# zengxianyu/sketchedit

Hardware: AMD Instinct MI355X
Metric: images/sec (higher is better)
Workload: dtype f32; 1 GPU; SketchEdit inference forward (netM+netG, use_cam, pool max) 256x256 batch 32 per GPU, procedural weights; global_batch=32, size=256, per_gpu_batch=32, execution=default, two streams

## Files before the change

### sketchedit_amd/_lib.py

```python
import contextlib
import ctypes
import os
import subprocess
import threading

import numpy as np

_HERE = os.path.dirname(os.path.abspath(__file__))
LIB_PATH = os.environ.get("SKETCHEDIT_HIP_LIB") or os.path.join(_HERE, "lib", "libsketchedit_hip.so")
CSRC = os.path.join(_HERE, "csrc")
SOURCES = ["se_gconv.hip", "se_rconv16.hip", "se_rconv96.hip", "se_rtile.hip", "se_rtilew.hip", "se_wino.hip", "se_wino24.hip", "se_wino48.hip", "se_wino_up.hip", "se_wino_up48.hip", "se_s2poly.hip", "se_attention.hip", "se_att_stream.hip", "se_misc.hip", "se_resize.hip",
           "se_window.hip", "se_feather.hip", "se_fill.hip", "se_select.hip", "se_lasso.hip", "se_modify.hip", "se_outline.hip", "se_move.hip", "se_blend.hip", "se_canvas.hip", "se_warp.hip", "se_filter.hip", "se_adjust.hip", "se_png.hip", "se_jpg.hip", "se_pack.hip",
           "se_plan.hip", "se_api_window.hip", "se_api_select.hip", "se_api_move.hip", "se_api_codec.hip", "se_api_debug.hip", "se_api.hip"]

SE_NET_G, SE_NET_M = 0, 1
RESAMPLE_LANCZOS, RESAMPLE_BILINEAR, RESAMPLE_BICUBIC = 1, 2, 3
FLAG_USE_CAM, FLAG_POOL_MAX, FLAG_NO_MASK_CC, FLAG_NO_MASK_COARSE, FLAG_JOINT_TRAIN_INP = 1, 2, 4, 8, 16
FLAG_LOW_LATENCY, FLAG_GRAPH, FLAG_PACKED_OUT, FLAG_BF16, FLAG_CONSERVATIVE = 32, 64, 128, 256, 512
LOW_LATENCY_MAX_PIXELS = 3 * 256 * 256
LOW_LATENCY_MAX_SINGLE_IMAGE = 512 * 512

SYMBOLS = ["se_create", "se_destroy", "se_last_error", "se_version", "se_load_weights", "se_weights_ready",
           "se_workspace_bytes", "se_netM_forward", "se_netM_forward_ex", "se_netG_forward", "se_netG_forward_taps", "se_inference", "se_inference_u8", "se_gated_conv2d",
           "se_gated_conv2d_ex", "se_attention", "se_attention_ex", "se_quantize_u8", "se_dequantize_u8", "se_inference_u8io", "se_profile_enable",
           "se_profile_report", "se_debug_set_option", "se_debug_get_option", "se_debug_reset_options", "se_debug_gconv_form",
           "se_resize_u8", "se_prepare_u8", "se_edit_u8", "se_edit_u8_workspace_bytes", "se_resample_coeffs",
           "se_window_gather_u8", "se_window_border_u8", "se_window_paste_u8", "se_edit_window_u8", "se_edit_window_u8_workspace_bytes",
           "se_window_gather_resize_u8", "se_window_paste_resize_u8", "se_edit_window_scaled_u8", "se_edit_window_scaled_u8_workspace_bytes",
           "se_window_saved_bytes", "se_window_save_u8", "se_window_swap_u8",
           "se_inference_locked", "se_inference_u8_locked", "se_window_gather_lock_u8", "se_window_paste_locked_u8",
           "se_edit_window_locked_u8", "se_edit_window_locked_u8_workspace_bytes", "se_sketch_tiles_u8",
           "se_sketch_strokes_u8",
           "se_pack_inputs", "se_column_reduce", "se_output_conv"]
PNG_SYMBOLS = ["se_png_bound", "se_png_encode_u8", "se_png_encode_u8_workspace_bytes"]
JPG_SYMBOLS = ["se_jpg_bound", "se_jpg_encode_u8", "se_jpg_encode_u8_workspace_bytes"]
JPG2_SYMBOLS = ["se_jpg2_bound", "se_jpg2_encode_u8", "se_jpg2_encode_u8_workspace_bytes", "se_jpg2_code_i16",
                "se_jpg2_code_i16_workspace_bytes"]
SE_JPG_420, SE_JPG_OPTIMIZE = 1, 2
JPG_TABLE_RECORD_BYTES = 1088
FEATHER_SYMBOLS = ["se_window_paste_feather_u8"]
FEATHER_MAX_RADIUS = 16
FILL_SYMBOLS = ["se_fill", "se_fill_window_u8", "se_fill_window_u8_workspace_bytes", "se_fill_keep_u8"]
SELECT_SYMBOLS = ["se_select_similar_u8", "se_select_flood_u8", "se_select_grow_u8"]
SELECT_MAX_GROW, SELECT_MAX_PASSES = 16, 64
LASSO_SYMBOLS = ["se_lasso_fill_u8", "se_plane_combine_u8"]
LASSO_MAX_EDGES, LASSO_MAX_EXTENT = 65536, 8192
COMBINE_ADD, COMBINE_SUBTRACT, COMBINE_INTERSECT, COMBINE_XOR, COMBINE_INVERT = range(5)
OUTLINE_SYMBOLS = ["se_outline_u8_workspace_bytes", "se_outline_u8"]
OUTLINE_TILE, OUTLINE_MAX_CAP = 64, 1 << 24
MOVE_SYMBOLS = ["se_move_drop_u8", "se_plane_shift_u8"]
MOVE_MAX_OFFSET, MOVE_MAX_RADIUS = 16384, 16
MOVE_FLIP_X, MOVE_FLIP_Y = 1, 2
BLEND_ENTRIES = ["sketchedit_move_blend_u8_workspace_bytes", "sketchedit_move_blend_u8"]
BLEND_MAX_SIDE = 2048
CANVAS_ENTRIES = ["skedit_canvas_u8"]
CANVAS_MIRROR_X, CANVAS_MIRROR_Y, CANVAS_TRANSPOSE = 1, 2, 4
CANVAS_EDGE, CANVAS_REFLECT, CANVAS_CONSTANT = 0, 1, 2
CANVAS_MAX_SIDE, CANVAS_MAX_OFFSET = 32768, 1 << 20
WARP_SYMBOLS = ["se_warp_drop_u8", "se_plane_warp_u8"]
WARP_MAX_COEF, WARP_MAX_TRANSLATION = 1 << 20, 1 << 40
FILTER_SYMBOLS = ["se_filter_blur_u8", "se_filter_mosaic_u8"]
FILTER_MAX_RADIUS, FILTER_ONE, FILTER_MAX_CELL = 32, 4096, 64
FILTER_MIN_AMOUNT, FILTER_MAX_AMOUNT, FILTER_MAX_FEATHER = -256, 1024, 16

ADJUST_SYMBOLS = ["se_adjust_u8", "se_adjust_hist_u8_workspace_bytes", "se_adjust_hist_u8", "se_adjust_lut_u8"]
ADJUST_MAX_COEF, ADJUST_MAX_OFFSET, ADJUST_ONE_AMOUNT = 32768, 1 << 20, 256
ADJUST_MAX_FEATHER, ADJUST_MAX_CLIP, ADJUST_HIST_GROUPS = 16, 200, 256
ADJUST_STRETCH, ADJUST_EQUALIZE, ADJUST_MATCH = 0, 1, 2
ADJUST_PER_CHANNEL, ADJUST_LUMA = 0, 1
MODIFY_SYMBOLS = ["se_plane_modify_u8"]
MODIFY_MAX_RADIUS = 32
MODIFY_EXPAND, MODIFY_CONTRACT, MODIFY_SMOOTH = range(3)


class SketchEditHipError(RuntimeError):
    pass


class NetGTaps(ctypes.Structure):
    _fields_ = [("pmconv6", ctypes.c_void_p), ("attn_out", ctypes.c_void_p), ("style_vec", ctypes.c_void_p)]


class Window(ctypes.Structure):
    _fields_ = [("frame_u8", ctypes.c_void_p), ("sketch_u8", ctypes.c_void_p), ("Hi", ctypes.c_int), ("Wi", ctypes.c_int),
                ("y0", ctypes.c_int), ("x0", ctypes.c_int)]


class OutputConvIO(ctypes.Structure):
    _fields_ = [(n, ctypes.c_void_p) for n in ("out", "hard", "lock", "img", "mask", "xnow", "composed", "rgb8", "m8")]


def build_library(force=False, verbose=False, extra_flags=()):
    import fcntl
    from concurrent.futures import ThreadPoolExecutor
    import glob
    hdrs = glob.glob(os.path.join(CSRC, "*.h")) + glob.glob(os.path.join(_HERE, "..", "include", "*.h"))
    hdr_t = max(os.path.getmtime(h) for h in hdrs)
    objdir = os.path.join(_HERE, "lib", "obj")
    os.makedirs(objdir, exist_ok=True)
    with open(os.path.join(_HERE, "lib", ".build.lock"), "w") as lock:
        fcntl.flock(lock, fcntl.LOCK_EX)
        jobs, objs = [], []
        for src in SOURCES:
            sp, op = os.path.join(CSRC, src), os.path.join(objdir, src.replace(".hip", ".o"))
            objs.append(op)
            cmd = ["hipcc", "--offload-arch=gfx950", "-O3", "-std=c++17", "-fPIC"] + list(extra_flags) + ["-c", sp, "-o", op]
            try:
                with open(op + ".cmd") as f:
                    same_cmd = f.read() == " ".join(cmd)
            except OSError:
                same_cmd = False
            if force or not same_cmd or not os.path.exists(op) or os.path.getmtime(op) < max(os.path.getmtime(sp), hdr_t):
                jobs.append(cmd)
        if not jobs and os.path.exists(LIB_PATH) and all(os.path.getmtime(LIB_PATH) >= os.path.getmtime(o) for o in objs):
            return LIB_PATH

        def run(cmd):
            if verbose:
                print(" ".join(cmd), flush=True)
            subprocess.check_call(cmd)
            if "-c" in cmd:
                with open(cmd[-1] + ".cmd", "w") as f:
                    f.write(" ".join(cmd))
        with ThreadPoolExecutor(max_workers=min(len(jobs), os.cpu_count() or 1) or 1) as ex:
            list(ex.map(run, jobs))
        run(["hipcc", "--offload-arch=gfx950", "-fPIC", "-shared", "-o", LIB_PATH + ".tmp"] + objs)
        os.replace(LIB_PATH + ".tmp", LIB_PATH)
    return LIB_PATH


_lib = None
_lib_lock = threading.Lock()


def load_library():
    global _lib
    with _lib_lock:
        if _lib is not None:
            return _lib
        if not os.path.exists(LIB_PATH):
            raise SketchEditHipError(
                "%s not found: build it with `python -c 'import __graft_entry__ as g; g.build()'` "
                "(there is no CPU or PyTorch fallback for this path)" % LIB_PATH)
        import torch
        lib = ctypes.CDLL(LIB_PATH)
        c_f = ctypes.c_void_p
        vp, ci, sz = ctypes.c_void_p, ctypes.c_int, ctypes.c_size_t
        lib.se_create.argtypes = [ci, ctypes.POINTER(vp)]
        lib.se_create.restype = ci
        lib.se_destroy.argtypes = [vp]
        lib.se_destroy.restype = None
        lib.se_last_error.argtypes = [vp]
        lib.se_last_error.restype = ctypes.c_char_p
        lib.se_version.argtypes = []
        lib.se_version.restype = ctypes.c_char_p
        lib.se_load_weights.argtypes = [vp, ci, ctypes.c_char_p, c_f, ctypes.POINTER(ci), ci]
        lib.se_load_weights.restype = ci
        lib.se_weights_ready.argtypes = [vp]
        lib.se_weights_ready.restype = ci
        lib.se_workspace_bytes.argtypes = [vp, ci, ci, ci]
        lib.se_workspace_bytes.restype = sz
        lib.se_netM_forward.argtypes = [vp, vp, c_f, c_f, c_f, c_f, vp, sz, ci, ci, ci]
        lib.se_netM_forward.restype = ci
        lib.se_netM_forward_ex.argtypes = [vp, vp, c_f, c_f, c_f, c_f, vp, sz, ci, ci, ci, ci]
        lib.se_netM_forward_ex.restype = ci
        lib.se_netG_forward.argtypes = [vp, vp, c_f, c_f, c_f, c_f, c_f, c_f, c_f, vp, sz, ci, ci, ci, ci]
        lib.se_netG_forward.restype = ci
        lib.se_netG_forward_taps.argtypes = [vp, vp, c_f, c_f, c_f, c_f, c_f, c_f, c_f, vp, sz, ci, ci, ci, ci, ctypes.POINTER(NetGTaps)]
        lib.se_netG_forward_taps.restype = ci
        lib.se_inference.argtypes = [vp, vp, c_f, c_f, c_f, c_f, c_f, c_f, c_f, c_f, vp, sz, ci, ci, ci, ci]
        lib.se_inference.restype = ci
        lib.se_inference_u8.argtypes = [vp, vp, c_f, c_f, vp, vp, vp, sz, ci, ci, ci, ci]
        lib.se_inference_u8.restype = ci
        lib.se_gated_conv2d.argtypes = [vp, vp, c_f, c_f, c_f, c_f] + [ci] * 10
        lib.se_gated_conv2d.restype = ci
        lib.se_gated_conv2d_ex.argtypes = [vp, vp, c_f, c_f, ci, c_f, c_f, c_f] + [ci] * 12
        lib.se_gated_conv2d_ex.restype = ci
        lib.se_attention.argtypes = [vp, vp, c_f, c_f, c_f, c_f, ci, ci, ci]
        lib.se_attention.restype = ci
        lib.se_attention_ex.argtypes = [vp, vp, c_f, c_f, c_f, c_f, ci, ci, ci, ci]
        lib.se_attention_ex.restype = ci
        lib.se_quantize_u8.argtypes = [vp, vp, c_f, c_f, vp, vp, ci, ci, ci]
        lib.se_quantize_u8.restype = ci
        lib.se_dequantize_u8.argtypes = [vp, vp, vp, vp, c_f, c_f, ci, ci, ci]
        lib.se_dequantize_u8.restype = ci
        lib.se_inference_u8io.argtypes = [vp, vp, vp, vp, vp, vp, vp, sz, ci, ci, ci, ci]
        lib.se_inference_u8io.restype = ci
        lib.se_resize_u8.argtypes = [vp, vp, vp, ci, ci, ci, ci, vp, ci, ci, ci]
        lib.se_resize_u8.restype = ci
        lib.se_prepare_u8.argtypes = [vp, vp, vp, ci, ci, vp, ci, ci, c_f, c_f, ci, ci]
        lib.se_prepare_u8.restype = ci
        lib.se_edit_u8.argtypes = [vp, vp, vp, vp, vp, vp, sz, ci, ci, ci, ci, ci, ci]
        lib.se_edit_u8.restype = ci
        lib.se_edit_u8_workspace_bytes.argtypes = [vp, ci, ci, ci]
        lib.se_edit_u8_workspace_bytes.restype = sz
        lib.se_window_gather_u8.argtypes = [vp, vp, ctypes.POINTER(Window), ci, ci, ci, c_f, c_f]
        lib.se_window_gather_u8.restype = ci
        lib.se_window_border_u8.argtypes = [vp, vp, ctypes.POINTER(Window), ci, ci, ci, vp, vp]
        lib.se_window_border_u8.restype = ci
        lib.se_window_paste_u8.argtypes = [vp, vp, ctypes.POINTER(Window), ci, ci, ci, vp, vp]
        lib.se_window_paste_u8.restype = ci
        lib.se_edit_window_u8.argtypes = [vp, vp, ctypes.POINTER(Window), ci, ci, ci, vp, vp, vp, ci, vp, sz, ci]
        lib.se_edit_window_u8.restype = ci
        lib.se_edit_window_u8_workspace_bytes.argtypes = [vp, ci, ci, ci]
        lib.se_edit_window_u8_workspace_bytes.restype = sz
        lib.se_window_gather_resize_u8.argtypes = [vp, vp, ctypes.POINTER(Window), ci, ci, ci, ci, ci, c_f, c_f]
        lib.se_window_gather_resize_u8.restype = ci
        lib.se_window_paste_resize_u8.argtypes = [vp, vp, ctypes.POINTER(Window), ci, ci, ci, ci, ci, vp, vp]
        lib.se_window_paste_resize_u8.restype = ci
        lib.se_edit_window_scaled_u8.argtypes = [vp, vp, ctypes.POINTER(Window), ci, ci, ci, ci, ci, vp, vp, vp, ci, vp, sz, ci]
        lib.se_edit_window_scaled_u8.restype = ci
        lib.se_edit_window_scaled_u8_workspace_bytes.argtypes = [vp, ci, ci, ci, ci, ci]
        lib.se_edit_window_scaled_u8_workspace_bytes.restype = sz
        lib.se_window_saved_bytes.argtypes = [ci, ci]
        lib.se_window_saved_bytes.restype = sz
        lib.se_window_save_u8.argtypes = [vp, vp, ctypes.POINTER(Window), ci, ci, ci, ctypes.POINTER(vp)]
        lib.se_window_save_u8.restype = ci
        lib.se_window_swap_u8.argtypes = [vp, vp, ctypes.POINTER(Window), ci, ci, ci, ctypes.POINTER(vp)]
        lib.se_window_swap_u8.restype = ci
        lib.se_inference_locked.argtypes = [vp, vp, c_f, c_f, vp, c_f, c_f, c_f, c_f, c_f, c_f, vp, sz, ci, ci, ci, ci]
        lib.se_inference_locked.restype = ci
        lib.se_inference_u8_locked.argtypes = [vp, vp, c_f, c_f, vp, vp, vp, vp, sz, ci, ci, ci, ci]
        lib.se_inference_u8_locked.restype = ci
        lib.se_window_gather_lock_u8.argtypes = [vp, vp, ctypes.POINTER(Window), ctypes.POINTER(vp), ci, ci, ci, ci, ci, vp]
        lib.se_window_gather_lock_u8.restype = ci
        lib.se_window_paste_locked_u8.argtypes = [vp, vp, ctypes.POINTER(Window), ctypes.POINTER(vp), ci, ci, ci, ci, ci, vp, vp]
        lib.se_window_paste_locked_u8.restype = ci
        lib.se_edit_window_locked_u8.argtypes = [vp, vp, ctypes.POINTER(Window), ctypes.POINTER(vp), ci, ci, ci, ci, ci, vp, vp, vp, ci, vp, sz, ci]
        lib.se_edit_window_locked_u8.restype = ci
        lib.se_edit_window_locked_u8_workspace_bytes.argtypes = [vp, ci, ci, ci, ci, ci]
        lib.se_edit_window_locked_u8_workspace_bytes.restype = sz
        lib.se_sketch_tiles_u8.argtypes = [vp, vp, vp, ci, ci, ci, vp]
        lib.se_sketch_tiles_u8.restype = ci
        lib.se_sketch_strokes_u8.argtypes = [vp, vp, vp, ci, ci, ci, vp, ci, vp, vp]
        lib.se_sketch_strokes_u8.restype = ci
        lib.se_pack_inputs.argtypes = [vp, vp, ci, c_f, c_f, c_f, c_f, c_f, vp, vp, ci, ci, ci, ci, ci]
        lib.se_pack_inputs.restype = ci
        lib.se_column_reduce.argtypes = [vp, vp, c_f, c_f, vp, ci, ci, ci, ci, ci, ci]
        lib.se_column_reduce.restype = ci
        lib.se_output_conv.argtypes = [vp, vp, c_f, c_f, c_f, ci, ci, ci, ci, ci, ctypes.POINTER(OutputConvIO), ci, ci, ci]
        lib.se_output_conv.restype = ci
        lib.se_png_bound.argtypes = [ci, ci]
        lib.se_png_bound.restype = sz
        lib.se_png_encode_u8.argtypes = [vp, vp, ctypes.POINTER(Window), ci, ci, ci, vp, sz, vp, vp, sz]
        lib.se_png_encode_u8.restype = ci
        lib.se_png_encode_u8_workspace_bytes.argtypes = [vp, ci, ci, ci]
        lib.se_png_encode_u8_workspace_bytes.restype = sz
        lib.se_jpg_bound.argtypes = [ci, ci]
        lib.se_jpg_bound.restype = sz
        lib.se_jpg_encode_u8.argtypes = [vp, vp, ctypes.POINTER(Window), ci, ci, ci, ci, vp, sz, vp, vp, sz]
        lib.se_jpg_encode_u8.restype = ci
        lib.se_jpg_encode_u8_workspace_bytes.argtypes = [vp, ci, ci, ci]
        lib.se_jpg_encode_u8_workspace_bytes.restype = sz
        lib.se_jpg2_bound.argtypes = [ci, ci, ci]
        lib.se_jpg2_bound.restype = sz
        lib.se_jpg2_encode_u8.argtypes = [vp, vp, ctypes.POINTER(Window), ci, ci, ci, ci, ci, vp, sz, vp, vp, vp, sz]
        lib.se_jpg2_encode_u8.restype = ci
        lib.se_jpg2_encode_u8_workspace_bytes.argtypes = [vp, ci, ci, ci, ci]
        lib.se_jpg2_encode_u8_workspace_bytes.restype = sz
        lib.se_jpg2_code_i16.argtypes = [vp, vp, vp, ci, ci, ci, ci, vp, sz, vp, vp, vp, sz]
        lib.se_jpg2_code_i16.restype = ci
        lib.se_jpg2_code_i16_workspace_bytes.argtypes = [vp, ci, ci, ci, ci]
        lib.se_jpg2_code_i16_workspace_bytes.restype = sz
        lib.se_window_paste_feather_u8.argtypes = [vp, vp, ctypes.POINTER(Window), ctypes.POINTER(vp), ci, ci, ci, ci, vp, vp]
        lib.se_window_paste_feather_u8.restype = ci
        lib.se_fill.argtypes = [vp, vp, c_f, c_f, vp, vp, c_f, c_f, c_f, c_f, vp, sz, ci, ci, ci, ci]
        lib.se_fill.restype = ci
        lib.se_fill_window_u8.argtypes = [vp, vp, ctypes.POINTER(Window), ctypes.POINTER(vp), ctypes.POINTER(vp), ci, ci, ci, ci, ci, vp, vp, vp, sz, ci]
        lib.se_fill_window_u8.restype = ci
        lib.se_fill_window_u8_workspace_bytes.argtypes = [vp, ci, ci, ci, ci, ci]
        lib.se_fill_window_u8_workspace_bytes.restype = sz
        lib.se_fill_keep_u8.argtypes = [vp, vp, ctypes.POINTER(Window), ctypes.POINTER(vp), ctypes.POINTER(vp), ctypes.POINTER(vp), ci, ci, ci]
        lib.se_fill_keep_u8.restype = ci
        lib.se_select_similar_u8.argtypes = [vp, vp, vp, ci, ci, ci, ci, ci, ci, vp]
        lib.se_select_similar_u8.restype = ci
        lib.se_select_flood_u8.argtypes = [vp, vp, vp, ci, ci, ci, vp]
        lib.se_select_flood_u8.restype = ci
        lib.se_select_grow_u8.argtypes = [vp, vp, vp, ci, ci, ci, vp]
        lib.se_select_grow_u8.restype = ci
        lib.se_lasso_fill_u8.argtypes = [vp, vp, vp, ci, ci, ci, vp]
        lib.se_lasso_fill_u8.restype = ci
        lib.se_plane_combine_u8.argtypes = [vp, vp, vp, vp, ci, ci, ci, vp]
        lib.se_plane_combine_u8.restype = ci
        lib.se_plane_modify_u8.argtypes = [vp, vp, vp, ci, ci, ci, ci, vp]
        lib.se_plane_modify_u8.restype = ci
        lib.se_move_drop_u8.argtypes =[vp, vp, vp, ci, ci, vp, ci, ci, ci, ci, vp, vp] + [ci] * 8
        lib.se_move_drop_u8.restype = ci
        lib.sketchedit_move_blend_u8_workspace_bytes.argtypes = [ci, ci]
        lib.sketchedit_move_blend_u8_workspace_bytes.restype = sz
        lib.sketchedit_move_blend_u8.argtypes = [vp, vp, vp, ci, ci, vp, ci, ci, ci, ci, vp, vp] + [ci] * 7 + [vp, sz]
        lib.sketchedit_move_blend_u8.restype = ci
        lib.skedit_canvas_u8.argtypes = [vp, vp, vp, ci, ci, ci, vp, ci, ci, ci, ci, ci, ci, ctypes.c_uint]
        lib.skedit_canvas_u8.restype = ci
        lib.se_plane_shift_u8.argtypes = [vp, vp, vp, ci, ci] + [ci] * 7 + [vp]
        lib.se_plane_shift_u8.restype = ci
        lib.se_warp_drop_u8.argtypes = [vp, vp, vp, ci, ci, vp, ci, ci, ci, ci, vp, vp] + [ci] * 8 + [vp]
        lib.se_warp_drop_u8.restype = ci
        lib.se_plane_warp_u8.argtypes = [vp, vp, vp, ci, ci] + [ci] * 4 + [vp, vp]
        lib.se_plane_warp_u8.restype = ci
        lib.se_filter_blur_u8.argtypes = [vp, vp, vp, ci, ci, vp, ci, ci, ci, ci, vp, vp] + [ci] * 4 + [vp, ci, ci, ci]
        lib.se_filter_blur_u8.restype = ci
        lib.se_filter_mosaic_u8.argtypes = [vp, vp, vp, ci, ci, vp, ci, ci, ci, ci, vp, vp] + [ci] * 7
        lib.se_filter_mosaic_u8.restype = ci
        lib.se_adjust_u8.argtypes = [vp, vp, vp, ci, ci, vp, ci, ci, ci, ci, vp, vp] + [ci] * 4 + [vp, vp, ci, ci]
        lib.se_adjust_u8.restype = ci
        lib.se_adjust_hist_u8_workspace_bytes.argtypes = [ci, ci]
        lib.se_adjust_hist_u8_workspace_bytes.restype = sz
        lib.se_adjust_hist_u8.argtypes = [vp, vp, vp, ci, ci, vp] + [ci] * 4 + [vp, vp, sz]
        lib.se_adjust_hist_u8.restype = ci
        lib.se_adjust_lut_u8.argtypes = [vp, vp, vp, vp, ci, ci, ci, vp]
        lib.se_adjust_lut_u8.restype = ci
        lib.se_outline_u8_workspace_bytes.argtypes = [vp, ci, ci]
        lib.se_outline_u8_workspace_bytes.restype = sz
        lib.se_outline_u8.argtypes = [vp, vp, vp, ci, ci, vp, ci, vp, vp, sz]
        lib.se_outline_u8.restype = ci
        lib.se_resample_coeffs.argtypes = [ci, ci, ci, vp, vp, sz]
        lib.se_resample_coeffs.restype = ci
        lib.se_profile_enable.argtypes = [vp, ci]
        lib.se_profile_enable.restype = ci
        lib.se_profile_report.argtypes = [vp, ctypes.c_char_p, sz]
        lib.se_profile_report.restype = ci
        lib.se_debug_set_option.argtypes = [ctypes.c_char_p, ci]
        lib.se_debug_set_option.restype = ci
        lib.se_debug_get_option.argtypes = [ctypes.c_char_p, ctypes.POINTER(ci)]
        lib.se_debug_get_option.restype = ci
        lib.se_debug_reset_options.argtypes = []
        lib.se_debug_reset_options.restype = None
        _lib = lib
        return lib


_shared = {}
_shared_lock = threading.Lock()


def shared_engine(device=0):
    with _shared_lock:
        if device not in _shared:
            _shared[device] = Engine(device)
        return _shared[device]


def set_option(name, value):
    if load_library().se_debug_set_option(name.encode(), int(value)):
        raise SketchEditHipError("unknown developer switch %r" % name)


def get_option(name):
    v = ctypes.c_int(0)
    if load_library().se_debug_get_option(name.encode(), ctypes.byref(v)):
        raise SketchEditHipError("unknown developer switch %r" % name)
    return v.value


def reset_options():
    load_library().se_debug_reset_options()


def gconv_form(cin, cout, H, W, k=3, stride=1, rate=1, act="elu", upsample=False, cin1=0, x1_is_vector=False, B=1,
               low_latency=False, bf16=False, conservative=False, net=SE_NET_G):
    flags = (FLAG_LOW_LATENCY if low_latency else 0) | (FLAG_BF16 if bf16 else 0) | (FLAG_CONSERVATIVE if conservative else 0)
    buf = ctypes.create_string_buffer(64)
    fn = load_library().se_debug_gconv_form
    fn.argtypes, fn.restype = [ctypes.c_int] * 14 + [ctypes.c_char_p, ctypes.c_size_t], ctypes.c_int
    if fn(cin, cin1, int(bool(x1_is_vector)), cout, k, stride, rate, {"elu": 0, "relu": 1, None: 2}[act],
          int(bool(upsample)), B, H, W, flags, net, buf, len(buf)):
        raise SketchEditHipError("gconv_form: not a layer gated_conv2d takes")
    return buf.value.decode().split(",")


def s2poly_tables():
    return np.array([[get_option("SE_S2POLY_TABLE:%d,%d" % (q, j)) for j in range(7)] for q in range(5)], np.int32)


def s2poly_probe_layer(cout):
    p = lambda n: (((7919 * n) % 2053 - 1026) / 1024.0).astype(np.float32)
    return p(np.arange(cout * 48 * 9, dtype=np.int64)).reshape(cout, 48, 3, 3), p(10007 + np.arange(cout, dtype=np.int64))


def s2poly_probe_pack(cout):
    fn = load_library().se_debug_get_option
    n = (cout // 96) * 38 * 96 * 32
    out = np.zeros(n + cout, np.int32)
    v = ctypes.c_int(0)
    for i in range(n + cout):
        if fn(("SE_S2POLY_PACK:%d,%d" % (cout, i)).encode(), ctypes.byref(v)):
            raise SketchEditHipError("SE_S2POLY_PACK: cout must be 96 or 192")
        out[i] = v.value
    f = out.view(np.float32)
    return f[:n].reshape(cout // 96, 38, 96, 32).copy(), f[n:].copy()


def pair_rule(B, H, W, low_latency=False):
    v = ctypes.c_int(-1)
    name = "SE_PAIR_RULE:%d,%d,%d,%d" % (B, H, W, FLAG_LOW_LATENCY if low_latency else 0)
    if load_library().se_debug_get_option(name.encode(), ctypes.byref(v)):
        raise SketchEditHipError("pair_rule: bad shape B=%d H=%d W=%d" % (B, H, W))
    return bool(v.value)


def flags_from_opt(opt):
    f = 0
    if getattr(opt, "use_cam", False):
        f |= FLAG_USE_CAM
    pool = getattr(opt, "pool_type", "avg")
    if pool == "max":
        f |= FLAG_POOL_MAX
    elif pool != "avg":
        raise NotImplementedError(pool)
    if getattr(opt, "no_mask_cc", False):
        f |= FLAG_NO_MASK_CC
    if getattr(opt, "no_mask_coarse", False):
        f |= FLAG_NO_MASK_COARSE
    if getattr(opt, "joint_train_inp", False):
        f |= FLAG_JOINT_TRAIN_INP
    return f


def _ptr(t):
    return None if t is None else ctypes.c_void_p(t.data_ptr())


def _check_dev(*ts):
    import torch
    for t in ts:
        if t is None:
            continue
        if not (isinstance(t, torch.Tensor) and t.is_cuda and t.dtype == torch.float32 and t.is_contiguous()):
            raise SketchEditHipError("expected contiguous float32 CUDA(HIP) tensors")


def upload_u8(a, device):
    import warnings
    import torch
    if isinstance(a, np.ndarray):
        with warnings.catch_warnings():
            warnings.simplefilter("ignore", UserWarning)
            a = torch.from_numpy(np.ascontiguousarray(a))
    return a.to(device, non_blocking=True).contiguous()


def _check_dev_u8(*ts):
    import torch
    for t in ts:
        if not (isinstance(t, torch.Tensor) and t.is_cuda and t.dtype == torch.uint8 and t.is_contiguous()):
            raise SketchEditHipError("expected contiguous uint8 CUDA(HIP) tensors")


class Engine:

    def __init__(self, device=0):
        import torch
        if not torch.cuda.is_available():
            raise SketchEditHipError("no HIP device visible: the sketchedit_amd forward only runs on an MI355X")
        self.lib = load_library()
        self.device = int(device)
        h = ctypes.c_void_p()
        if self.lib.se_create(self.device, ctypes.byref(h)) != 0:
            raise SketchEditHipError("se_create: " + self.lib.se_last_error(None).decode())
        self.h = h
        self._ws = None
        self._ws_lock = threading.Lock()
        self._ws_stream = None
        self._graph_stream = None
        self.precision = "f32"
        self.conservative = False
        self._static = {}
        self._graph_lock = threading.Lock()

    def close(self):
        if getattr(self, "h", None):
            self.lib.se_destroy(self.h)
            self.h = None

    def __del__(self):
        try:
            self.close()
        except Exception:
            pass

    def _err(self, what):
        raise SketchEditHipError("%s: %s" % (what, self.lib.se_last_error(self.h).decode()))

    def load_state_dict(self, net, state_dict):
        net_id = SE_NET_G if net == "G" else SE_NET_M
        for k, v in state_dict.items():
            a = v.detach().cpu().numpy() if hasattr(v, "detach") else np.asarray(v)
            a = np.ascontiguousarray(a, dtype=np.float32)
            shape = (ctypes.c_int * a.ndim)(*a.shape)
            if self.lib.se_load_weights(self.h, net_id, k.encode(), a.ctypes.data_as(ctypes.c_void_p), shape, a.ndim):
                self._err("se_load_weights(%s)" % k)

    def weights_ready(self):
        return bool(self.lib.se_weights_ready(self.h))

    def workspace(self, B, H, W):
        need = self.lib.se_workspace_bytes(self.h, B, H, W)
        if need == 0:
            self._err("se_workspace_bytes")
        return self._workspace_bytes(need)

    def _workspace_bytes(self, need):
        import torch
        with self._ws_lock:
            cur = torch.cuda.current_stream(self.device)
            if self._ws is None or self._ws.numel() < need:
                if self._ws is not None:
                    self._ws.record_stream(self._ws_stream)
                self._ws = torch.empty(need, dtype=torch.uint8, device="cuda:%d" % self.device)
                with self._graph_lock:
                    self._static.clear()
            elif self._ws_stream is not None and self._ws_stream != cur:
                cur.wait_stream(self._ws_stream)
            self._ws_stream = cur
            return self._ws

    def _stream(self):
        import torch
        return ctypes.c_void_p(torch.cuda.current_stream(self.device).cuda_stream)

    def netM(self, image, sketch, want_image=True):
        import torch
        _check_dev(image, sketch)
        B, _, H, W = image.shape
        ws = self.workspace(B, H, W)
        mask = torch.empty((B, 1, H, W), dtype=torch.float32, device=image.device)
        mim = torch.empty((B, 3, H, W), dtype=torch.float32, device=image.device) if want_image else None
        if self.lib.se_netM_forward_ex(self.h, self._stream(), _ptr(image), _ptr(sketch), _ptr(mask), _ptr(mim),
                                       _ptr(ws), ws.numel(), B, H, W,
                                       (FLAG_BF16 if self.precision == "bf16" else 0) | (FLAG_CONSERVATIVE if self.conservative else 0)):
            self._err("se_netM_forward_ex")
        return mask, mim

    def netG(self, x, x2, mask, mask2, guide, flags):
        import torch
        _check_dev(x, x2, mask, mask2, guide)
        B, _, H, W = x.shape
        ws = self.workspace(B, H, W)
        coarse = torch.empty((B, 3, H, W), dtype=torch.float32, device=x.device)
        fine = torch.empty_like(coarse)
        flags = (flags & 31) | (FLAG_BF16 if self.precision == "bf16" else 0)
        if self.lib.se_netG_forward(self.h, self._stream(), _ptr(x), _ptr(x2), _ptr(mask), _ptr(mask2), _ptr(guide),
                                    _ptr(coarse), _ptr(fine), _ptr(ws), ws.numel(), B, H, W, flags):
            self._err("se_netG_forward")
        return coarse, fine

    def netG_taps(self, x, x2, mask, mask2, guide, flags):
        import torch
        _check_dev(x, x2, mask, mask2, guide)
        B, _, H, W = x.shape
        ws = self.workspace(B, H, W)
        mk = lambda *shape: torch.empty(shape, dtype=torch.float32, device=x.device)
        r = dict(coarse=mk(B, 3, H, W), fine=mk(B, 3, H, W), pmconv6=mk(B, 96, H // 4, W // 4), style_vec=mk(B, 96))
        if flags & FLAG_USE_CAM:
            r["attn_out"] = mk(B, 96, H // 4, W // 4)
        taps = NetGTaps(r["pmconv6"].data_ptr(), r["attn_out"].data_ptr() if "attn_out" in r else None, r["style_vec"].data_ptr())
        flags = (flags & 31) | (FLAG_BF16 if self.precision == "bf16" else 0)
        if self.lib.se_netG_forward_taps(self.h, self._stream(), _ptr(x), _ptr(x2), _ptr(mask), _ptr(mask2), _ptr(guide),
                                         _ptr(r["coarse"]), _ptr(r["fine"]), _ptr(ws), ws.numel(), B, H, W, flags, ctypes.byref(taps)):
            self._err("se_netG_forward_taps")
        return r

    def set_conservative(self, on=True):
        self.conservative = bool(on)

    def set_precision(self, precision):
        if precision not in ("f32", "bf16"):
            raise ValueError(precision)
        self.precision = precision

    @staticmethod
    def is_low_latency(B, H, W, low_latency=None):
        if low_latency is not None:
            return bool(low_latency)
        return B * H * W <= LOW_LATENCY_MAX_PIXELS or (B == 1 and H * W <= LOW_LATENCY_MAX_SINGLE_IMAGE)

    def exec_flags(self, B, H, W, low_latency=None, graph=False):
        return (FLAG_LOW_LATENCY if self.is_low_latency(B, H, W, low_latency) else 0) | (FLAG_GRAPH if graph else 0) | \
            (FLAG_BF16 if self.precision == "bf16" else 0) | (FLAG_CONSERVATIVE if self.conservative else 0)

    def inference(self, image, sketch, flags, visualize=False, out=None, low_latency=None, graph=False, lock=None):
        import torch
        _check_dev(image, sketch)
        if lock is not None:
            self._check_lock(lock, image)
            graph = False
        if graph and out is not None:
            raise SketchEditHipError("graph=True replays into buffers the Engine keeps per shape: `out=` cannot be honoured "
                                     "(copy from the returned tensors, or call without graph=True)")
        B, _, H, W = image.shape
        ws = self.workspace(B, H, W)
        dev = image.device
        flags = (flags & 31) | self.exec_flags(B, H, W, low_latency, graph)

        def new_outputs(have=None):
            mk = lambda c: torch.empty((B, c, H, W), dtype=torch.float32, device=dev)
            o = dict(composed=have["composed"], mask=have["mask"]) if have else dict(composed=mk(3), mask=mk(1))
            if visualize:
                o.update(hard=mk(1), maskim=mk(3), coarse=mk(3), fine=mk(3))
            return o

        if graph:
            with self._graph_lock:
                return self._inference_graph(image, sketch, flags, visualize, ws, B, H, W, new_outputs)
        r = new_outputs(out)
        self._call_inference(image, sketch, r, ws, B, H, W, flags, self._stream(), lock)
        return r

    @staticmethod
    def _check_lock(lock, image):
        _check_dev_u8(lock)
        B, _, H, W = image.shape
        if tuple(lock.shape) != (B, H, W):
            raise SketchEditHipError("lock: expected a (B,H,W) uint8 plane of the images' size")

    def _call_inference(self, image, sketch, r, ws, B, H, W, flags, stream, lock=None):
        if lock is not None:
            if self.lib.se_inference_locked(self.h, stream, _ptr(image), _ptr(sketch), _ptr(lock), _ptr(r["composed"]),
                                            _ptr(r["mask"]), _ptr(r.get("hard")), _ptr(r.get("maskim")), _ptr(r.get("coarse")),
                                            _ptr(r.get("fine")), _ptr(ws), ws.numel(), B, H, W, flags):
                self._err("se_inference_locked")
            return
        if self.lib.se_inference(self.h, stream, _ptr(image), _ptr(sketch), _ptr(r["composed"]), _ptr(r["mask"]),
                                 _ptr(r.get("hard")), _ptr(r.get("maskim")), _ptr(r.get("coarse")), _ptr(r.get("fine")),
                                 _ptr(ws), ws.numel(), B, H, W, flags):
            self._err("se_inference")

    def _inference_graph(self, image, sketch, flags, visualize, ws, B, H, W, new_outputs):
        import torch
        key = (B, H, W, bool(visualize))
        st = self._static.get(key)
        if st is None:
            st = self._static[key] = {"image": torch.empty_like(image), "sketch": torch.empty_like(sketch),
                                      "outs": new_outputs()}
        st["image"].copy_(image)
        st["sketch"].copy_(sketch)
        image, sketch = st["image"], st["sketch"]
        r = dict(st["outs"])
        cur = torch.cuda.current_stream(self.device)
        if self._graph_stream is None:
            self._graph_stream = torch.cuda.Stream(device=self.device)
        gs = self._graph_stream
        gs.wait_stream(cur)
        self._call_inference(image, sketch, r, ws, B, H, W, flags, ctypes.c_void_p(gs.cuda_stream))
        cur.wait_stream(gs)
        return r

    def inference_u8(self, image, sketch, flags, low_latency=None, lock=None):
        import torch
        _check_dev(image, sketch)
        if lock is not None:
            self._check_lock(lock, image)
        B, _, H, W = image.shape
        ws = self.workspace(B, H, W)
        rgb = torch.empty((B, H, W, 3), dtype=torch.uint8, device=image.device)
        m8 = torch.empty((B, H, W), dtype=torch.uint8, device=image.device)
        flags = (flags & 31) | self.exec_flags(B, H, W, low_latency, False)
        if lock is not None:
            if self.lib.se_inference_u8_locked(self.h, self._stream(), _ptr(image), _ptr(sketch), _ptr(lock), _ptr(rgb), _ptr(m8),
                                               _ptr(ws), ws.numel(), B, H, W, flags):
                self._err("se_inference_u8_locked")
        elif self.lib.se_inference_u8(self.h, self._stream(), _ptr(image), _ptr(sketch), _ptr(rgb), _ptr(m8), _ptr(ws),
                                      ws.numel(), B, H, W, flags):
            self._err("se_inference_u8")
        return rgb, m8

    def dequantize_u8(self, image_u8, sketch_u8):
        import torch
        _check_dev_u8(image_u8, sketch_u8)
        B, H, W, _ = image_u8.shape
        image = torch.empty((B, 3, H, W), dtype=torch.float32, device=image_u8.device)
        sketch = torch.empty((B, 1, H, W), dtype=torch.float32, device=image_u8.device)
        if self.lib.se_dequantize_u8(self.h, self._stream(), _ptr(image_u8), _ptr(sketch_u8), _ptr(image), _ptr(sketch), B, H, W):
            self._err("se_dequantize_u8")
        return image, sketch

    def inference_u8io(self, image_u8, sketch_u8, flags, low_latency=None, out=None):
        import torch
        _check_dev_u8(image_u8, sketch_u8)
        B, H, W, _ = image_u8.shape
        assert tuple(sketch_u8.shape) == (B, H, W)
        ws = self.workspace(B, H, W)
        rgb, m8 = out if out is not None else (torch.empty((B, H, W, 3), dtype=torch.uint8, device=image_u8.device),
                                               torch.empty((B, H, W), dtype=torch.uint8, device=image_u8.device))
        flags = (flags & 31) | self.exec_flags(B, H, W, low_latency, False)
        if self.lib.se_inference_u8io(self.h, self._stream(), _ptr(image_u8), _ptr(sketch_u8), _ptr(rgb), _ptr(m8), _ptr(ws),
                                      ws.numel(), B, H, W, flags):
            self._err("se_inference_u8io")
        return rgb, m8

    def resize_u8(self, x, size, filter=RESAMPLE_BICUBIC, out=None):
        import torch
        _check_dev_u8(x)
        flat = x.dim() == 3
        B, Hin, Win = x.shape[:3]
# ... 845 lines not shown
```

### sketchedit_amd/csrc/se_api_debug.hip

```cpp
#include "se_host.h"
#include "se_s2poly.h"

using namespace se;

extern "C" {

int se_profile_enable(se_ctx* c, int on) {
  if (!c) return 1;
  std::lock_guard<std::mutex> lk(c->mu);
  HIPCHK(c, hipSetDevice(c->device));
  c->prof.recs.clear();
  c->prof.used = 0;
  if (on && c->prof.pool.empty()) {
    c->prof.pool.resize(2 * 1024);
    for (auto& e : c->prof.pool) HIPCHK(c, hipEventCreate(&e));
  }
  c->prof.on = on != 0;
  return 0;
}

int se_profile_report(se_ctx* c, char* buf, size_t cap) {
  if (!c || !buf || cap < 64) return 1;
  std::lock_guard<std::mutex> lk(c->mu);
  HIPCHK(c, hipSetDevice(c->device));
  HIPCHK(c, hipDeviceSynchronize());
  double ms[PL_COUNT] = {0}, fl[PL_COUNT] = {0}, by[PL_COUNT] = {0}, ex[PL_COUNT] = {0}, bl[PL_COUNT] = {0};
  long n[PL_COUNT] = {0};
  for (auto& r : c->prof.recs) {
    float t = 0.f;
    if (hipEventElapsedTime(&t, r.a, r.b) == hipSuccess) { ms[r.label] += t; fl[r.label] += r.flops; ex[r.label] += r.exec_flops; by[r.label] += r.bytes; bl[r.label] += (double)r.blocks; n[r.label]++; }
  }
  std::string s = "{\"kernels\": [";
  bool first = true;
  for (int l = 0; l < PL_COUNT; ++l) {
    if (!n[l]) continue;
    char t[384];
    snprintf(t, sizeof t, "%s{\"kernel\": \"%s\", \"launches\": %ld, \"total_ms\": %.6f, \"flops\": %.6e, \"flops_executed\": %.6e, \"bytes\": %.6e, \"workgroups\": %.1f}",
             first ? "" : ", ", prof_label_name(l), n[l], ms[l], fl[l], ex[l], by[l], bl[l] / (double)n[l]);
    s += t;
    first = false;
  }
  s += "], \"layers\": [";
  std::vector<std::string> keys;
  std::map<std::string, std::pair<double, double>> agg;
  std::map<std::string, double> aggx;
  std::map<std::string, long> cnt;
  for (auto& r : c->prof.recs) {
    if (!r.name) continue;
    float t = 0.f;
    if (hipEventElapsedTime(&t, r.a, r.b) != hipSuccess) continue;
    std::string k = std::string(prof_label_name(r.label)) + ":" + r.name;
    if (!cnt.count(k)) keys.push_back(k);
    agg[k].first += t; agg[k].second += r.flops; aggx[k] += r.exec_flops; cnt[k]++;
  }
  first = true;
  for (auto& k : keys) {
    char t[384];
    snprintf(t, sizeof t, "%s{\"layer\": \"%s\", \"launches\": %ld, \"total_ms\": %.6f, \"flops\": %.6e, \"flops_executed\": %.6e}",
             first ? "" : ", ", k.c_str(), cnt[k], agg[k].first, agg[k].second, aggx[k]);
    s += t;
    first = false;
  }
  s += "], \"launches\": [";
  first = true;
  for (auto& r : c->prof.recs) {
    char t[256];
    snprintf(t, sizeof t, "%s{\"form\": \"%s\", \"kernel\": \"%s\", \"layer\": \"%s\", \"workgroups\": %ld}", first ? "" : ", ",
             r.form ? r.form : "?", prof_label_name(r.label), r.name ? r.name : "", r.blocks);
    s += t;
    first = false;
  }
  s += "]}";
  if (s.size() + 1 > cap) return fail(c, "profile buffer too small");
  memcpy(buf, s.c_str(), s.size() + 1);
  return 0;
}

int se_debug_set_option(const char* name, int value) { return opt_set(name, value); }
int se_debug_get_option(const char* name, int* value) {
  static const char q[] = "SE_PAIR_RULE:";
  if (name && value && !strncmp(name, q, sizeof q - 1)) {
    int B = 0, H = 0, W = 0, flags = 0, end = 0;
    if (sscanf(name + sizeof q - 1, "%d,%d,%d,%d%n", &B, &H, &W, &flags, &end) != 4 || name[sizeof q - 1 + end] || B < 1 || H < 1 || W < 1) return 1;
    *value = pair_rule(B, H, W, flags) ? 1 : 0;
    return 0;
  }
  static const char qt[] = "SE_S2POLY_TABLE:", qp[] = "SE_S2POLY_PACK:";
  if (name && value && !strncmp(name, qt, sizeof qt - 1)) {
    int q = -1, j = -1, end = 0;
    if (sscanf(name + sizeof qt - 1, "%d,%d%n", &q, &j, &end) != 2 || name[sizeof qt - 1 + end] || q < 0 || q > 4 || j < 0 || j > 6) return 1;
    *value = j == 0 ? s2poly_src_a(q) : j == 1 ? s2poly_src_b(q) : j < 5 ? s2poly_wcoef(q, j - 2) : s2poly_fold(q, j - 5);
    return 0;
  }
  if (name && value && !strncmp(name, qp, sizeof qp - 1)) {
    int cout = 0, end = 0;
    long long i = -1;
    if (sscanf(name + sizeof qp - 1, "%d,%lld%n", &cout, &i, &end) != 2 || name[sizeof qp - 1 + end] || (cout != 96 && cout != 192) || i < 0) return 1;
    static std::mutex mu;
    static std::vector<float> kept[2];
    std::lock_guard<std::mutex> lk(mu);
    std::vector<float>& all = kept[cout == 192];
    if (all.empty()) {
      auto probe = [](long long n) { return (float)((7919 * n) % 2053 - 1026) / 1024.f; };
      std::vector<float> w((size_t)cout * 48 * 9), b(cout), bias;
      for (size_t n = 0; n < w.size(); ++n) w[n] = probe((long long)n);
      for (int n = 0; n < cout; ++n) b[n] = probe(10007 + n);
      if (!s2poly_pack_host(w.data(), b.data(), cout, all, bias)) return 1;
      all.insert(all.end(), bias.begin(), bias.end());
    }
    if ((size_t)i >= all.size()) return 1;
    memcpy(value, &all[(size_t)i], sizeof(int));
    return 0;
  }
  return opt_get(name, value);
}
void se_debug_reset_options(void) { opt_reset(); }

int se_debug_gconv_form(int cin, int cin1, int src1_is_vector, int cout, int k, int stride, int rate, int act, int upsample,
                        int B, int H, int W, int exec_flags, int net_id, char* out, size_t cap) {
  if (!out || cin <= 0 || cin1 < 0 || cout <= 0 || k <= 0 || stride <= 0 || rate <= 0 || B <= 0 || H <= 0 || W <= 0) return 1;
  const bool bf = (exec_flags & SE_FLAG_BF16) != 0;
  const int gran = bf ? 8 : 4;
  if (cin1 && ((cin % gran) || (cin1 % gran))) return 1;
  const LayerDef d = {"test", cin + cin1, cout, k, stride, rate, act, upsample};
  const bool raw = small_layer(d);
  if (raw && (k != 3 || cin != 12 || cin1 || (cout != 1 && cout != 3) || stride != 1 || rate != 1 || upsample)) return 1;
  if (!raw && (cout % 8)) return 1;
  const LayerFacts f = layer_facts(d, cin + cin1);
  if (!raw && f.cfg < 0) return 1;
  const int Cp = (cin + gran - 1) & ~(gran - 1);
  if (!raw && Cp + cin1 != f.CG[bf] * gran) return 1;
  const bool vec = cin1 && src1_is_vector;
  const ConvCall q = {d, f, B, H, W, Cp, cin1, cin1 ? (vec ? SRC2_VECTOR : SRC2_TENSOR) : SRC2_NONE, bf,
                      (exec_flags & SE_FLAG_LOW_LATENCY) != 0, (exec_flags & SE_FLAG_CONSERVATIVE) != 0, net_id, vec};
  const Choice ch = choose_form(q);
  const char* name = form_name(ch, q);
  if (!name) return 1;
  const std::string s = std::string(ch.fold ? "vecbias," : "") + name;
  if (s.size() + 1 > cap) return 1;
  memcpy(out, s.c_str(), s.size() + 1);
  return 0;
}

int se_gated_conv2d_ex(se_ctx* c, void* stream, const float* x, const float* x1, int x1_is_vector, const float* w_host,
                       const float* b_host, float* y, int B, int Cin, int Cin1, int H, int W, int Cout, int k, int stride,
                       int rate, int act, int upsample, int exec_flags) {
  if (!c || !x || !w_host || !b_host || !y) return 1;
  std::lock_guard<std::mutex> lk(c->mu);
  HIPCHK(c, hipSetDevice(c->device));
  begin_call(c, stream, exec_flags & (SE_FLAG_LOW_LATENCY | SE_FLAG_BF16));
  const bool bf = c->bf16;
  if (!x1) Cin1 = 0;
  if (x1 && ((Cin % 4) || (Cin1 % 4))) return fail(c, "two-source conv: channel counts must be multiples of 4");
  if (bf && x1 && ((Cin % 8) || (Cin1 % 8))) return fail(c, "two-source bf16 conv: channel counts must be multiples of 8");
  const int CinT = Cin + Cin1;
  Layer L;
  L.def = LayerDef{"test", CinT, Cout, k, stride, rate, act, upsample};
  const bool raw = small_layer(L.def);
  if (raw && (k != 3 || CinT != 12 || x1 || (Cout != 1 && Cout != 3) || stride != 1 || rate != 1 || upsample))
    return fail(c, "raw conv: only 3x3 12->{1,3}");
  if (!raw && (Cout % 8)) return fail(c, "gated conv needs Cout %% 8 == 0");
  L.w.assign(w_host, w_host + (size_t)Cout * CinT * k * k);
  L.b.assign(b_host, b_host + Cout);
  std::vector<int> chans(CinT);
  std::iota(chans.begin(), chans.end(), 0);
  if (pack_layer_images(L, chans, c->err)) return 1;
  const int Cp = bf ? (Cin + 7) & ~7 : (Cin + 3) & ~3;
  DevBuf xin, x1in, yout, vb_test;
  struct Drain {
    se_ctx* c;
    ~Drain() {
      (void)hipStreamSynchronize(c->st);
      c->vbias_ws = nullptr; c->vec32 = nullptr;
    }
  } drain{c};
  HIPCHK(c, xin.alloc((size_t)B * H * W * Cp * 4));
  if (poison(c, xin, (size_t)B * H * W * Cp * 4, c->st)) return 1;
  int rc = (bf ? launch_nchw_to_nhwc16 : launch_nchw_to_nhwc)(x, xin, B, Cin, Cp, H, W, c->st) != hipSuccess;
  if (!rc && x1) {
    const size_t n1 = x1_is_vector ? (size_t)B * Cin1 : (size_t)B * H * W * Cin1;
    HIPCHK(c, x1in.alloc(n1 * 4));
    if (poison(c, x1in, n1 * 4, c->st)) return 1;
    if (x1_is_vector && !bf) rc = hipMemcpyAsync(x1in, x1, n1 * 4, hipMemcpyDeviceToDevice, c->st) != hipSuccess;
    else if (x1_is_vector) rc = launch_nchw_to_nhwc16(x1, x1in, B, Cin1, Cin1, 1, 1, c->st) != hipSuccess;
    else rc = (bf ? launch_nchw_to_nhwc16 : launch_nchw_to_nhwc)(x1, x1in, B, Cin1, Cin1, H, W, c->st) != hipSuccess;
  }
  if (!rc && raw) {
    SmallConvParams sp;
    memset(&sp, 0, sizeof sp);
    sp.x = xin; sp.w = L.direct[bf]; sp.b = L.d_b; sp.B = B; sp.H = H; sp.W = W; sp.cout = Cout; sp.mode = 4;
    sp.bf16 = bf ? 1 : 0;
    sp.out_nchw = y;
    rc = launch_small_conv(sp, c->st) != hipSuccess;
  } else if (!rc) {
    const ConvShape sh = conv_shape(L.def, H, W);
    const int Gs = bf ? (Cout / 2 + 7) & ~7 : Cout / 2;
    HIPCHK(c, yout.alloc((size_t)B * sh.Ho * sh.Wo * Gs * 4));
    if (poison(c, yout, (size_t)B * sh.Ho * sh.Wo * Gs * 4, c->st)) return 1;
    if (x1in && x1_is_vector) {
      HIPCHK(c, vb_test.alloc((size_t)B * 9 * 192 * 4));
      if (poison(c, vb_test, (size_t)B * 9 * 192 * 4, c->st)) return 1;
      c->vbias_ws = vb_test;
      c->vec32 = bf ? x1 : nullptr;
    }
    rc = run_gconv(c, L, xin, Cp, x1in, Cin1, x1_is_vector, yout, B, H, W);
    if (!rc) rc = (bf ? launch_nhwc16_to_nchw : launch_nhwc_to_nchw)(yout, y, B, Cout / 2, Gs, sh.Ho, sh.Wo, c->st) != hipSuccess;
  }
  return rc;
}

int se_gated_conv2d(se_ctx* c, void* stream, const float* x, const float* w_host, const float* b_host, float* y, int B,
                    int Cin, int H, int W, int Cout, int k, int stride, int rate, int act, int upsample) {
  return se_gated_conv2d_ex(c, stream, x, nullptr, 0, w_host, b_host, y, B, Cin, 0, H, W, Cout, k, stride, rate, act,
                            upsample, 0);
}

int se_attention_ex(se_ctx* c, void* stream, const float* x, const float* mask_full, float* out, float* similar_out, int B,
                    int h, int w, int exec_flags) {
  if (!c || !x || !mask_full || !out) return 1;
  std::lock_guard<std::mutex> lk(c->mu);
  if (h < 4 || w < 4 || (h % 2) || (w % 2)) return fail(c, "attention: h, w must be even and >= 4");
  HIPCHK(c, hipSetDevice(c->device));
  begin_call(c, stream, exec_flags & SE_FLAG_BF16);
  const bool bf = c->bf16;
  const int R = (h / 2) * (w / 2), Rp = att_row_stride(R, true) + 64;
  const bool streaming = att_streaming(h, w, bf, similar_out != nullptr);
  const int L = ((h - 4) / 2 + 1) * ((w - 4) / 2 + 1);
  if (streaming && similar_out)
    return fail(c, "attention: similar_out (the %d x %d score matrix) is not available on a %dx%d feature map: "
                   "it runs in the streaming form, which never forms it", L, L, h, w);
  const size_t rr = streaming ? 0 : 2 * (size_t)B * R * Rp;
  const size_t bytes = ((size_t)B * h * w * 96 * 3 + rr + (size_t)B * Rp * (7 + 4 * 96) + 64 * 96 * B + 2 * (size_t)B * R + 9 * (size_t)(w / 2 + 72) + (size_t)B * (768 + (h / 2) * 384)) * 4 + (1 << 16);
  char* ws = nullptr;
  HIPCHK(c, hipMalloc(&ws, bytes));
  if (poison(c, ws, bytes, c->st)) { (void)hipStreamSynchronize(c->st); (void)hipFree(ws); return 1; }
  c->arena.reset(ws, bytes, false);
  c->arena2.reset(nullptr, 0, false);
  Plan P(c, c->G, B);
  Act xin = P.alloc(h, w, 96), o = P.alloc(h, w, 96);
  int rc = P.rc;
  if (!rc) rc = (bf ? launch_nchw_to_nhwc16 : launch_nchw_to_nhwc)(x, xin.p, B, 96, 96, h, w, c->st) != hipSuccess;
  if (!rc) rc = run_attention(c, P, xin, mask_full, o, similar_out);
  if (!rc) rc = (bf ? launch_nhwc16_to_nchw : launch_nhwc_to_nchw)(o.p, out, B, 96, 96, h, w, c->st) != hipSuccess;
  (void)hipStreamSynchronize(c->st);
  (void)hipFree(ws);
  return rc;
}

int se_attention(se_ctx* c, void* stream, const float* x, const float* mask_full, float* out, float* similar_out, int B,
                 int h, int w) {
  return se_attention_ex(c, stream, x, mask_full, out, similar_out, B, h, w, 0);
}

int se_pack_inputs(se_ctx* c, void* stream, int net_id, const float* x, const float* x2, const float* mask, const float* mask2,
                   const float* guide, void* packed_out, void* style_out, int B, int H, int W, int flags, int exec_flags) {
  if (!c) return 1;
  std::lock_guard<std::mutex> lk(c->mu);
  if (B < 1 || H < 1 || W < 1) return fail(c, "pack: bad shape B=%d H=%d W=%d", B, H, W);
  if (net_id != SE_NET_M && net_id != SE_NET_G) return fail(c, "pack: net_id must be SE_NET_G or SE_NET_M");
  if (!x || !guide || !packed_out || (net_id == SE_NET_G && (!x2 || !mask || !mask2 || !style_out))) return fail(c, "null pointer argument");
  HIPCHK(c, hipSetDevice(c->device));
  begin_call(c, stream, exec_flags & SE_FLAG_BF16);
  if (net_id == SE_NET_M) {
    HIPCHK(c, (c->bf16 ? launch_pack_m16 : launch_pack_m)(x, guide, (float*)packed_out, B, H, W, c->st));
  } else {
    HIPCHK(c, (c->bf16 ? launch_pack_g16 : launch_pack_g)(x, x2, mask, mask2, guide, (float*)packed_out, (float*)style_out, B, H, W,
                                                          (flags & SE_FLAG_NO_MASK_CC) ? 1 : 0,
                                                          (flags & SE_FLAG_JOINT_TRAIN_INP) ? 1 : 0, c->st));
  }
  return 0;
}

int se_column_reduce(se_ctx* c, void* stream, const float* x, float* out, unsigned short* out_bf16, int B, int C, int H, int W,
                     int op, int exec_flags) {
  if (!c) return 1;
  std::lock_guard<std::mutex> lk(c->mu);
  if (!x || !out) return fail(c, "null pointer argument");
  if (B < 1 || C < 1 || H < 1 || W < 1) return fail(c, "column reduce: bad shape B=%d C=%d H=%d W=%d", B, C, H, W);
  if (op < 0 || op > 2) return fail(c, "column reduce: op must be 0 (max), 1 (mean) or 2 (rsqrt of the sum of squares)");
  const bool bf = (exec_flags & SE_FLAG_BF16) != 0;
  if (C > 256 || C % (bf ? 8 : 4))
    return fail(c, "column reduce: C = %d must be a multiple of %d and at most 256", C, bf ? 8 : 4);
  if ((double)B * H * W * C * (bf ? 2 : 4) >= 2147483648.0) return fail(c, "column reduce: B H W C beyond the 32-bit byte range");
  HIPCHK(c, hipSetDevice(c->device));
  begin_call(c, stream, exec_flags & SE_FLAG_BF16);
  DevBuf xin, part;
  struct Drain {
    se_ctx* c;
    ~Drain() { (void)hipStreamSynchronize(c->st); }
  } drain{c};
  const size_t xbytes = (size_t)B * H * W * C * (bf ? 2 : 4), pbytes = (size_t)B * COLREDUCE_SPLITS * C * 4;
  HIPCHK(c, xin.alloc(xbytes));
  HIPCHK(c, part.alloc(pbytes));
  if (poison(c, xin, xbytes, c->st) || poison(c, part, pbytes, c->st)) return 1;
  HIPCHK(c, (bf ? launch_nchw_to_nhwc16 : launch_nchw_to_nhwc)(x, xin, B, C, C, H, W, c->st));
  HIPCHK(c, launch_colreduce(xin, part, out, B, H * W, C, op, c->st, bf ? 1 : 0, (float*)out_bf16));
  return 0;
}

int se_output_conv(se_ctx* c, void* stream, const float* x, const float* w_host, const float* b_host, int B, int H, int W, int cout,
                   int mode, const se_output_conv_io* io, int no_mask_coarse, int packed, int exec_flags) {
  if (!c) return 1;
  std::lock_guard<std::mutex> lk(c->mu);
  if (!x || !w_host || !b_host || !io) return fail(c, "null pointer argument");
  if (B < 1 || H < 1 || W < 1) return fail(c, "output conv: bad shape B=%d H=%d W=%d", B, H, W);
  if (mode < 0 || mode > 3) return fail(c, "output conv: mode must be 0..3");
  if (cout != (mode == 0 ? 1 : 3)) return fail(c, "output conv: mode %d has %d output channels", mode, mode == 0 ? 1 : 3);
  if (mode == 0 && !io->out) return fail(c, "output conv: mode 0 writes `out`");
  if (mode == 2 && (!io->img || !io->mask || !io->xnow)) return fail(c, "output conv: mode 2 needs img, mask and xnow");
  if (mode == 3 && (io->composed || io->rgb8 || io->m8) && (!io->img || !io->mask))
    return fail(c, "output conv: the composite of mode 3 needs img and mask");
  HIPCHK(c, hipSetDevice(c->device));
  begin_call(c, stream, exec_flags & SE_FLAG_BF16);
  const bool bf = c->bf16;
  Layer L;
  L.def = LayerDef{"test", 12, cout, 3, 1, 1, ACT_NONE, 0};
  L.w.assign(w_host, w_host + (size_t)cout * 12 * 9);
  L.b.assign(b_host, b_host + cout);
  std::vector<int> chans(12);
  std::iota(chans.begin(), chans.end(), 0);
  if (pack_layer_images(L, chans, c->err)) return 1;
  DevBuf xin;
  struct Drain {
    se_ctx* c;
    ~Drain() { (void)hipStreamSynchronize(c->st); }
  } drain{c};
  const int Cp = bf ? 16 : 12;
  const size_t xbytes = (size_t)B * H * W * Cp * (bf ? 2 : 4);
  HIPCHK(c, xin.alloc(xbytes));
  if (poison(c, xin, xbytes, c->st)) return 1;
  HIPCHK(c, (bf ? launch_nchw_to_nhwc16 : launch_nchw_to_nhwc)(x, xin, B, 12, Cp, H, W, c->st));
  SmallConvParams sp;
  memset(&sp, 0, sizeof sp);
  sp.x = xin; sp.w = L.direct[bf]; sp.b = L.d_b; sp.B = B; sp.H = H; sp.W = W; sp.cout = cout;
  sp.bf16 = bf ? 1 : 0;
  sp.mode = mode; sp.out_nchw = io->out; sp.hard = io->hard; sp.img = io->img; sp.mask = io->mask; sp.xnow = (float*)io->xnow;
  sp.composed = io->composed; sp.no_mask_coarse = no_mask_coarse ? 1 : 0;
  if (mode == 3) { sp.rgb8 = io->rgb8; sp.m8 = io->m8; }
  if (mode == 0) sp.lock = io->lock;
  if (packed) {
    const long packed_bs = 4l * H * W;
    if (mode == 0) sp.out_bs = packed_bs;
    if (mode == 3) { sp.mask_bs = packed_bs; sp.comp_bs = packed_bs; }
  }
  HIPCHK(c, launch_small_conv(sp, c->st));
  return 0;
}

}
```

### sketchedit_amd/csrc/se_dispatch.h

```cpp
#pragma once
#include "se_kernels.h"

namespace se {

enum { ACT_ELU = 0, ACT_RELU = 1, ACT_NONE = 2 };

struct LayerDef {
  const char* name;
  int cin, cout, k, stride, rate, act, up;
};

inline bool small_layer(const LayerDef& d) { return d.act == ACT_NONE || d.cout == 3; }

struct ConvShape { int Ho, Wo, pad; };
inline ConvShape conv_shape(const LayerDef& d, int Hin, int Win) {
  const int pad = d.rate * (d.k - 1) / 2;
  if (d.up) return {2 * Hin, 2 * Win, pad};
  const int span = d.rate * (d.k - 1) + 1;
  return {(Hin + 2 * pad - span) / d.stride + 1, (Win + 2 * pad - span) / d.stride + 1, pad};
}

inline int choose_cfg(int G) {
  if (G <= 16) return GC_N24;
  if (G <= 24) return GC_N48;
  if (G <= 48) return GC_N96;
  if (G <= 96) return GC_N192;
  return -1;
}

inline bool rconv96_eligible(const LayerDef& d) {
  if (d.cout != 96 || d.rate != 1 || d.k != 3 || d.act == ACT_NONE) return false;
  if (d.stride == 2) return !d.up && d.cin == 24;
  if (d.stride != 1) return false;
  return d.up ? d.cin == 96 : (d.cin == 48 || d.cin == 24);
}

struct LayerFacts {
  bool small;
  int cfg, NP, G, T;
  int nch[2], CG[2];
  int dense, nchd;
  bool u, ub, u1, wv, wv16, u24, ub24, u24b, wx, wx2, wd, wdw, w16d, w16s, w96;
  bool s2p;
};

inline LayerFacts layer_facts(const LayerDef& d, int nchans) {
  LayerFacts f = {};
  f.cfg = -1;
  f.small = small_layer(d);
  if (f.small) return f;
  f.G = d.cout / 2;
  if (choose_cfg(f.G) < 0 || (f.G % 4)) return f;
  f.cfg = choose_cfg(f.G);
  f.NP = gconv_np(f.cfg);
  const int KW = d.up ? 2 : d.k;
  f.T = KW * KW;
  for (int bf = 0; bf < 2; ++bf) {
    const int per = bf ? 8 : 4, Cp = (nchans + per - 1) / per * per;
    f.CG[bf] = Cp / per;
    f.nch[bf] = (f.T * Cp + 8 * per - 1) / (8 * per);
  }
  const bool first = d.k == 5 && d.stride == 1 && d.rate == 1 && d.cout == 48;
  f.w16d = first && nchans >= 3 && nchans <= 4;
  f.wd = f.wdw = first && nchans >= 3 && nchans <= 5;
  f.dense = f.wd ? nchans : 0;
  f.nchd = (25 * f.dense + 31) / 32;
  f.w16s = d.k == 3 && d.stride == 1 && !d.up && (d.cin == 96 || d.cin == 192) && d.cout == 192;
  f.w96 = rconv96_eligible(d);
  f.s2p = d.k == 3 && d.stride == 2 && d.rate == 1 && !d.up && nchans == 48 && d.cin == 48 && (d.cout == 96 || d.cout == 192);
  if (d.k != 3 || d.stride != 1 || (nchans + 3) / 4 * 4 != d.cin) return f;
  if (d.up) {
    f.u = f.ub = (d.cin == 96 && d.cout == 96) || (d.cin == 48 && d.cout == 48);
  } else if ((d.cin == 96 || d.cin == 192) && d.cout == 192) {
    f.u = f.u24 = f.ub24 = true;
    f.u1 = f.wv = f.wv16 = f.u24b = d.cin == 192;
  } else if (d.cin == 48 && d.cout == 192) {
    f.u24 = f.ub24 = true;
  } else if (d.cin == 24 && d.cout == 24 && d.rate == 1) {
    f.wx = f.wx2 = true;
  } else if ((d.cin == 48 || d.cin == 24) && d.cout == 96) {
    f.u = f.ub = true;
  }
  return f;
}

enum { SRC2_NONE = 0, SRC2_TENSOR = 1, SRC2_VECTOR = 2 };
struct ConvCall {
  LayerDef def; LayerFacts facts;
  int B, Hin, Win, C0, C1;
  int src2;
  bool bf16, low_latency, conservative;
  int net;
  bool fold_scratch;
};

enum Form {
  F_SMALL_CONV, F_WINO, F_WINO24, F_WINO24_C48, F_WINO48, F_WINO48_C24, F_WINOUP, F_WINOUP48, F_RTILEW, F_RTILEW2,
  F_RTILE_DENSE5, F_RTILE_DENSE5W, F_RTILE_D4, F_RTILE, F_RCONV16, F_RCONV16_DUAL, F_RCONV96, F_S2POLY48, F_GATHER
};
struct Choice {
  Form form;
  bool fold;
  bool wino_range;
};

inline bool magic_cg_ok(int CG, int nch) {
  const int m = (65536 + CG - 1) / CG;
  for (int gi = 0; gi < nch * 8 + 8; ++gi)
    if (((gi * m) >> 16) != gi / CG) return false;
  return true;
}
inline bool magic_kw_ok(int KW, int T) {
  const int m = 256 / KW + 1;
  for (int t = 0; t <= T + 8; ++t)
    if (((t * m) >> 8) != t / KW) return false;
  return true;
}

inline Form choose_rtile(const ConvCall& q) {
  const LayerDef& d = q.def;
  const LayerFacts& f = q.facts;
  const bool bf = q.bf16;
  const int Hin = q.Hin, Win = q.Win, C0 = q.C0;
  const long long B = q.B;
  if (!opt(OPT_RTILE) || q.src2 || d.stride != 1 || d.rate != 1 || (f.cfg != GC_N48 && f.cfg != GC_N24)) return F_GATHER;
  const int TR = rtile_rows(bf);
  const long tiles = (long)((Hin + TR - 1) / TR) * ((Win + 15) / 16) * (d.up ? 4 : 1);
  if (q.low_latency && tiles < opt(OPT_RTILE_LL_MIN)) return F_GATHER;
  const int es = bf ? 2 : 4, gran = bf ? 8 : 4;
  if (C0 != f.CG[bf] * gran) return F_GATHER;
  const int wx_mode = opt(OPT_RTILE_WX);
  if (wx_mode != 0 && !bf && f.wx && d.k == 3 && !d.up && C0 == 24 && d.cin == 24 && d.cout == 24 && (Win % 2) == 0 &&
      B * Hin * Win * 96 < (1ll << 31))
    return wx_mode != 1 && f.wx2 && (Hin % 2) == 0 ? F_RTILEW2 : F_RTILEW;
  if (opt(OPT_RTILE_DENSE) != 0 && !bf && f.wd && f.dense && d.k == 5 && !d.up && f.cfg == GC_N48 && (long long)Hin * Win * C0 * 4 < (1ll << 31))
    return opt(OPT_RTILE_D5W) != 0 && f.wdw && (Win % 2) == 0 ? F_RTILE_DENSE5W : F_RTILE_DENSE5;
  if (opt(OPT_RTILE_DENSE) != 0 && bf && f.w16d && d.k == 5 && !d.up && f.cfg == GC_N48 && C0 == 8 && B * Hin * Win * 16 < (1ll << 31))
    return F_RTILE_D4;
  const int KW = d.up ? 2 : d.k;
  const int raw_bytes = ((TR + KW - 1) * (16 + KW - 1) * C0 * es + 1023) & ~1023;
  if (raw_bytes + f.nch[bf] * f.NP * 128 > 80 * 1024) return F_GATHER;
  if (B * Hin * Win * C0 * es >= (1ll << 31)) return F_GATHER;
  if (!magic_cg_ok(f.CG[bf], f.nch[bf]) || !magic_kw_ok(KW, f.T)) return F_GATHER;
  return F_RTILE;
}

inline bool rconv16_dual_ok(const LayerFacts& f, const LayerDef& d, int Hin, int Win) {
  if (opt(OPT_RCONV16_DUAL) == 0) return false;
  return f.w16s && (d.rate % 2) == 0 && Win / d.rate == 8 && Hin / d.rate <= 8 && Hin / d.rate >= 4;
}

inline Choice choose_form(const ConvCall& q) {
  const LayerDef& d = q.def;
  const LayerFacts& f = q.facts;
  const int Hin = q.Hin, Win = q.Win, C0 = q.C0, C1 = q.C1;
  const long long B = q.B;
  const bool two = q.src2 != SRC2_NONE, vec = q.src2 == SRC2_VECTOR, ll = q.low_latency;
  const ConvShape sh = conv_shape(d, Hin, Win);
  Choice ch = {F_GATHER, false, false};
  auto is = [&](Form form) { ch.form = form; return ch; };
  if (f.small) return is(F_SMALL_CONV);
  if (q.bf16) {
    const bool use_rconv = opt(OPT_RCONV16) != 0 && !ll && d.k == 3 && d.stride == 1 && !d.up && d.cout == 192 && C0 == 96 && f.w16s &&
                           B * Hin * Win * 192 < (1ll << 31);
    if (opt(OPT_VECBIAS) != 0 && use_rconv && vec && q.fold_scratch && f.wv16 && d.rate == 1 && d.cin == 192 && C1 == 96 && Hin >= 12 && Win >= 12) {
      ch.fold = true;
      return is(F_RCONV16);
    }
    if (use_rconv && d.cin == 96 && !two && (Hin % d.rate) == 0 && (Win % d.rate) == 0 && f.nch[1] == 14) {
      if (Hin / d.rate >= 12 && Win / d.rate >= 12) return is(F_RCONV16);
      if (rconv16_dual_ok(f, d, Hin, Win)) return is(F_RCONV16_DUAL);
    }
    if (opt(OPT_RCONV96) != 0 && !ll && f.w96 && !two && C0 == d.cin && Hin >= 12 && Win >= 12 &&
        B * sh.Ho * sh.Wo * 96 < (1ll << 31) && B * Hin * Win * C0 * 2 < (1ll << 31))
      return is(F_RCONV96);
    return is(choose_rtile(q));
  }
  auto grid_ok = [&](long wgs, int min_wg) { return !ll || (min_wg > 0 && wgs >= min_wg); };
  const int min192 = opt(OPT_LL_WINO_MIN_WG), min48 = opt(OPT_LL_WINO48_MIN_WG);
  const int f43_mode = opt(OPT_WINOGRAD_F43);
  const bool use_wino = opt(OPT_WINOGRAD) != 0;
  const bool even2 = (Hin % (2 * d.rate)) == 0 && (Win % (2 * d.rate)) == 0;
  const long wg64 = ((long)(Hin / 2) * (Win / 2) + 63) / 64;
  const bool fits96 = B * Hin * Win * 384 < (1ll << 31), fits48 = B * Hin * Win * 192 < (1ll << 31);
  const bool wino_src_ok = (!two && C0 == 96 && d.cin == 96) || (two && C0 == 96 && C1 == 96 && d.cin == 192);
  if (use_wino && !d.up && f.u && wino_src_ok && !fits96) ch.wino_range = true;
  if (use_wino && !d.up && f.u && wino_src_ok && fits96 && even2 && grid_ok(wg64, min192)) {
    ch.fold = opt(OPT_VECBIAS) != 0 && vec && d.rate == 1 && f.u1 && f.wv && q.fold_scratch && Hin >= 2 && Win >= 2;
    const bool s1 = two && !ch.fold;
    const bool f43_net_ok = q.net == 0 || (f43_mode == 1 && !q.conservative);
    const bool f43 = (f43_mode == 1 || f43_mode == 2) && f43_net_ok && (s1 ? (!vec && f.u24b) : f.u24) && f.ub24 && (Win % (4 * d.rate)) == 0;
    return is(f43 ? F_WINO24 : F_WINO);
  }
  if (use_wino && f43_mode != 0 && !d.up && !two && C0 == 48 && d.cin == 48 && d.cout == 192 && d.stride == 1 && f.u24 && f.ub24 && fits96 &&
      (Hin % (2 * d.rate)) == 0 && (Win % (4 * d.rate)) == 0 && grid_ok(((long)(Hin / 2) * (Win / 4) + 31) / 32, min192))
    return is(F_WINO24_C48);
  if (use_wino && opt(OPT_WINOGRAD48) != 0 && !d.up && f.u && f.ub && !two && fits48 && even2 && grid_ok(wg64, min48)) {
    if (C0 == 48 && d.cin == 48) return is(F_WINO48);
    if (C0 == 24 && d.cin == 24 && d.cout == 96 && d.stride == 1) return is(F_WINO48_C24);
  }
  if (use_wino && opt(OPT_WINOGRAD_UP) != 0 && d.up && f.u && f.ub && !two && (Hin % 2) == 0 && (Win % 2) == 0 && grid_ok(4 * wg64, min48)) {
    if (C0 == 96 && d.cin == 96 && fits96) return is(F_WINOUP);
    if (opt(OPT_WINOGRAD_UP48) != 0 && C0 == 48 && d.cin == 48 && d.cout == 48 && fits48 && B * sh.Ho * sh.Wo * 96 < (1ll << 31)) return is(F_WINOUP48);
  }
  const int s2_mode = opt(OPT_S2_POLY);
  if ((s2_mode == 1 || (s2_mode == 2 && q.net == 0)) && !ll && f.s2p && !two && d.k == 3 && d.stride == 2 && d.rate == 1 && !d.up && C0 == 48 &&
      d.cin == 48 && (d.cout == 96 || d.cout == 192) && (Hin % 4) == 0 && (Win % 4) == 0 && fits48)
    return is(F_S2POLY48);
  return is(choose_rtile(q));
}

inline const char* gconv_form_name(int cfg, bool small_grid, bool up2, bool two_src, bool bf16) {
#define SE_GF(n) n, n "_bf16", n "_2src", n "_2src_bf16", n "_up2", n "_up2_bf16", n "_up2_2src", n "_up2_2src_bf16"
#define SE_GS(n) { SE_GF(n), SE_GF(n "_small") }
  static const char* const names[4][16] = {SE_GS("gconv_n192"), SE_GS("gconv_n96"), SE_GS("gconv_n48"), SE_GS("gconv_n24")};
#undef SE_GS
#undef SE_GF
  if (cfg < 0 || cfg > 3) return nullptr;
  return names[cfg][(small_grid ? 8 : 0) | (up2 ? 4 : 0) | (two_src ? 2 : 0) | (bf16 ? 1 : 0)];
}

inline const char* form_name(const Choice& ch, const ConvCall& q) {
  const LayerDef& d = q.def;
  const bool two = q.src2 != SRC2_NONE && !ch.fold;
  switch (ch.form) {
    case F_SMALL_CONV: return "small_conv";
    case F_WINO: return two ? "wino_2src" : "wino";
    case F_WINO24: return two ? "wino24_2src" : "wino24";
    case F_WINO24_C48: return "wino24_c48";
    case F_WINO48: return "wino48";
    case F_WINO48_C24: return "wino48_c24";
    case F_WINOUP: return "winoup";
    case F_WINOUP48: return "winoup48";
    case F_RTILEW: return "rtilew";
    case F_RTILEW2: return "rtilew2";
    case F_RTILE_DENSE5: return "rtile_dense5";
    case F_RTILE_DENSE5W: return "rtile_dense5w";
    case F_RTILE_D4: return "rtile_bf16_d4";
    case F_RTILE: return q.bf16 ? (d.up ? "rtile_bf16_up2" : "rtile_bf16") : (d.up ? "rtile_up2" : "rtile");
    case F_RCONV16: return "rconv16";
    case F_RCONV16_DUAL: return "rconv16_dual";
    case F_S2POLY48: return "s2poly48";
    case F_RCONV96: return d.up ? "rconv96_up" : d.stride == 2 ? "rconv96_s2" : q.C0 == 24 ? "rconv96_c24" : "rconv96";
    case F_GATHER: return gconv_form_name(q.facts.cfg, q.low_latency, d.up != 0, q.C0 / (q.bf16 ? 8 : 4) != q.facts.CG[q.bf16], q.bf16);
  }
  return nullptr;
}

}
```

### sketchedit_amd/csrc/se_kernels.h

```cpp
#pragma once
#include <hip/hip_runtime.h>
#include <stddef.h>
#include <stdint.h>

#include <vector>

struct se_window;

namespace se {

enum ProfLabel { PL_GCONV_N192 = 0, PL_GCONV_N96, PL_GCONV_N48, PL_GCONV_N24, PL_WINO_N192, PL_WINO_N96, PL_WINO_UP96, PL_SMALL_CONV, PL_PACK, PL_COLREDUCE,
                 PL_ATT_PREP, PL_ATT_SCORE, PL_ATT_SOFTMAX, PL_ATT_BOXSUM, PL_ATT_PV, PL_LAYOUT,
                 PL_ATT_STREAM_STATS, PL_ATT_STREAM_OUT, PL_RESIZE_H, PL_RESIZE_V, PL_WINDOW_GATHER, PL_WINDOW_BORDER, PL_WINDOW_PASTE,
                 PL_WINDOW_RESAMPLE_H, PL_WINDOW_PASTE_V, PL_WINDOW_SAVE, PL_WINDOW_SWAP, PL_WINDOW_LOCK_GATHER, PL_WINDOW_PASTE_LOCKED,
                 PL_WINDOW_PASTE_V_LOCKED, PL_SKETCH_TILES, PL_SKETCH_STROKES, PL_PNG_ROWS, PL_PNG_STRIPES,
                 PL_PNG_FINISH, PL_JPG_BLOCKS, PL_JPG_ROWS, PL_JPG_FINISH, PL_JPG2_BLOCKS, PL_JPG2_HIST, PL_JPG2_TABLES,
                 PL_WINDOW_PASTE_FEATHER, PL_FILL_MASKS, PL_FILL_KEEP, PL_BLEND_INIT, PL_BLEND_PULL, PL_BLEND_RELAX, PL_BLEND_APPLY, PL_CANVAS_MAP, PL_CANVAS_TURN,
                 PL_SELECT_SIMILAR, PL_SELECT_FLOOD, PL_SELECT_GROW, PL_MODIFY_DISC, PL_MODIFY_VOTE,
                 PL_LASSO_FILL, PL_PLANE_COMBINE, PL_ADJUST, PL_HIST_TILES, PL_HIST_SUM, PL_ADJUST_LUT, PL_OUTLINE_COUNT, PL_OUTLINE_SCAN, PL_OUTLINE_EMIT, PL_FILTER_BLUR, PL_FILTER_MOSAIC, PL_MOVE_DROP,
                 PL_PLANE_SHIFT, PL_WARP_DROP, PL_PLANE_WARP, PL_COUNT };
const char* prof_label_name(int l);
struct Profiler {
  struct Rec { int label; const char* name; const char* form; double flops; double exec_flops; double bytes; long blocks; hipEvent_t a, b; };
  std::vector<Rec> recs;
  std::vector<hipEvent_t> pool;
  size_t used = 0;
  bool on = false;
};
void set_profiler(Profiler* p);
void set_launch_cost(double flops, double bytes, const char* name = nullptr, double exec_flops = -1.0);
void set_launch_grid(long blocks);
hipError_t ensure_max_lds(const void* func, int bytes);

#define SE_OPTIONS(X)                                                                                         \
  X(XCD_REMAP, 1)                                                             \
  X(RTILE, 1)                                              \
  X(RTILE_LL_MIN, 256)         \
  X(RTILE_WX, 2)          \
  X(RTILE_DENSE, 1)                                          \
  X(RTILE_D5W, 1)                                        \
  X(TEST_OFFSET_LIMIT, 0)  \
  X(TEST_POISON, 0)       \
  X(RCONV16, 1) X(RCONV16_DUAL, 1) X(RCONV96, 1) X(VECBIAS, 1)                                                  \
  X(WINOGRAD, 1) X(WINOGRAD48, 1) X(WINOGRAD_UP, 1) X(WINOGRAD_UP48, 1)                                         \
  X(WINOGRAD_F43, 1)      \
  X(S2_POLY, 1)           \
  X(GCONV_FAST, 1) X(FORK_DEFAULT, 1) X(LL_WINO_MIN_WG, 64) X(LL_WINO48_MIN_WG, 128)                            \
  X(ATT_FUSED, -1) X(ATT_FUSED_BF16, -1) X(ATT_PTILDE_LDS, 1) X(ATT_STATS_LDS, 1) X(ATT_E16, 1) X(ATT_SYM, 1)   \
  X(ATT_STREAM, 0)        \
  X(PAIR_MIN_PIXELS, 1 << 21)
enum Opt {
#define X(name, dflt) OPT_##name,
  SE_OPTIONS(X)
#undef X
  OPT_COUNT
};
int opt(int o);
int opt_set(const char* name, int value);
int opt_get(const char* name, int* value);
void opt_reset();
long long opt_epoch();

struct GConvParams {
  const float* src0;
  const float* src1;
  const float* wpk;
  const float* bias;
  float* dst;
  const float* zeros;
  int B, Hin, Win, Ho, Wo;
  int C0, C1;
  int C0g, CG;
  int T, KW;
  int magicCG, magicKW;
  int magicKH;
  unsigned rep;
  unsigned div_hw_m, div_w_m;
  int div_hw_l, div_w_l;
  int stride, dil, pad;
  int ushift;
  int up2;
  int OH, OW;
  int Hlim, Wlim;
  int src1_vec;
  int nch;
  int G;
  int act;
  int total_pix;
  int xcd;
  int np_full;
  int nf_full;
  int bf16;
  int small_grid;
};

static inline void udiv_magic_host(unsigned d, unsigned* m, int* l) {
  int ll = 0;
  while ((1ull << ll) < d) ++ll;
  *l = ll;
  *m = (unsigned)(((1ull << 32) * ((1ull << ll) - d)) / d + 1);
}

enum GConvCfg { GC_N192 = 0, GC_N96 = 1, GC_N48 = 2, GC_N24 = 3 };
static inline int gconv_np(int cfg) { return cfg == GC_N192 ? 192 : cfg == GC_N96 ? 96 : cfg == GC_N48 ? 48 : 32; }
static inline bool gconv_mixed(int cfg) { return cfg >= GC_N48; }

hipError_t launch_gconv(int cfg, const GConvParams& p, hipStream_t st);

struct WinoParams {
  const float* src;
  const float* src1;
  int src1_vec;
  const float* upk;
  const float* bias;
  float* dst;
  int B, h, w, d;
  int th, tw;
  int total_tiles;
  int act;
  int xcd;
  unsigned div_tpi_m, div_tw_m, div_d_m;
  int div_tpi_l, div_tw_l, div_d_l;
  const float* vbias;
};
hipError_t launch_wino(const WinoParams& p, hipStream_t st);
hipError_t launch_vecbias(const float* wv, const float* vec, float* T, int B, int C1, hipStream_t st, int round_vec = 0);
hipError_t launch_wino24(const WinoParams& p, hipStream_t st);
hipError_t launch_wino24_c48(const WinoParams& p, hipStream_t st);
hipError_t launch_wino48(const WinoParams& p, hipStream_t st);
hipError_t launch_wino48_c24(const WinoParams& p, hipStream_t st);
hipError_t launch_winoup(const WinoParams& p, hipStream_t st);
hipError_t launch_winoup48(const WinoParams& p, hipStream_t st);
hipError_t launch_s2poly48(const WinoParams& p, int halves, hipStream_t st);

struct RConvParams {
  const void* src;
  const void* wpk;
  const float* bias;
  void* dst;
  int B, h, w, d;
  int hs, ws;
  int ty, tx;
  int act;
  int xcd;
  const float* vbias;
  int dual;
};
hipError_t launch_rconv16(const RConvParams& p, hipStream_t st);

struct RConv96Params {
  const void* src;
  const void* wpk;
  const float* bias;
  void* dst;
  int B, h, w;
  int CG;
  int ty, tx;
  int stride, oh, ow;
  int up2;
  int act;
  int xcd;
};
hipError_t launch_rconv96(const RConv96Params& p, hipStream_t st);

struct RTileParams {
  const float* src;
  const float* wpk;
  const float* bias;
  float* dst;
  int B, Hin, Win;
  int C;
  int CG;
  int T, KW;
  int magicCG, magicKW;
  int pad;
  int up2, OH, OW;
  int G;
  int nch, NP;
  int RH, RW;
  int raw_bytes;
  unsigned div_cg_m, div_rw_m;
  int div_cg_l, div_rw_l;
  int ty, tx;
  int act, bf16, xcd;
  int dense;
};
hipError_t launch_rtile(const RTileParams& p, hipStream_t st);
hipError_t launch_rtilew(const RTileParams& p, hipStream_t st);
hipError_t launch_rtilew2(const RTileParams& p, hipStream_t st);
int rtile_rows(bool bf16);

struct SmallConvParams {
  const float* x;
  const float* w;
  const float* b;
  int B, H, W, cout;
  int mode;
  float* out_nchw;
  float* hard;
  const float* img;
  const float* mask;
  float* xnow;
  float* composed;
  int no_mask_coarse;
  long out_bs;
  long mask_bs;
  long comp_bs;
  int bf16;
  unsigned char* rgb8;
  unsigned char* m8;
  const unsigned char* lock;
};
hipError_t launch_small_conv(const SmallConvParams& p, hipStream_t st);

hipError_t launch_pack_m(const float* image, const float* sketch, float* dst4, int B, int H, int W, hipStream_t st);
hipError_t launch_pack_g(const float* x, const float* x2, const float* mask, const float* mask2, const float* guide,
                         float* coarse8, float* style8, int B, int H, int W, int no_mask_cc, int joint,
                         hipStream_t st);
hipError_t launch_nchw_to_nhwc(const float* src, float* dst, int B, int C, int Cpad, int H, int W, hipStream_t st);
hipError_t launch_dequantize_u8(const unsigned char* rgb, const unsigned char* sk8, const float* lut, float* image, float* sketch,
                                int B, int H, int W, hipStream_t st);
hipError_t launch_nhwc_to_nchw(const float* src, float* dst, int B, int C, int Cstride, int H, int W, hipStream_t st);
hipError_t launch_quantize_u8(const float* composed, const float* mask, unsigned char* rgb, unsigned char* m8, int B, int H,
                              int W, hipStream_t st);
hipError_t launch_colreduce(const float* x, float* partial, float* out, int B, int HW, int C, int op, hipStream_t st,
                            int x_bf16 = 0, float* out_bf16 = nullptr);
hipError_t launch_pack_m16(const float* image, const float* sketch, float* dst8, int B, int H, int W, hipStream_t st);
hipError_t launch_pack_g16(const float* x, const float* x2, const float* mask, const float* mask2, const float* guide,
                           float* coarse8, float* style8, int B, int H, int W, int no_mask_cc, int joint, hipStream_t st);
hipError_t launch_nchw_to_nhwc16(const float* src, float* dst, int B, int C, int Cpad, int H, int W, hipStream_t st);
hipError_t launch_nhwc16_to_nchw(const float* src, float* dst, int B, int C, int Cstride, int H, int W, hipStream_t st);
static const int COLREDUCE_SPLITS = 128;

struct AttParams {
  const float* x;
  const float* rn;
  float* xn;
  const float* hard;
  float* valid;
  float* S;
  float* out;
  int B, h, w, hs, ws, L, Lp;
  float scale;
  float th;
  int hc, wc, R, Rp;
  float* xT;
  float* E;
  float* P;
  float* Pt;
  float* stats;
  float* kmul;
  float* kadd;
  int guard;
  float* validR;
  float* similar;
  int bf16;
  int e16;
  float* emean;
  float* epart;
  float* ea;
  float* eb;
  float* ea4;
  float* kadd2;
  int sym;
  int symT;
};
hipError_t launch_attention(const AttParams& p, hipStream_t st);
hipError_t launch_att2_prep(const AttParams& p, hipStream_t st);
hipError_t launch_attention_stream(const AttParams& p, hipStream_t st);
int att_stream_xt_tail();

int resample_ksize(int in, int out, int filter);
int resample_coeffs(int in, int out, int filter, int* bounds, int* kk);
enum { RESIZE_OUT_U8 = 0, RESIZE_OUT_IMAGE_F32 = 1, RESIZE_OUT_SKETCH_F32 = 2, RESIZE_OUT_LOCK_U8 = 3 };
struct ResizeOut {
  int mode;
  unsigned char* u8;
  float* f32;
  const float* lut;
  int H, W;
};
hipError_t launch_resample_h(const unsigned char* in, const int* d_bounds, const int* d_kk, const int* h_bounds, int ksize,
                             int B, int Hrows, int Win, int Wout, int C, const ResizeOut& o, hipStream_t st);
hipError_t launch_resample_v(const unsigned char* in, const int* d_bounds, const int* d_kk, int ksize, int B, int Hin, int Hout,
                             int W, int C, const ResizeOut& o, hipStream_t st);
hipError_t launch_window_resample_h(const se_window* d_wins, const int* d_bounds, const int* d_kk, const int* h_bounds, int ksize,
                                    int B, int hs, int ws, int Wout, int C, const ResizeOut& o, hipStream_t st);
hipError_t launch_window_paste_v(const se_window* d_wins, const unsigned char* rgb, const unsigned char* m8, const int* d_bounds,
                                 const int* d_kk, int ksize, int B, int Hin, int hs, int P, int ws, hipStream_t st, bool locked = false);
hipError_t launch_window_lock_resample_h(const se_window* d_wins, const int* d_bounds, const int* d_kk, const int* h_bounds, int ksize,
                                         int B, int hs, int ws, int Wout, const ResizeOut& o, hipStream_t st);
constexpr int RESAMPLE_MAX_KSIZE = 8191;

hipError_t launch_window_gather(const se_window* d_wins, const float* lut, float* image, float* sketch, int B, int H, int W,
                                hipStream_t st);
hipError_t launch_window_border(const se_window* d_wins, const unsigned char* m8, int* hits, int B, int H, int W, int hs, int ws,
                                hipStream_t st);
hipError_t launch_window_paste(const se_window* d_wins, const unsigned char* rgb, const unsigned char* m8, int B, int H, int W,
                               hipStream_t st, bool locked = false);
hipError_t launch_window_paste_feather(const se_window* d_wins, const unsigned char* rgb, const unsigned char* m8, int B, int hs, int ws,
                                       int radius, hipStream_t st);
hipError_t launch_window_lock_gather(const se_window* d_wins, unsigned char* out, int B, int H, int W, hipStream_t st);
hipError_t launch_window_journal(const se_window* d_wins, int B, int hs, int ws, bool swap, hipStream_t st);
hipError_t launch_sketch_tiles(const unsigned char* plane, int Hi, int Wi, int tile, int* tiles_out, hipStream_t st);
hipError_t launch_sketch_strokes(const se_window* d_wins, int B, int hs, int ws, const int* segs, long nseg_sum, unsigned char* sketch_out,
                                 hipStream_t st);
hipError_t launch_fill_masks(const unsigned char* fill, const unsigned char* lock, float* hole, float* hard, float* zero, int B, int H,
                             int W, hipStream_t st);
hipError_t launch_fill_keep(const se_window* d_wins, int B, int hs, int ws, hipStream_t st);
hipError_t launch_select_similar(const unsigned char* frame, int Hi, int Wi, int seed_y, int seed_x, int tolerance, int contiguous,
                                 unsigned char* state, hipStream_t st);
hipError_t launch_select_flood(unsigned char* state, int Hi, int Wi, unsigned* changed, hipStream_t st);
hipError_t launch_select_grow(const unsigned char* state, int Hi, int Wi, int grow, unsigned char* out, hipStream_t st);
hipError_t launch_plane_modify(const unsigned char* plane, int Hi, int Wi, int op, int radius, unsigned char* out, hipStream_t st);
hipError_t launch_lasso_fill(const int* edges, int N, int Hi, int Wi, unsigned char* plane_out, hipStream_t st);
hipError_t launch_plane_combine(const unsigned char* a, const unsigned char* b, int Hi, int Wi, int op, unsigned char* out, hipStream_t st);
hipError_t launch_outline_count(const unsigned char* plane, int Hi, int Wi, int* cnt, hipStream_t st);
hipError_t launch_outline_scan(int* cnt, int Hi, int Wi, int cap, int* info_out, hipStream_t st);
hipError_t launch_outline_emit(const unsigned char* plane, int Hi, int Wi, const int* offs, int* edges_out, int cap, hipStream_t st);
hipError_t launch_move_drop(unsigned char* frame, int Hi, int Wi, const unsigned char* lift, int ly0, int lx0, int lw, int lpitch,
                            const unsigned char* sel, const unsigned char* lock, int by0, int bx0, int by1, int bx1, int dy, int dx, int flip,
                            int radius, hipStream_t st);
hipError_t launch_plane_shift(const unsigned char* sel, int Hi, int Wi, int by0, int bx0, int by1, int bx1, int dy, int dx, int flip,
                              unsigned char* out, hipStream_t st);
size_t blend_workspace_bytes(int eh, int ew);
hipError_t launch_move_blend(unsigned char* frame, int Hi, int Wi, const unsigned char* lift, int ly0, int lx0, int lh, int lw, int lpitch,
                             const unsigned char* sel, const unsigned char* lock, int by0, int bx0, int by1, int bx1, int dy, int dx, int flip,
                             void* ws, hipStream_t st);
hipError_t launch_canvas(const unsigned char* in, int Hi, int Wi, int C, unsigned char* out, int Hn, int Wn, int oy, int ox, int orient,
                         int pad, unsigned rgb, hipStream_t st);
hipError_t launch_filter_blur(unsigned char* frame, int Hi, int Wi, const unsigned char* lift, int ly0, int lx0, int lw, int lpitch,
                              const unsigned char* sel, const unsigned char* lock, int by0, int bx0, int by1, int bx1, const int* taps,
                              int radius, int amount, int feather, hipStream_t st);
hipError_t launch_filter_mosaic(unsigned char* frame, int Hi, int Wi, const unsigned char* lift, int ly0, int lx0, int lw, int lpitch,
                                const unsigned char* sel, const unsigned char* lock, int by0, int bx0, int by1, int bx1, int cell, int amount,
                                int feather, hipStream_t st);
int adjust_hist_groups(int bh, int bw);
hipError_t launch_adjust(unsigned char* frame, int Hi, int Wi, const unsigned char* lift, int ly0, int lx0, int lw, int lpitch,
                         const unsigned char* sel, const unsigned char* lock, int by0, int bx0, int by1, int bx1, const unsigned char* lut,
                         const int* matrix, int amount, int feather, hipStream_t st);
hipError_t launch_hist_tiles(const unsigned char* frame, int Wi, const unsigned char* sel, int by0, int bx0, int by1, int bx1, unsigned* slabs,
                             hipStream_t st);
hipError_t launch_hist_sum(const unsigned* slabs, int groups, unsigned* hist, hipStream_t st);
hipError_t launch_adjust_lut(const unsigned* hist_src, const unsigned* hist_ref, int mode, int which, int clip, unsigned char* lut, hipStream_t st);
hipError_t launch_warp_drop(unsigned char* frame, int Hi, int Wi, const unsigned char* lift, int ly0, int lx0, int lw, int lpitch,
                            const unsigned char* sel, const unsigned char* lock, int by0, int bx0, int by1, int bx1, int ry0, int rx0,
                            int rh, int rw, const long long* m, hipStream_t st);
hipError_t launch_plane_warp(const unsigned char* sel, int Hi, int Wi, int by0, int bx0, int by1, int bx1, const long long* m,
                             unsigned char* out, hipStream_t st);
int png_stripes(int hs);
size_t png_stripe_bound(size_t n);
size_t png_slot_bytes(int ws);
hipError_t launch_png_rows(const se_window* d_wins, int B, int hs, int ws, unsigned char* ftype, hipStream_t st);
hipError_t launch_png_stripes(const se_window* d_wins, int B, int hs, int ws, const unsigned char* ftype, unsigned* sizes, unsigned* parts,
                              unsigned char* slots, hipStream_t st);
hipError_t launch_png_finish(int B, int hs, int ws, const unsigned* sizes, const unsigned* parts, const unsigned char* slots, unsigned char* out,
                             size_t cap, unsigned long long* sizes_out, hipStream_t st);
int jpg_rows(int hs, int flags);
int jpg_row_blocks(int ws, int flags);
size_t jpg_row_bound(int nblk, int flags);
size_t jpg_slot_bytes(int nblk, int flags);
hipError_t launch_jpg_blocks(const se_window* d_wins, int B, int hs, int ws, int quality, short* coef, hipStream_t st);
hipError_t launch_jpg2_blocks420(const se_window* d_wins, int B, int hs, int ws, int quality, short* coef, hipStream_t st);
hipError_t launch_jpg2_hist(int B, int R, int nblk, int flags, const short* coef, unsigned* hist, hipStream_t st);
hipError_t launch_jpg2_tables(int B, int R, const unsigned* hist, unsigned* codes, unsigned char* tables_out, hipStream_t st);
hipError_t launch_jpg_rows(int B, int R, int nblk, int flags, const short* coef, const unsigned* codes, unsigned* sizes,
                           unsigned char* slots, hipStream_t st);
hipError_t launch_jpg_finish(int B, int R, int nblk, size_t slot_bytes, const unsigned* sizes, const unsigned char* slots,
                             unsigned char* out, size_t cap, unsigned long long* sizes_out, hipStream_t st);

}
```

### sketchedit_amd/csrc/se_pack.h

```cpp
#pragma once
#include <hip/hip_runtime.h>

#include "se_dispatch.h"

#include <cstddef>
#include <string>
#include <vector>

namespace se {

class DevBuf {
 public:
  DevBuf() = default;
  DevBuf(const DevBuf&) = delete;
  DevBuf& operator=(const DevBuf&) = delete;
  DevBuf(DevBuf&& o) noexcept : p_(o.p_) { o.p_ = nullptr; }
  DevBuf& operator=(DevBuf&& o) noexcept {
    if (this != &o) { reset(); p_ = o.p_; o.p_ = nullptr; }
    return *this;
  }
  ~DevBuf() { reset(); }
  hipError_t alloc(size_t bytes) { reset(); return hipMalloc(&p_, bytes); }
  void reset() {
    if (p_) (void)hipFree(p_);
    p_ = nullptr;
  }
  operator float*() const { return p_; }

 private:
  float* p_ = nullptr;
};

struct Layer {
  LayerDef def;
  std::vector<float> w, b;
  bool have_w = false, have_b = false, packed = false;
  LayerFacts facts = {};
  DevBuf direct[2];
  DevBuf d_b;
  DevBuf d_u;
  DevBuf d_ub;
  DevBuf d_w16d;
  DevBuf d_w16s;
  DevBuf d_w96;
  DevBuf d_u1;
  DevBuf d_wv;
  DevBuf d_wv16;
  DevBuf d_u24;
  DevBuf d_ub24;
  DevBuf d_u24b;
  DevBuf d_wx;
  DevBuf d_wx2;
  DevBuf d_wd;
  DevBuf d_wdw;
  DevBuf d_s2p;
  DevBuf d_s2pb;
};

int pack_layer_images(Layer& L, const std::vector<int>& chans, std::string& err);

}
```

### sketchedit_amd/csrc/se_pack.hip

```cpp
#include "se_pack.h"
#include "se_kernels.h"
#include "se_s2poly.h"

#include <cstring>

namespace se {
namespace {

template <class V>
int upload(DevBuf& dst, const std::vector<V>& host, std::string& err) {
  const size_t bytes = host.size() * sizeof(V);
  hipError_t e = dst.alloc(bytes);
  if (e == hipSuccess) e = hipMemcpy(dst, host.data(), bytes, hipMemcpyHostToDevice);
  if (e == hipSuccess) return 0;
  err = std::string("weight image upload failed: ") + hipGetErrorString(e);
  return 1;
}

unsigned short bf16_bits(float f) {
  unsigned u;
  memcpy(&u, &f, 4);
  if ((u & 0x7fffffffu) > 0x7f800000u) return (unsigned short)((u >> 16) | 0x40);
  u += 0x7fffu + ((u >> 16) & 1u);
  return (unsigned short)(u >> 16);
}
float bf16_round(float f) {
  const unsigned u = (unsigned)bf16_bits(f) << 16;
  float r;
  memcpy(&r, &u, 4);
  return r;
}

int mixed_row_channel(int n, int G) {
  const int f = n / 16 * 8 + n % 8;
  if (f >= G) return -1;
  return n % 16 < 8 ? f : G + f;
}

int out_channel_of_row(int cfg, int n, int G) {
  if (gconv_mixed(cfg)) return mixed_row_channel(n, G);
  const int NF = gconv_np(cfg) / 32;
  const int nt = n / 16, r = n % 16;
  if (nt < NF) { int f = nt * 16 + r; return f < G ? f : -1; }
  int g = (nt - NF) * 16 + r;
  return g < G ? G + g : -1;
}

std::vector<float> mixed_bias(const Layer& L, int NP) {
  std::vector<float> bias(NP);
  for (int n = 0; n < NP; ++n) bias[n] = L.b[mixed_row_channel(n, NP / 2)];
  return bias;
}

int swz(int n, int s, int e, int per = 4) { return (s ^ ((n >> 1) & 7)) * per + e; }

float subpixel_tap(const float* g, int py, int px, int a, int b) {
  float v = 0.f;
  for (int ky = a == 0 ? 0 : 1 + py; ky <= (a == 0 ? py : 2); ++ky)
    for (int kx = b == 0 ? 0 : 1 + px; kx <= (b == 0 ? px : 2); ++kx) v += g[ky * 3 + kx];
  return v;
}

void wino_f23(const float* g, int stride, float u[4]) {
  static const float Gm[4][3] = {{1.f, 0.f, 0.f}, {.5f, .5f, .5f}, {.5f, -.5f, .5f}, {0.f, 0.f, 1.f}};
  for (int nu = 0; nu < 4; ++nu) u[nu] = Gm[nu][0] * g[0] + Gm[nu][1] * g[stride] + Gm[nu][2] * g[2 * stride];
}
void wino_f22(const float* g, float U[4][4]) {
  float t[3][4];
  for (int kx = 0; kx < 3; ++kx) wino_f23(g + kx, 3, t[kx]);
  for (int xi = 0; xi < 4; ++xi) {
    const float r[3] = {t[0][xi], t[1][xi], t[2][xi]};
    wino_f23(r, 1, U[xi]);
  }
}
void winoup_class(const float* w9, int py, int px, float U[3][3]) {
  static const float Gm[3][2] = {{1.f, 0.f}, {1.f, 1.f}, {0.f, 1.f}};
  float g[2][2];
  for (int a = 0; a < 2; ++a)
    for (int b = 0; b < 2; ++b) g[a][b] = subpixel_tap(w9, py, px, a, b);
  for (int xi = 0; xi < 3; ++xi)
    for (int nu = 0; nu < 3; ++nu) {
      float u = 0.f;
      for (int a = 0; a < 2; ++a)
        for (int b = 0; b < 2; ++b) u += Gm[xi][a] * Gm[nu][b] * g[a][b];
      U[xi][nu] = u;
    }
}

template <class E> E to_elem(float v);
template <> float to_elem<float>(float v) { return v; }
template <> unsigned short to_elem<unsigned short>(float v) { return bf16_bits(v); }

template <class E>
int pack_direct(Layer& L, const std::vector<int>& cin_map, std::string& err) {
  constexpr int KC = 128 / sizeof(E), PER = 16 / sizeof(E), BF = sizeof(E) == 2;
  const LayerDef& d = L.def;
  const LayerFacts& f = L.facts;
  if (f.cfg < 0) {
    err = std::string("layer ") + d.name + ": unsupported gated width " + std::to_string(f.G);
    return 1;
  }
  const int cfg = f.cfg, G = f.G, NP = f.NP, nch = f.nch[BF];
  const int Cp = (int)cin_map.size();
  const bool up2 = d.up != 0;
  const int KW = up2 ? 2 : d.k, K = f.T * Cp, ncls = up2 ? 4 : 1;
  std::vector<E> img((size_t)ncls * nch * NP * KC, E(0));
  for (int cls = 0; cls < ncls; ++cls)
    for (int n = 0; n < NP; ++n) {
      const int oc = out_channel_of_row(cfg, n, G);
      if (oc < 0) continue;
      for (int kf = 0; kf < K; ++kf) {
        const int tap = kf / Cp, ic = cin_map[kf % Cp];
        if (ic < 0) continue;
        const int ty = tap / KW, tx = tap % KW, kin = kf % KC;
        const float* g = &L.w[((size_t)oc * d.cin + ic) * d.k * d.k];
        const float v = up2 ? subpixel_tap(g, cls >> 1, cls & 1, ty, tx) : g[ty * d.k + tx];
        img[(((size_t)cls * nch + kf / KC) * NP + n) * KC + swz(n, kin / PER, kin % PER, PER)] = to_elem<E>(v);
      }
    }
  return upload(L.direct[BF], img, err);
}

int pack_wino(Layer& L, std::string& err);
int pack_wino24(Layer& L, std::string& err);
int pack_rtilew(Layer& L, std::string& err);
int pack_wino48(Layer& L, std::string& err);
int pack_wino48_c24(Layer& L, std::string& err);
int pack_winoup(Layer& L, std::string& err);
int pack_winoup48(Layer& L, std::string& err);

int pack_layer(Layer& L, const std::vector<int>& cin_map, std::string& err) {
  const LayerDef& d = L.def;
  const LayerFacts& f = L.facts;
  if (pack_direct<float>(L, cin_map, err)) return 1;
  std::vector<float> bias(f.NP, 0.f);
  for (int n = 0; n < f.NP; ++n) {
    const int oc = out_channel_of_row(f.cfg, n, f.G);
    if (oc >= 0) bias[n] = L.b[oc];
  }
  if (upload(L.d_b, bias, err)) return 1;
  L.packed = true;
  if (f.u && d.up) return d.cin == 96 ? pack_winoup(L, err) : pack_winoup48(L, err);
  if (f.u && f.u24) return pack_wino(L, err);
  if (f.u24) return pack_wino24(L, err);
  if (f.wx) return pack_rtilew(L, err);
  if (f.u) return d.cin == 48 ? pack_wino48(L, err) : pack_wino48_c24(L, err);
  return 0;
}

int dense_kin(int j) {
  const int step = j / 4;
  return (step / 4) * 16 + (j % 4) * 4 + step % 4;
}

int pack_layer_dense(Layer& L, const std::vector<int>& cin_map, std::string& err) {
  const LayerDef& d = L.def;
  const int Cd = L.facts.dense;
  const int G = d.cout / 2, NP = 48, T = d.k * d.k, K = T * Cd, nch = L.facts.nchd;
  std::vector<float> img((size_t)nch * NP * 32, 0.f);
  for (int n = 0; n < NP; ++n) {
    const int oc = out_channel_of_row(GC_N48, n, G);
    if (oc < 0) continue;
    for (int kf = 0; kf < K; ++kf) {
      const int tap = kf / Cd, ic = cin_map[kf % Cd], ty = tap / d.k, tx = tap % d.k;
      const int kin = dense_kin(kf % 32);
      img[((size_t)(kf / 32) * NP + n) * 32 + swz(n, kin / 4, kin % 4)] = L.w[(((size_t)oc * d.cin + ic) * d.k + ty) * d.k + tx];
    }
  }
  if (upload(L.d_wd, img, err)) return 1;
  static const double Gx[6][5] = {{1. / 4, 0., 0., 0., 0.}, {-1. / 6, -1. / 6, -1. / 6, -1. / 6, -1. / 6}, {-1. / 6, 1. / 6, -1. / 6, 1. / 6, -1. / 6},
                                  {1. / 24, 1. / 12, 1. / 6, 1. / 3, 2. / 3}, {1. / 24, -1. / 12, 1. / 6, -1. / 3, 2. / 3}, {0., 0., 0., 0., 1.}};
  std::vector<float> imw((size_t)6 * NP * 32, 0.f);
  for (int n = 0; n < NP; ++n) {
    const int oc = out_channel_of_row(GC_N48, n, G);
    if (oc < 0) continue;
    for (int j = 0; j < 5 * Cd; ++j) {
      const int ky = j / Cd, ic = cin_map[j % Cd];
      const float* g = &L.w[(((size_t)oc * d.cin + ic) * 5 + ky) * 5];
      const int kin = dense_kin(j);
      for (int nu = 0; nu < 6; ++nu) {
        double u = 0.;
        for (int kx = 0; kx < 5; ++kx) u += Gx[nu][kx] * (double)g[kx];
        imw[((size_t)nu * NP + n) * 32 + swz(n, kin / 4, kin % 4)] = (float)u;
      }
    }
  }
  return upload(L.d_wdw, imw, err);
}

int pack_layer16_d4(Layer& L, const std::vector<int>& cin4, std::string& err) {
  const LayerDef& d = L.def;
  const int G = d.cout / 2, NP = 48, nch = 2;
  std::vector<unsigned short> img((size_t)nch * NP * 64, 0);
  for (int n = 0; n < NP; ++n) {
    const int oc = out_channel_of_row(GC_N48, n, G);
    if (oc < 0) continue;
    for (int ky = 0; ky < 5; ++ky)
      for (int kx = 0; kx < 5; ++kx)
        for (int cc = 0; cc < 4; ++cc) {
          const int ic = cin4[cc];
          if (ic < 0) continue;
          const int gi = 3 * ky + kx / 2, e = 4 * (kx & 1) + cc;
          img[((size_t)(gi / 8) * NP + n) * 64 + swz(n, gi % 8, e, 8)] = bf16_bits(L.w[(((size_t)oc * d.cin + ic) * 5 + ky) * 5 + kx]);
        }
  }
  return upload(L.d_w16d, img, err);
}

int pack_rconv16(Layer& L, std::string& err) {
  const LayerDef& d = L.def;
  static const int F[4] = {0, 2, 3, 1};
  std::vector<unsigned short> img((size_t)27 * 192 * 32, 0);
  for (int n = 0; n < 192; ++n) {
    const int oc = out_channel_of_row(GC_N192, n, 96);
    const int rt = n / 16, r = n % 16;
    for (int s = 0; s < 27; ++s) {
      const int tap = s / 3, kk = s % 3, ty = tap / 3, tx = tap % 3;
      for (int e = 0; e < 32; ++e) {
        const int ic = kk * 32 + e, g = e / 8;
        const float v = L.w[(((size_t)oc * d.cin + ic) * 3 + ty) * 3 + tx];
        img[((size_t)s * 12 + rt) * 512 + r * 32 + ((g ^ F[r >> 2]) * 8) + (e % 8)] = bf16_bits(v);
      }
    }
  }
  return upload(L.d_w16s, img, err);
}

int pack_rconv96(Layer& L, std::string& err) {
  const LayerDef& d = L.def;
  static const int F[4] = {0, 2, 3, 1};
  const bool up2 = d.up != 0;
  const int KW = up2 ? 2 : 3, T = KW * KW, CG = d.cin / 8, NG = T * CG, nstep = (NG + 3) / 4, ncls = up2 ? 4 : 1;
  std::vector<unsigned short> img((size_t)ncls * nstep * 96 * 32, 0);
  for (int cls = 0; cls < ncls; ++cls)
    for (int n = 0; n < 96; ++n) {
      const int oc = out_channel_of_row(GC_N96, n, 48);
      const int rt = n / 16, r = n % 16;
      for (int gi = 0; gi < NG; ++gi) {
        const int tap = gi / CG, cg = gi % CG, ty = tap / KW, tx = tap % KW, s_ = gi / 4, g = gi % 4;
        for (int e = 0; e < 8; ++e) {
          const float* w9 = &L.w[((size_t)oc * d.cin + cg * 8 + e) * 9];
          const float v = up2 ? subpixel_tap(w9, cls >> 1, cls & 1, ty, tx) : w9[ty * 3 + tx];
          img[(((size_t)cls * nstep + s_) * 6 + rt) * 512 + r * 32 + ((g ^ F[r >> 2]) * 8) + e] = bf16_bits(v);
        }
      }
    }
  return upload(L.d_w96, img, err);
}

int pack_wino(Layer& L, std::string& err) {
  const LayerDef& d = L.def;
  const int NP = 192, nch = d.cin / 32;
  std::vector<float> img((size_t)16 * nch * NP * 32, 0.f);
  for (int n = 0; n < NP; ++n) {
    const int oc = out_channel_of_row(GC_N192, n, 96);
    for (int ic = 0; ic < d.cin; ++ic) {
      float U[4][4];
      wino_f22(&L.w[((size_t)oc * d.cin + ic) * 9], U);
      for (int pos = 0; pos < 16; ++pos)
        img[(((size_t)pos * nch + ic / 32) * NP + n) * 32 + swz(n, ic % 32 / 4, ic % 4)] = U[pos >> 2][pos & 3];
    }
  }
  if (upload(L.d_u, img, err)) return 1;
  if (L.facts.u1) {
    std::vector<float> img1((size_t)16 * 3 * NP * 32), wv((size_t)9 * 96 * NP);
    for (int pos = 0; pos < 16; ++pos)
      memcpy(&img1[(size_t)pos * 3 * NP * 32], &img[(size_t)pos * nch * NP * 32], (size_t)3 * NP * 32 * 4);
    for (int n = 0; n < NP; ++n) {
      const int oc = out_channel_of_row(GC_N192, n, 96);
      for (int t = 0; t < 9; ++t)
        for (int ch = 0; ch < 96; ++ch) wv[((size_t)t * 96 + ch) * NP + n] = L.w[((size_t)oc * d.cin + 96 + ch) * 9 + t];
    }
    if (upload(L.d_u1, img1, err) || upload(L.d_wv, wv, err)) return 1;
    for (auto& v : wv) v = bf16_round(v);
    if (upload(L.d_wv16, wv, err)) return 1;
  }
  return pack_wino24(L, err);
}

int pack_rtilew(Layer& L, std::string& err) {
  const LayerDef& d = L.def;
  const int G = d.cout / 2;
  std::vector<float> img((size_t)4 * 3 * 24 * 32, 0.f), img2((size_t)16 * 24 * 32, 0.f);
  for (int prow = 0; prow < 24; ++prow) {
    const int oc = prow < 8 ? prow : prow < 16 ? G + (prow - 8) : prow < 20 ? 8 + (prow - 16) : G + 8 + (prow - 20);
    for (int ic = 0; ic < 24; ++ic) {
      const float* g = &L.w[((size_t)oc * d.cin + ic) * 9];
      for (int ky = 0; ky < 3; ++ky) {
        float u[4];
        wino_f23(g + 3 * ky, 1, u);
        const int k = ky * 24 + ic;
        for (int nu = 0; nu < 4; ++nu) img[(((size_t)nu * 3 + k / 32) * 24 + prow) * 32 + swz(prow, k % 32 / 4, k % 4)] = u[nu];
      }
      float U[4][4];
      wino_f22(g, U);
      const int s_ = ic < 16 ? ic / 4 : 4 + (ic - 16) / 2, e = ic < 16 ? ic % 4 : (ic - 16) % 2 + 2 * (((ic - 16) / 2) & 1);
      for (int pos = 0; pos < 16; ++pos) img2[((size_t)pos * 24 + prow) * 32 + swz(prow, s_, e)] = U[pos >> 2][pos & 3];
    }
  }
  if (upload(L.d_wx, img, err)) return 1;
  return upload(L.d_wx2, img2, err);
}

int pack_wino24(Layer& L, std::string& err) {
  const LayerDef& d = L.def;
  static const double Gy[4][3] = {{1., 0., 0.}, {.5, .5, .5}, {.5, -.5, .5}, {0., 0., 1.}};
  static const double Gx[6][3] = {{1. / 4, 0., 0.}, {-1. / 6, -1. / 6, -1. / 6}, {-1. / 6, 1. / 6, -1. / 6},
                                  {1. / 24, 1. / 12, 1. / 6}, {1. / 24, -1. / 12, 1. / 6}, {0., 0., 1.}};
  static const int NU[2][3] = {{0, 1, 2}, {5, 3, 4}};
  const int NP = 192;
  const int nchk_first = d.cin == 48 ? 2 : 3, nchk_last = L.facts.u24b ? 6 : nchk_first;
  for (int nchk = nchk_first; nchk <= nchk_last; nchk += 3) {
    std::vector<float> img((size_t)24 * nchk * NP * 32, 0.f);
    for (int n = 0; n < NP; ++n) {
      const int oc = mixed_row_channel(n, 96);
      for (int ic = 0; ic < nchk * 32 && ic < d.cin; ++ic) {
        const float* g = &L.w[((size_t)oc * d.cin + ic) * 9];
        double tt[4][3];
        for (int i = 0; i < 4; ++i)
          for (int kx = 0; kx < 3; ++kx) tt[i][kx] = Gy[i][0] * g[kx] + Gy[i][1] * g[3 + kx] + Gy[i][2] * g[6 + kx];
        for (int xi = 0; xi < 4; ++xi)
          for (int h = 0; h < 2; ++h)
            for (int j = 0; j < 3; ++j) {
              const int nu = NU[h][j];
              const double u = tt[xi][0] * Gx[nu][0] + tt[xi][1] * Gx[nu][1] + tt[xi][2] * Gx[nu][2];
              const int it = ((xi * 2 + h) * nchk + ic / 32) * 3 + j;
              img[((size_t)it * NP + n) * 32 + swz(n, ic % 32 / 4, ic % 4)] = (float)u;
            }
      }
    }
    if (upload(nchk <= 3 ? L.d_u24 : L.d_u24b, img, err)) return 1;
    if (nchk <= 3 && upload(L.d_ub24, mixed_bias(L, NP), err)) return 1;
  }
  return 0;
}

int pack_wino48(Layer& L, std::string& err) {
  const LayerDef& d = L.def;
  const int NP = 96;
  std::vector<float> img((size_t)24 * NP * 32, 0.f);
  for (int n = 0; n < NP; ++n) {
    const int oc = mixed_row_channel(n, 48);
    for (int ic = 0; ic < 48; ++ic) {
      float U[4][4];
      wino_f22(&L.w[((size_t)oc * d.cin + ic) * 9], U);
      for (int pos = 0; pos < 16; ++pos) {
        const int pp = pos >> 1, u6 = (pos & 1) * 3 + ic / 16;
        const int it = pp * 3 + u6 / 2, kin = (u6 % 2) * 16 + ic % 16;
        img[((size_t)it * NP + n) * 32 + swz(n, kin / 4, kin % 4)] = U[pos >> 2][pos & 3];
      }
    }
  }
  if (upload(L.d_u, img, err)) return 1;
  return upload(L.d_ub, mixed_bias(L, NP), err);
}

int pack_wino48_c24(Layer& L, std::string& err) {
  const LayerDef& d = L.def;
  const int NP = 96;
  std::vector<float> img((size_t)16 * NP * 32, 0.f);
  for (int n = 0; n < NP; ++n) {
    const int oc = mixed_row_channel(n, 48);
    for (int ic = 0; ic < 24; ++ic) {
      float U[4][4];
      wino_f22(&L.w[((size_t)oc * d.cin + ic) * 9], U);
      const int s_ = ic < 16 ? ic / 4 : 4 + (ic - 16) / 2, e = ic < 16 ? ic % 4 : (ic - 16) % 2;
      for (int pos = 0; pos < 16; ++pos) img[((size_t)pos * NP + n) * 32 + swz(n, s_, e)] = U[pos >> 2][pos & 3];
    }
  }
  if (upload(L.d_u, img, err)) return 1;
  return upload(L.d_ub, mixed_bias(L, NP), err);
}

int pack_winoup(Layer& L, std::string& err) {
  const LayerDef& d = L.def;
  const int NP = 96;
  std::vector<float> img((size_t)4 * 27 * NP * 32, 0.f);
  for (int cls = 0; cls < 4; ++cls)
    for (int n = 0; n < NP; ++n) {
      const int oc = mixed_row_channel(n, 48);
      for (int ic = 0; ic < 96; ++ic) {
        float U[3][3];
        winoup_class(&L.w[((size_t)oc * d.cin + ic) * 9], cls >> 1, cls & 1, U);
        for (int xi = 0; xi < 3; ++xi)
          for (int nu = 0; nu < 3; ++nu) {
            const int it = (xi * 3 + nu) * 3 + ic / 32, kin = ic % 32;
            img[(((size_t)cls * 27 + it) * NP + n) * 32 + swz(n, kin / 4, kin % 4)] = U[xi][nu];
          }
      }
    }
  if (upload(L.d_u, img, err)) return 1;
  return upload(L.d_ub, mixed_bias(L, NP), err);
}

int pack_winoup48(Layer& L, std::string& err) {
  const LayerDef& d = L.def;
  const int NP = 48, NIT = 14;
  std::vector<float> img((size_t)4 * NIT * NP * 32, 0.f);
  for (int cls = 0; cls < 4; ++cls)
    for (int n = 0; n < NP; ++n) {
      const int oc = mixed_row_channel(n, 24);
      for (int ic = 0; ic < 48; ++ic) {
        float U[3][3];
        winoup_class(&L.w[((size_t)oc * d.cin + ic) * 9], cls >> 1, cls & 1, U);
        for (int pos = 0; pos < 9; ++pos) {
          const int pp = pos >> 1, u6 = (pos & 1) * 3 + ic / 16;
          const int it = pp * 3 + u6 / 2, kin = (u6 % 2) * 16 + ic % 16;
          img[(((size_t)cls * NIT + it) * NP + n) * 32 + swz(n, kin / 4, kin % 4)] = U[pos / 3][pos % 3];
        }
      }
    }
  if (upload(L.d_u, img, err)) return 1;
  return upload(L.d_ub, mixed_bias(L, NP), err);
}

int pack_s2poly48(Layer& L, std::string& err) {
  const LayerDef& d = L.def;
  std::vector<float> img, bias;
  if (d.cin != 48 || (int)L.w.size() != d.cout * 48 * 9 || !s2poly_pack_host(L.w.data(), L.b.data(), d.cout, img, bias)) {
    err = std::string("layer ") + d.name + ": no polyphase image for this shape";
    return 1;
  }
  if (upload(L.d_s2p, img, err)) return 1;
  return upload(L.d_s2pb, bias, err);
}

int pack_small(Layer& L, std::string& err) {
  const LayerDef& d = L.def;
  std::vector<float> img((size_t)d.cout * 9 * 12);
  for (int oc = 0; oc < d.cout; ++oc)
    for (int t = 0; t < 9; ++t)
      for (int ic = 0; ic < 12; ++ic) img[((size_t)oc * 9 + t) * 12 + ic] = L.w[(((size_t)oc * 12 + ic) * 3 + t / 3) * 3 + t % 3];
  if (upload(L.direct[0], img, err) || upload(L.d_b, L.b, err)) return 1;
  for (auto& v : img) v = bf16_round(v);
  if (upload(L.direct[1], img, err)) return 1;
  L.packed = true;
  return 0;
}

int pack_gated(Layer& L, const std::vector<int>& chans, std::string& err) {
  const LayerFacts& f = L.facts;
  const int nc = (int)chans.size();
  auto padded = [&](int per) {
    std::vector<int> m(chans);
    m.resize((nc + per - 1) / per * per, -1);
    return m;
  };
  if (pack_direct<unsigned short>(L, padded(8), err)) return 1;
  if (f.w16d && pack_layer16_d4(L, padded(4), err)) return 1;
  if (f.w16s && pack_rconv16(L, err)) return 1;
  if (f.w96 && pack_rconv96(L, err)) return 1;
  if (f.wd && pack_layer_dense(L, chans, err)) return 1;
  if (f.s2p) {
    for (int i = 0; i < nc; ++i)
      if (chans[i] != i) { err = std::string("layer ") + L.def.name + ": the polyphase image needs its input channels in checkpoint order"; return 1; }
    if (pack_s2poly48(L, err)) return 1;
  }
  return pack_layer(L, padded(4), err);
}

}

int pack_layer_images(Layer& L, const std::vector<int>& chans, std::string& err) {
  const LayerFacts f = L.facts = layer_facts(L.def, (int)chans.size());
  if (f.small ? pack_small(L, err) : pack_gated(L, chans, err)) return 1;
  const struct { const char* name; const float* img; bool fact; } have[] = {
      {"u", L.d_u, f.u}, {"ub", L.d_ub, f.ub}, {"u1", L.d_u1, f.u1}, {"wv", L.d_wv, f.wv}, {"wv16", L.d_wv16, f.wv16},
      {"u24", L.d_u24, f.u24}, {"ub24", L.d_ub24, f.ub24}, {"u24b", L.d_u24b, f.u24b}, {"wx", L.d_wx, f.wx}, {"wx2", L.d_wx2, f.wx2},
      {"wd", L.d_wd, f.wd}, {"wdw", L.d_wdw, f.wdw}, {"w16d", L.d_w16d, f.w16d}, {"w16s", L.d_w16s, f.w16s}, {"w96", L.d_w96, f.w96},
      {"s2p", L.d_s2p, f.s2p}, {"s2pb", L.d_s2pb, f.s2p}};
  for (const auto& h : have)
    if ((h.img != nullptr) != h.fact) {
      err = std::string("layer ") + L.def.name + ": weight image " + h.name + (h.fact ? " is missing" : " was built against the layer's facts");
      return 1;
    }
  return 0;
}

}
```

### sketchedit_amd/csrc/se_plan.hip

```cpp
#include "se_host.h"

#include <numeric>

using namespace se;

namespace {

#define ENC(p)                                                                                    \
  {p "2_downsample", 24, 96, 3, 2, 1, ACT_ELU, 0}, {p "3", 48, 96, 3, 1, 1, ACT_ELU, 0},          \
      {p "4_downsample", 48, 192, 3, 2, 1, ACT_ELU, 0}, {p "5", 96, 192, 3, 1, 1, ACT_ELU, 0},    \
      {p "6", 96, 192, 3, 1, 1, ACT_ELU, 0}, {p "7_atrous", 96, 192, 3, 1, 2, ACT_ELU, 0},        \
      {p "8_atrous", 96, 192, 3, 1, 4, ACT_ELU, 0}, {p "9_atrous", 96, 192, 3, 1, 8, ACT_ELU, 0}, \
      {p "10_atrous", 96, 192, 3, 1, 16, ACT_ELU, 0}
#define DEC(p, c11in, c17out)                                                                        \
  {p "11", c11in, 192, 3, 1, 1, ACT_ELU, 0}, {p "12", 96, 192, 3, 1, 1, ACT_ELU, 0},                 \
      {p "13_upsample_conv", 96, 96, 3, 1, 1, ACT_ELU, 1}, {p "14", 48, 96, 3, 1, 1, ACT_ELU, 0},    \
      {p "15_upsample_conv", 48, 48, 3, 1, 1, ACT_ELU, 1}, {p "16", 24, 24, 3, 1, 1, ACT_ELU, 0},    \
      {p "17", 12, c17out, 3, 1, 1, ACT_NONE, 0}

}

namespace se {

const LayerDef G_LAYERS[] = {
    {"conv1", 5, 48, 5, 1, 1, ACT_ELU, 0}, ENC("conv"), DEC("conv", 192, 3),
    {"wconv1", 5, 48, 5, 1, 1, ACT_ELU, 0}, ENC("wconv"),
    {"xconv1", 3, 48, 5, 1, 1, ACT_ELU, 0},
    {"xconv2_downsample", 24, 48, 3, 2, 1, ACT_ELU, 0}, {"xconv3", 24, 96, 3, 1, 1, ACT_ELU, 0},
    {"xconv4_downsample", 48, 96, 3, 2, 1, ACT_ELU, 0}, {"xconv5", 48, 192, 3, 1, 1, ACT_ELU, 0},
    {"xconv6", 96, 192, 3, 1, 1, ACT_ELU, 0}, {"xconv7_atrous", 96, 192, 3, 1, 2, ACT_ELU, 0},
    {"xconv8_atrous", 96, 192, 3, 1, 4, ACT_ELU, 0}, {"xconv9_atrous", 96, 192, 3, 1, 8, ACT_ELU, 0},
    {"xconv10_atrous", 96, 192, 3, 1, 16, ACT_ELU, 0},
    {"pmconv1", 3, 48, 5, 1, 1, ACT_ELU, 0},
    {"pmconv2_downsample", 24, 48, 3, 2, 1, ACT_ELU, 0}, {"pmconv3", 24, 96, 3, 1, 1, ACT_ELU, 0},
    {"pmconv4_downsample", 48, 192, 3, 2, 1, ACT_ELU, 0}, {"pmconv5", 96, 192, 3, 1, 1, ACT_ELU, 0},
    {"pmconv6", 96, 192, 3, 1, 1, ACT_RELU, 0}, {"pmconv9", 96, 192, 3, 1, 1, ACT_ELU, 0},
    {"pmconv10", 96, 192, 3, 1, 1, ACT_ELU, 0},
    DEC("allconv", 192, 3),
};
const LayerDef M_LAYERS[] = {
    {"conv1", 4, 48, 5, 1, 1, ACT_ELU, 0}, ENC("conv"), DEC("conv", 96, 3), DEC("conv_mask_", 96, 1),
};
const int NG = sizeof(G_LAYERS) / sizeof(LayerDef), NM = sizeof(M_LAYERS) / sizeof(LayerDef);

}

namespace {

struct ConvLaunch {
  se_ctx* c;
  const Layer& L; const LayerDef& d; const LayerFacts& f;
  const float* src0; int C0; const float* src1; int C1, src1_vec; float* dst;
  int B, Hin, Win, Ho, Wo, pad;
  bool bf;
  double alg(int taps) const { return 2.0 * (double)B * Ho * Wo * d.cout * d.cin * taps; }

  WinoParams wino_params(const float* upk, const float* bias, int dil, int tcols) const {
    WinoParams wp;
    memset(&wp, 0, sizeof wp);
    wp.src = src0; wp.upk = upk; wp.bias = bias; wp.dst = dst;
    wp.B = B; wp.h = Hin; wp.w = Win; wp.d = dil; wp.th = Hin / 2; wp.tw = Win / tcols;
    wp.total_tiles = B * wp.th * wp.tw; wp.act = d.act;
    wp.xcd = xcd_remap_enabled();
    udiv_magic_host((unsigned)(wp.th * wp.tw), &wp.div_tpi_m, &wp.div_tpi_l);
    udiv_magic_host((unsigned)wp.tw, &wp.div_tw_m, &wp.div_tw_l);
    udiv_magic_host((unsigned)wp.d, &wp.div_d_m, &wp.div_d_l);
    return wp;
  }
  int launch_form_wino(const Choice& ch) const {
    const double alg3x3 = alg(9);
    if (ch.form == F_WINO24_C48) {
      const WinoParams wp = wino_params(L.d_u24, L.d_ub24, d.rate, 4);
      set_launch_cost(alg3x3, 4.0 * ((double)B * Hin * Win * 48 + (double)B * Hin * Win * 96), d.name, alg3x3 * 24.0 / 72.0);
      HIPCHK(c, launch_wino24_c48(wp, c->st));
      return 0;
    }
    const bool folded = ch.fold, f43 = ch.form == F_WINO24;
    if (folded) HIPCHK(c, launch_vecbias(L.d_wv, src1, c->vbias_ws, B, 96, c->st));
    const float* s1 = folded ? nullptr : src1;
    WinoParams wp = f43 ? wino_params(s1 ? L.d_u24b : L.d_u24, L.d_ub24, d.rate, 4) : wino_params(folded ? L.d_u1 : L.d_u, L.d_b, d.rate, 2);
    wp.src1 = s1; wp.src1_vec = folded ? 0 : src1_vec; wp.vbias = folded ? c->vbias_ws : nullptr;
    if ((double)B * Hin * Win * 384.0 >= 2147483648.0) return fail(c, "layer %s: tensor exceeds 2^31 bytes", d.name);
    set_launch_cost(alg3x3, 4.0 * 2.0 * (double)B * Hin * Win * 96, d.name,
                    f43 ? alg3x3 * 24.0 / 72.0 * (folded ? 0.5 : 1.0) : alg3x3 * 16.0 / 36.0 * (folded ? 0.5 : 1.0));
    HIPCHK(c, f43 ? launch_wino24(wp, c->st) : launch_wino(wp, c->st));
    return 0;
  }
  int launch_form_wino48(const Choice& ch) const {
    const WinoParams wp = wino_params(L.d_u, L.d_ub, d.rate, 2);
    const bool c24 = ch.form == F_WINO48_C24;
    set_launch_cost(alg(9), c24 ? 4.0 * ((double)B * Hin * Win * 24 + (double)B * Hin * Win * 48) : 4.0 * 2.0 * (double)B * Hin * Win * 48, d.name,
                    alg(9) * 16.0 / 36.0);
    HIPCHK(c, c24 ? launch_wino48_c24(wp, c->st) : launch_wino48(wp, c->st));
    return 0;
  }
  int launch_form_s2poly(const Choice&) const {
    const int halves = d.cout / 96;
    WinoParams wp = wino_params(L.d_s2p, L.d_s2pb, 1, 2);
    wp.th = Hin / 4; wp.tw = Win / 4; wp.total_tiles = B * wp.th * wp.tw;
    udiv_magic_host((unsigned)(wp.th * wp.tw), &wp.div_tpi_m, &wp.div_tpi_l);
    udiv_magic_host((unsigned)wp.tw, &wp.div_tw_m, &wp.div_tw_l);
    set_launch_cost(alg(9), 4.0 * ((double)halves * B * Hin * Win * 48 + (double)B * Ho * Wo * (d.cout / 2)), d.name, alg(9) * 25.0 / 36.0);
    HIPCHK(c, launch_s2poly48(wp, halves, c->st));
    return 0;
  }
  int launch_form_winoup(const Choice& ch) const {
    const WinoParams wp = wino_params(L.d_u, L.d_ub, 1, 2);
    if (ch.form == F_WINOUP) {
      set_launch_cost(alg(9), 4.0 * ((double)B * Hin * Win * 96 + (double)B * Ho * Wo * 48), d.name, alg(9) * 9.0 / 36.0);
      HIPCHK(c, launch_winoup(wp, c->st));
      return 0;
    }
    set_launch_cost(alg(9), 4.0 * ((double)B * Hin * Win * 48 + (double)B * Ho * Wo * 24), d.name, alg(9) * 9.0 / 36.0 * 28.0 / 27.0);
    HIPCHK(c, launch_winoup48(wp, c->st));
    return 0;
  }

  RTileParams rtile_params(const float* wpk, int trows) const {
    RTileParams p;
    memset(&p, 0, sizeof p);
    p.src = src0; p.wpk = wpk; p.bias = L.d_b; p.dst = dst;
    p.B = B; p.Hin = Hin; p.Win = Win; p.C = C0; p.OH = Ho; p.OW = Wo;
    p.G = bf ? (f.G + 7) & ~7 : f.G; p.NP = f.NP;
    p.ty = (Hin + trows - 1) / trows; p.tx = (Win + 15) / 16;
    p.act = d.act; p.bf16 = bf ? 1 : 0; p.xcd = xcd_remap_enabled();
    return p;
  }
  int launch_form_rtilew(const Choice& ch) const {
    const bool two_d = ch.form == F_RTILEW2;
    RTileParams p = rtile_params(two_d ? L.d_wx2 : L.d_wx, 16);
    udiv_magic_host((unsigned)(p.ty * p.tx), &p.div_cg_m, &p.div_cg_l);
    udiv_magic_host((unsigned)p.tx, &p.div_rw_m, &p.div_rw_l);
    set_launch_cost(alg(9), 4.0 * ((double)B * Hin * Win * d.cin + (double)B * Ho * Wo * (d.cout / 2)), d.name,
                    (double)B * p.ty * p.tx * 8.0 * (two_d ? 96.0 : 160.0) * 2048.0);
    HIPCHK(c, two_d ? launch_rtilew2(p, c->st) : launch_rtilew(p, c->st));
    return 0;
  }
  int launch_form_rtile_dense5(const Choice& ch) const {
    const bool along_x = ch.form == F_RTILE_DENSE5W;
    const long long per_img = (long long)Hin * Win * C0 * 4;
    const long long lim = addr_limit();
    const int bmax = (int)std::max<long long>(1, (lim - 1) / per_img);
    for (int b0 = 0; b0 < B; b0 += bmax) {
      const int nb = std::min(bmax, B - b0);
      RTileParams p = rtile_params(along_x ? L.d_wdw : L.d_wd, 8);
      p.src = src0 + (size_t)b0 * Hin * Win * C0; p.dst = dst + (size_t)b0 * Ho * Wo * f.G; p.B = nb;
      p.dense = along_x ? f.dense + 100 : f.dense; p.nch = f.nchd;
      const double algn = 2.0 * (double)nb * Ho * Wo * d.cout * d.cin * 25;
      set_launch_cost(algn, 4.0 * ((double)nb * Hin * Win * d.cin + (double)nb * Ho * Wo * (d.cout / 2)), d.name,
                      along_x ? (double)nb * p.ty * p.tx * 4.0 * (6.0 * ((5 * f.dense + 3) / 4) * 3.0) * 2048.0
                              : 2.0 * (double)nb * Hin * Win * 48.0 * (4.0 * ((25 * f.dense + 3) / 4)));
      HIPCHK(c, launch_rtile(p, c->st));
    }
    return 0;
  }
  int launch_form_rtile(const Choice& ch) const {
    const int es = bf ? 2 : 4, TR = rtile_rows(bf);
    RTileParams p = rtile_params(ch.form == F_RTILE_D4 ? L.d_w16d : L.direct[bf], TR);
    p.pad = pad;
    if (ch.form == F_RTILE_D4) {
      p.CG = 1; p.T = 25; p.KW = 5; p.nch = 2; p.dense = 204;
      p.RH = 32 + 4; p.RW = 21;
      p.raw_bytes = (p.RH * p.RW * 8 + 1023) & ~1023;
      udiv_magic_host(1u, &p.div_cg_m, &p.div_cg_l);
      set_launch_cost(alg(25), 2.0 * ((double)B * Hin * Win * d.cin + (double)B * Ho * Wo * (d.cout / 2)), d.name, 2.0 * (double)B * Hin * Win * 48.0 * 128.0);
    } else {
      const int KW = d.up ? 2 : d.k, CG = f.CG[bf], nch = f.nch[bf];
      p.CG = CG; p.T = f.T; p.KW = KW; p.nch = nch; p.up2 = d.up ? 1 : 0;
      p.RH = TR + KW - 1; p.RW = 16 + KW - 1;
      p.raw_bytes = (p.RH * p.RW * C0 * es + 1023) & ~1023;
      p.magicCG = (65536 + CG - 1) / CG; p.magicKW = 256 / KW + 1;
      udiv_magic_host((unsigned)(C0 * es / 16), &p.div_cg_m, &p.div_cg_l);
      set_launch_cost(alg(d.k * d.k), (double)es * ((double)B * Hin * Win * d.cin + (double)B * Ho * Wo * (d.cout / 2)), d.name,
                      2.0 * (double)B * Hin * Win * (d.up ? 4.0 : 1.0) * f.NP * (nch * (bf ? 64.0 : 32.0)));
    }
    udiv_magic_host((unsigned)p.RW, &p.div_rw_m, &p.div_rw_l);
    HIPCHK(c, launch_rtile(p, c->st));
    return 0;
  }

  int launch_form_rconv16(const Choice& ch) const {
    if (ch.fold) HIPCHK(c, launch_vecbias(L.d_wv16, c->vec32, c->vbias_ws, B, 96, c->st, 1));
    RConvParams rp;
    memset(&rp, 0, sizeof rp);
    rp.dual = ch.form == F_RCONV16_DUAL;
    rp.src = src0; rp.wpk = L.d_w16s; rp.bias = L.d_b; rp.dst = dst; rp.vbias = ch.fold ? c->vbias_ws : nullptr;
    rp.B = B; rp.h = Hin; rp.w = Win; rp.d = d.rate; rp.hs = Hin / d.rate; rp.ws = Win / d.rate;
    rp.ty = (rp.hs + 7) / 8; rp.tx = (rp.ws + 15) / 16;
    rp.act = d.act; rp.xcd = xcd_remap_enabled();
    set_launch_cost(alg(9), 2.0 * 2.0 * (double)B * Hin * Win * 96, d.name, 2.0 * (double)B * Hin * Win * 192.0 * 864.0);
    HIPCHK(c, launch_rconv16(rp, c->st));
    return 0;
  }
  int launch_form_rconv96(const Choice&) const {
    RConv96Params rp;
    memset(&rp, 0, sizeof rp);
    rp.src = src0; rp.wpk = L.d_w96; rp.bias = L.d_b; rp.dst = dst;
    rp.B = B; rp.h = Hin; rp.w = Win; rp.CG = C0 / 8;
    rp.stride = d.stride; rp.oh = Ho; rp.ow = Wo;
    rp.ty = ((d.stride == 2 ? Ho : Hin) + 15) / 16; rp.tx = ((d.stride == 2 ? Wo : Win) + 15) / 16;
    rp.up2 = d.up ? 1 : 0; rp.act = d.act; rp.xcd = xcd_remap_enabled();
    const int T = d.up ? 4 : 9, nstep = (T * rp.CG + 3) / 4;
    set_launch_cost(alg(9), 2.0 * ((double)B * Hin * Win * d.cin + (double)B * Ho * Wo * 48), d.name,
                    2.0 * (double)B * (d.stride == 2 ? (double)Ho * Wo : (double)Hin * Win) * (d.up ? 4.0 : 1.0) * 96.0 * (nstep * 32.0));
    HIPCHK(c, launch_rconv96(rp, c->st));
    return 0;
  }

  int launch_form_gather(const Choice&) const {
    const int es = bf ? 2 : 4, gran = bf ? 8 : 4, CG = f.CG[bf], nch = f.nch[bf], KW = d.up ? 2 : d.k;
    GConvParams p;
    memset(&p, 0, sizeof p);
    p.bf16 = bf ? 1 : 0;
    p.src0 = src0; p.src1 = src1 ? src1 : src0; p.wpk = L.direct[bf]; p.bias = L.d_b; p.dst = dst; p.zeros = c->zeros;
    p.B = B; p.Hin = Hin; p.Win = Win; p.Ho = d.up ? Hin : Ho; p.Wo = d.up ? Win : Wo;
    p.up2 = d.up ? 1 : 0; p.OH = Ho; p.OW = Wo;
    p.C0 = C0; p.C1 = C1 ? C1 : C0; p.C0g = C0 / gran; p.CG = CG;
    p.T = f.T; p.KW = KW; p.stride = d.stride; p.dil = d.rate; p.pad = pad;
    p.magicCG = (65536 + CG - 1) / CG; p.magicKW = 256 / KW + 1; p.magicKH = f.T / KW;
    if (!magic_cg_ok(CG, nch)) return fail(c, "layer %s: magic division check failed", d.name);
    if (!magic_kw_ok(KW, f.T)) return fail(c, "layer %s: magic tap division check failed", d.name);
    const int Gs = bf ? (f.G + 7) & ~7 : f.G;
    if ((double)B * Hin * Win * (C0 > C1 ? C0 : C1) * es >= 2147483648.0 || (double)B * Ho * Wo * Gs * es >= 2147483648.0)
      return fail(c, "layer %s: a tensor of this launch exceeds 2^31 bytes (32-bit byte offsets) -- split the batch", d.name);
    for (int j = 0; j < p.magicKH; ++j) p.rep |= 1u << (j * KW);
    udiv_magic_host((unsigned)(p.Ho * p.Wo), &p.div_hw_m, &p.div_hw_l);
    udiv_magic_host((unsigned)p.Wo, &p.div_w_m, &p.div_w_l);
    p.Hlim = Hin; p.Wlim = Win;
    p.src1_vec = src1_vec; p.nch = nch; p.G = Gs; p.act = d.act; p.total_pix = B * p.Ho * p.Wo;
    p.xcd = xcd_remap_enabled();
    p.np_full = f.NP; p.nf_full = f.NP / 32; p.small_grid = c->low_latency ? 1 : 0;
    set_launch_cost(alg(d.k * d.k), (double)es * ((double)B * Hin * Win * d.cin + (double)B * Ho * Wo * (d.cout / 2)), d.name,
                    2.0 * (double)B * p.Ho * p.Wo * (d.up ? 4.0 : 1.0) * f.NP * (nch * (bf ? 64.0 : 32.0)));
    HIPCHK(c, launch_gconv(f.cfg, p, c->st));
    return 0;
  }
};

}

namespace se {

int run_gconv(se_ctx* c, const Layer& L, const float* src0, int C0, const float* src1, int C1, int src1_vec, float* dst,
              int B, int Hin, int Win) {
  const LayerDef& d = L.def;
  const LayerFacts& f = L.facts;
  const ConvShape sh = conv_shape(d, Hin, Win);
  const bool bf = c->bf16;
  if (!L.packed) return fail(c, "layer %s: weights not loaded", d.name);
  if (bf && !L.direct[1]) return fail(c, "layer %s: no bf16 weight image", d.name);
  if (bf && (C0 + C1) != f.CG[1] * 8) return fail(c, "layer %s: bf16 source channels %d+%d != packed %d", d.name, C0, C1, f.CG[1] * 8);
  if (!bf && (C0 + C1) != f.CG[0] * 4) return fail(c, "layer %s: source channels %d+%d != packed %d", d.name, C0, C1, f.CG[0] * 4);
  const ConvCall q = {d, f, B, Hin, Win, C0, C1, src1 ? (src1_vec ? SRC2_VECTOR : SRC2_TENSOR) : SRC2_NONE, bf, c->low_latency,
                      c->conservative, c->cur_net, c->vbias_ws && (!bf || c->vec32)};
  const Choice ch = choose_form(q);
  static bool said = false;
  if (ch.wino_range && !said) {
    said = true;
    fprintf(stderr, "sketchedit_hip: layer %s: %d x %dx%d x 96 floats exceed the Winograd kernel's 32-bit byte offsets; "
                    "using the direct kernel (about 2x slower) -- split the batch\n", d.name, B, Hin, Win);
  }
  const ConvLaunch a = {c, L, d, f, src0, C0, src1, C1, src1_vec, dst, B, Hin, Win, sh.Ho, sh.Wo, sh.pad, bf};
  switch (ch.form) {
    case F_WINO: case F_WINO24: case F_WINO24_C48: return a.launch_form_wino(ch);
    case F_WINO48: case F_WINO48_C24: return a.launch_form_wino48(ch);
    case F_WINOUP: case F_WINOUP48: return a.launch_form_winoup(ch);
    case F_RTILEW: case F_RTILEW2: return a.launch_form_rtilew(ch);
    case F_RTILE_DENSE5: case F_RTILE_DENSE5W: return a.launch_form_rtile_dense5(ch);
    case F_RTILE: case F_RTILE_D4: return a.launch_form_rtile(ch);
    case F_RCONV16: case F_RCONV16_DUAL: return a.launch_form_rconv16(ch);
    case F_RCONV96: return a.launch_form_rconv96(ch);
    case F_S2POLY48: return a.launch_form_s2poly(ch);
    case F_GATHER: return a.launch_form_gather(ch);
    case F_SMALL_CONV: break;
  }
  return fail(c, "layer %s: not a gated conv", d.name);
}

}

namespace {

Act encoder(Plan& P, const std::string& p, Act& in, Act* keep9, Layer* first = nullptr) {
  Act x = first ? P.conv_layer(*first, in) : P.conv((p + "1").c_str(), in);
  x = P.conv((p + "2_downsample").c_str(), x);
  x = P.conv((p + "3").c_str(), x);
  x = P.conv((p + "4_downsample").c_str(), x);
  x = P.conv((p + "5").c_str(), x);
  x = P.conv((p + "6").c_str(), x);
  x = P.conv((p + "7_atrous").c_str(), x);
  x = P.conv((p + "8_atrous").c_str(), x);
  Act x9 = P.conv((p + "9_atrous").c_str(), x);
  Act x10 = P.conv((p + "10_atrous").c_str(), x9, keep9 == nullptr);
  if (keep9) *keep9 = x9;
  return x10;
}

Act decoder(Plan& P, const std::string& p, Act& in, const float* src1 = nullptr, int C1 = 0, int vec = 0) {
  Act x = P.conv((p + "11").c_str(), in, true, src1, C1, vec);
  x = P.conv((p + "12").c_str(), x);
  x = P.conv((p + "13_upsample_conv").c_str(), x);
  x = P.conv((p + "14").c_str(), x);
  x = P.conv((p + "15_upsample_conv").c_str(), x);
  x = P.conv((p + "16").c_str(), x);
  return x;
}

int small(Plan& P, const char* name, Act& in, int mode, float* out_nchw, float* hard, const float* img,
          const float* mask, float* xnow, float* composed, int no_mask_coarse, long packed_bs = 0,
          const unsigned char* lock = nullptr) {
  if (P.rc) return P.rc;
  se_ctx* c = P.c;
  if (!c->dry) {
    Layer& L = P.net.at(name);
    if (!L.packed) return P.rc = fail(c, "layer %s: weights not loaded", name);
    SmallConvParams sp;
    memset(&sp, 0, sizeof sp);
    sp.x = in.p; sp.w = L.direct[c->bf16]; sp.b = L.d_b; sp.B = P.B; sp.H = in.H; sp.W = in.W; sp.cout = L.def.cout;
    sp.bf16 = c->bf16 ? 1 : 0;
    sp.mode = mode; sp.out_nchw = out_nchw; sp.hard = hard; sp.img = img; sp.mask = mask; sp.xnow = xnow;
    sp.composed = composed; sp.no_mask_coarse = no_mask_coarse;
    if (mode == 3) { sp.rgb8 = c->rgb8; sp.m8 = c->m8; }
    if (mode == 0) sp.lock = lock;
    if (packed_bs) {
      if (mode == 0) sp.out_bs = packed_bs;
      if (mode == 3) { sp.mask_bs = packed_bs; sp.comp_bs = packed_bs; }
    }
    set_launch_cost(2.0 * (double)P.B * in.H * in.W * L.def.cout * 108.0,
                    4.0 * (double)P.B * in.H * in.W * (12 + L.def.cout), L.def.name);
    hipError_t e = launch_small_conv(sp, c->st);
    if (e != hipSuccess) return P.rc = fail(c, "small conv %s: %s", name, hipGetErrorString(e));
  }
  P.free(in);
  return 0;
}

}

namespace se {

int plan_netM(se_ctx* c, const float* image, const float* sketch, float* mask_out, float* hard_out, float* maskim_out,
              int B, int H, int W, long packed_bs, const unsigned char* lock) {
  Plan P(c, c->M, B);
  c->cur_net = SE_NET_M;
  Act in = P.alloc(H, W, 4);
  if (P.rc) return P.rc;
  if (!c->dry) HIPCHK(c, c->bf16 ? launch_pack_m16(image, sketch, in.p, B, H, W, c->st) : launch_pack_m(image, sketch, in.p, B, H, W, c->st));
  Act x9;
  const bool want_img = maskim_out != nullptr;
  Act x10 = encoder(P, "conv", in, want_img ? &x9 : nullptr);
  if (want_img) {
    Act d = decoder(P, "conv", x9);
    small(P, "conv17", d, 1, maskim_out, nullptr, nullptr, nullptr, nullptr, nullptr, 0);
  }
  Act d = decoder(P, "conv_mask_", x10);
  small(P, "conv_mask_17", d, 0, mask_out, hard_out, nullptr, nullptr, nullptr, nullptr, 0, packed_bs, lock);
  return P.rc;
}

int plan_netG(se_ctx* c, const float* x, const float* x2, const float* mask, const float* mask2, const float* guide,
              float* coarse_out, float* fine_out, const float* soft_mask, float* composed_out, int B, int H, int W,
              int flags, long packed_bs) {
  Plan P(c, c->G, B);
  c->cur_net = SE_NET_G;
  const int joint = (flags & SE_FLAG_JOINT_TRAIN_INP) ? 1 : 0;
  Act cin = P.alloc(H, W, 8);
  P.ar = P.forked() ? &c->arena2 : P.home();
  Act sin = P.alloc(H, W, joint ? 4 : 8);
  P.ar = P.home();
  if (P.rc) return P.rc;
  if (!c->dry)
    HIPCHK(c, (c->bf16 ? launch_pack_g16 : launch_pack_g)(x, x2, mask, mask2, guide, cin.p, sin.p, B, H, W,
                                                          (flags & SE_FLAG_NO_MASK_CC) ? 1 : 0, joint, c->st));
  if (P.side_begin()) return 1;
  Act xs = encoder(P, "wconv", sin, nullptr, joint ? &c->wconv1_j4 : nullptr);
  Act part = P.alloc(1, COLREDUCE_SPLITS, 192), vec32 = P.alloc(1, 1, 192), vec = P.alloc(1, 1, 96);
  if (P.rc) return P.rc;
  if (!c->dry)
    HIPCHK(c, launch_colreduce(xs.p, part.p, c->bf16 ? vec32.p : vec.p, B, xs.H * xs.W, 96, (flags & SE_FLAG_POOL_MAX) ? 0 : 1,
                               c->st, c->bf16 ? 1 : 0, c->bf16 ? vec.p : nullptr));
  if (!c->dry && c->taps && c->taps->style_vec)
    HIPCHK(c, hipMemcpyAsync(c->taps->style_vec, c->bf16 ? vec32.p : vec.p, (size_t)B * 96 * 4, hipMemcpyDeviceToDevice, c->st));
  P.free(xs);
  P.free(part);
  if (!c->bf16) P.free(vec32);
  if (P.side_end()) return 1;
  Act xc = encoder(P, "conv", cin, nullptr);
  if (P.rc) return P.rc;
  if (P.join()) return 1;
  float* vb = P.alloc_raw((size_t)B * 9 * 192);
  if (P.rc) return P.rc;
  c->vbias_ws = vb;
  c->vec32 = c->bf16 ? vec32.p : nullptr;
  Act d = decoder(P, "conv", xc, vec.p, 96, 1);
  c->vbias_ws = nullptr; c->vec32 = nullptr;
  P.release(vb);
  if (c->bf16) P.free(vec32);
  P.free(vec);
  Act xnow = P.alloc(H, W, 4);
  if (P.rc) return P.rc;
  small(P, "conv17", d, 2, coarse_out, nullptr, x, mask, xnow.p, nullptr, (flags & SE_FLAG_NO_MASK_COARSE) ? 1 : 0);
  if (P.rc) return P.rc;
  if (P.side_begin()) return 1;
  Act pm = P.conv("pmconv1", xnow, false);
  pm = P.conv("pmconv2_downsample", pm);
  pm = P.conv("pmconv3", pm);
  pm = P.conv("pmconv4_downsample", pm);
  pm = P.conv("pmconv5", pm);
  pm = P.conv("pmconv6", pm);
  if (P.rc) return P.rc;
  if (!c->dry && c->taps && c->taps->pmconv6)
    HIPCHK(c, (c->bf16 ? launch_nhwc16_to_nchw : launch_nhwc_to_nchw)(pm.p, c->taps->pmconv6, B, 96, 96, pm.H, pm.W, c->st));
  if (flags & SE_FLAG_USE_CAM) {
    Act att = P.alloc(pm.H, pm.W, 96);
    if (P.rc) return P.rc;
    if (run_attention(c, P, pm, mask, att, nullptr)) return P.rc ? P.rc : 1;
    P.free(pm);
    pm = att;
    if (!c->dry && c->taps && c->taps->attn_out)
      HIPCHK(c, (c->bf16 ? launch_nhwc16_to_nchw : launch_nhwc_to_nchw)(pm.p, c->taps->attn_out, B, 96, 96, pm.H, pm.W, c->st));
  }
  pm = P.conv("pmconv9", pm);
  pm = P.conv("pmconv10", pm);
  if (P.rc) return P.rc;
  if (P.side_end()) return 1;
  Act hcur = P.conv("xconv1", xnow, false);
  hcur = P.conv("xconv2_downsample", hcur);
  hcur = P.conv("xconv3", hcur);
  hcur = P.conv("xconv4_downsample", hcur);
  hcur = P.conv("xconv5", hcur);
  hcur = P.conv("xconv6", hcur);
  hcur = P.conv("xconv7_atrous", hcur);
  hcur = P.conv("xconv8_atrous", hcur);
  hcur = P.conv("xconv9_atrous", hcur);
  Act hallu = P.conv("xconv10_atrous", hcur);
  if (P.rc) return P.rc;
  if (P.join()) return 1;
  P.free(xnow);
  Act d2 = decoder(P, "allconv", hallu, pm.p, 96, 0);
  P.free(pm);
  small(P, "allconv17", d2, 3, fine_out, nullptr, x, soft_mask, nullptr, soft_mask ? composed_out : nullptr, 0, packed_bs);
  c->rgb8 = nullptr; c->m8 = nullptr;
  return P.rc;
}

int att_row_stride(int R, bool bf) {
  const int chunk = bf ? 64 : 32;
  int Rp = (R + chunk - 1) / chunk * chunk;
  return Rp;
}

bool att_streaming(int h, int w, bool bf, bool want_similar) {
  const int R = (h / 2) * (w / 2), Rp = att_row_stride(R, bf);
  const bool fits = (double)R * Rp * 4.0 < 2147483648.0;
  if (want_similar && !fits) return true;
  if (opt(OPT_ATT_STREAM) == 1 && !want_similar) return true;
  return !fits;
}

int run_attention(se_ctx* c, Plan& P, Act& x, const float* mask_full, Act& out, float* similar_nchw) {
  const int h = x.H, w = x.W, B = P.B;
  const int hs = (h - 4) / 2 + 1, ws = (w - 4) / 2 + 1, L = hs * ws, Lp = (L + 31) & ~31;
  const bool bf = c->bf16;
  const bool stream = att_streaming(h, w, bf, similar_nchw != nullptr);
  const int hc = h / 2, wc = w / 2, R = hc * wc;
  const int Rp = att_row_stride(R, bf);
  const int guard = (wc + 8 + 63) & ~63;
  if (stream && similar_nchw)
    return P.rc = fail(c, "attention: similar_out (the %d x %d score matrix) is not available on a %dx%d feature map: "
                          "it runs in the streaming form, which never forms it", L, L, h, w);
  float* part = P.alloc_raw((size_t)B * COLREDUCE_SPLITS * 96);
  float* rn = P.alloc_raw((size_t)B * 96);
  float* xn = P.alloc_raw(bf ? ((size_t)B * h * w * 96 + 1) / 2 : (size_t)B * h * w * 96);
  float *valid = nullptr, *S = nullptr, *S2 = nullptr, *xT = nullptr, *stats = nullptr;
  if (stream) {
    valid = P.alloc_raw(3 * (size_t)B * Rp);
    stats = P.alloc_raw((size_t)B * R * 2);
    xT = P.alloc_raw((bf ? (size_t)B * 4 * 96 * Rp / 2 : (size_t)B * 4 * 96 * Rp) + att_stream_xt_tail());
  } else {
    valid = P.alloc_raw(7 * ((size_t)B * Rp + guard) + (size_t)B * 768 + (size_t)B * hc * 384);
    stats = P.alloc_raw((size_t)B * R * 2);
    xT = P.alloc_raw(bf ? (size_t)B * 4 * 96 * Rp / 2 : (size_t)B * 4 * 96 * Rp);
    S = P.alloc_raw((size_t)B * R * Rp + 2 * guard);
    S2 = P.alloc_raw(bf ? (size_t)B * R * Rp / 2 : (size_t)B * R * Rp);
  }
  if (P.rc) return P.rc;
  if (!c->dry) {
    HIPCHK(c, launch_colreduce(x.p, part, rn, B, h * w, 96, 2, c->st, bf ? 1 : 0));
    AttParams a;
    memset(&a, 0, sizeof a);
    a.x = x.p; a.rn = rn; a.xn = xn; a.hard = mask_full; a.out = out.p;
    a.B = B; a.h = h; a.w = w; a.hs = hs; a.ws = ws; a.L = L; a.Lp = Lp;
    a.scale = 10.f; a.th = 0.1f;
    if (stream) {
      a.hc = hc; a.wc = wc; a.R = R; a.Rp = Rp; a.bf16 = bf ? 1 : 0;
      a.validR = valid; a.kmul = valid + (size_t)B * Rp; a.kadd = valid + 2 * (size_t)B * Rp;
      a.xT = xT; a.stats = stats;
      HIPCHK(c, launch_attention_stream(a, c->st));
    } else {
      a.hc = hc; a.wc = wc; a.R = R; a.Rp = Rp; a.bf16 = bf ? 1 : 0;
      a.validR = valid + guard; a.xT = xT; a.E = S + guard; a.P = S2; a.stats = stats; a.guard = guard; a.similar = similar_nchw;
      a.kmul = valid + ((size_t)B * Rp + guard) + guard; a.kadd = valid + 2 * ((size_t)B * Rp + guard) + guard;
      a.kadd2 = valid + 3 * ((size_t)B * Rp + guard) + guard; a.ea4 = valid + 4 * ((size_t)B * Rp + guard) + guard;
      a.ea = valid + 5 * ((size_t)B * Rp + guard) + guard; a.eb = valid + 6 * ((size_t)B * Rp + guard) + guard;
      a.emean = valid + 7 * ((size_t)B * Rp + guard); a.epart = a.emean + (size_t)B * 768;
      HIPCHK(c, launch_attention(a, c->st));
    }
  }
  P.release(S2); P.release(S); P.release(xT); P.release(stats); P.release(valid);
  P.release(xn); P.release(rn); P.release(part);
  return 0;
}

}

namespace {

long long max_act_bytes_per_image(se_ctx* c, int H, int W, int flags) {
  const std::vector<long long> key = {H, W, (flags & SE_FLAG_BF16) ? 1 : 0};
  auto it = c->act_per_img.find(key);
  if (it != c->act_per_img.end()) return it->second;
  const bool dry0 = c->dry, ll0 = c->low_latency, bf0 = c->bf16, pair0 = c->paired;
  c->dry = true; c->low_latency = false; c->bf16 = (flags & SE_FLAG_BF16) != 0; c->paired = false;
  c->dry_max_act = 0;
  float dummy;
  c->arena.reset(nullptr, 0, true, 0); c->arena2.reset(nullptr, 0, true, 1);
  plan_netM(c, nullptr, nullptr, nullptr, nullptr, &dummy, 1, H, W, 0);
  c->arena.reset(nullptr, 0, true, 0); c->arena2.reset(nullptr, 0, true, 1);
  plan_netG(c, nullptr, nullptr, nullptr, nullptr, nullptr, nullptr, nullptr, nullptr, nullptr, 1, H, W, SE_FLAG_USE_CAM | SE_FLAG_POOL_MAX, 0);
  c->dry = dry0; c->low_latency = ll0; c->bf16 = bf0; c->paired = pair0;
  const long long v = (long long)c->dry_max_act;
  c->act_per_img[key] = v;
  return v;
}

}

namespace se {

int pass_size(se_ctx* c, int B, int H, int W, int flags) {
  const long long per_img = max_act_bytes_per_image(c, H, W, flags);
  const long long lim = addr_limit();
  if (per_img <= 0) { fail(c, "internal: no activation size for %dx%d", H, W); return 0; }
  if (per_img >= lim) {
    fail(c, "a %dx%d image exceeds the kernels' 32-bit byte offsets (%lld bytes per activation, limit %lld)", H, W, per_img, lim);
    return 0;
  }
  const long long bmax = (lim - 1) / per_img;
  if (B <= bmax) return B;
  const long long passes = (B + bmax - 1) / bmax;
  return (int)((B + passes - 1) / passes);
}

se_ctx::Peaks plan_peaks(se_ctx* c, int which, int B, int H, int W, int flags, bool want_maskim, bool pair) {
  const std::vector<long long> key = {which, B, H, W,
                                      flags & (SE_FLAG_USE_CAM | SE_FLAG_JOINT_TRAIN_INP | SE_FLAG_LOW_LATENCY | SE_FLAG_BF16),
                                      want_maskim ? 1 : 0, c->fork2 ? 1 : 0, opt_epoch(), c->serial ? 1 : 0, pair ? 1 : 0};
  auto it = c->peaks.find(key);
  if (it != c->peaks.end()) return it->second;
  const bool dry0 = c->dry, ll0 = c->low_latency, bf0 = c->bf16, pair0 = c->paired;
  const int half0 = c->half;
  c->dry = true;
  c->low_latency = (flags & SE_FLAG_LOW_LATENCY) != 0;
  c->bf16 = (flags & SE_FLAG_BF16) != 0;
  float dummy;
  se_ctx::Peaks pk{0, 0};
  for (int half = 0; half < (pair ? 2 : 1); ++half) {
    const int nb = !pair ? B : half ? B - pair_first(B) : pair_first(B);
    c->paired = pair; c->half = half;
    if (which & 1) {
      c->arena.reset(nullptr, 0, true, 0); c->arena2.reset(nullptr, 0, true, 1);
      plan_netM(c, nullptr, nullptr, nullptr, nullptr, want_maskim ? &dummy : nullptr, nb, H, W);
      if (c->arena.peak > pk.main) pk.main = c->arena.peak;
      if (c->arena2.peak > pk.side) pk.side = c->arena2.peak;
    }
// ... 38 lines not shown
```

### sketchedit_amd/kernel_labels.py

```python

KERNEL_LABELS = {
    "wino_kernel": "wino_n192", "wino24_kernel": "wino_n192", "rconv16": "gconv_n192", "gconv_kernel<12": "gconv_n192",
    "wino48_kernel": "wino_n96", "rconv96": "gconv_n96", "gconv_kernel<6": "gconv_n96",
    "s2poly48_kernel": "wino_n96",
    "winoup_kernel": "wino_up96",
    "winoup48_kernel": "gconv_n48", "rtile_dense5w_kernel": "gconv_n48", "rtile_dense5_kernel": "gconv_n48",
    "rtile_kernel<3": "gconv_n48", "gconv_kernel<3": "gconv_n48",
    "rtilew2_kernel": "gconv_n24", "rtilew_kernel": "gconv_n24", "rtile_kernel<2": "gconv_n24", "gconv_kernel<2": "gconv_n24",
    "dtail_kernel": "dtail",
    "att2_pair_kernel": "att_score", "att2_pv_kernel": "att_pv",
    "att2_softmax": "att_softmax", "att2_stats": "att_softmax",
    "att2_boxsum": "att_boxsum", "att2_ptilde": "att_boxsum",
    "att2_prep": "att_prep", "att2_transpose": "att_prep", "att2_emean": "att_prep", "att2_eoff": "att_prep",
    "att2_similar": "layout",
    "small_conv_kernel": "small_conv", "pack_": "pack", "colreduce": "colreduce", "vecbias_kernel": "colreduce",
    "nchw_to_nhwc": "layout", "nhwc_to_nchw": "layout", "nhwc16_to_nchw": "layout", "quantize_u8_kernel": "layout",
    "dequant_u8_kernel": "layout",
    "(anonymous namespace)::window_resample_h_kernel": "window_resample_h", "(anonymous namespace)::window_paste_v_kernel": "window_paste_v",
    "window_resample_h_kernel": "window_resample_h", "window_paste_v_kernel": "window_paste_v",
    "(anonymous namespace)::resample_h_kernel": "resize_h", "(anonymous namespace)::resample_v_kernel": "resize_v",
    "resample_h_kernel": "resize_h", "resample_v_kernel": "resize_v",
    "(anonymous namespace)::window_gather_kernel": "window_gather", "(anonymous namespace)::window_border_kernel": "window_border",
    "(anonymous namespace)::window_paste_kernel": "window_paste",
    "window_gather_kernel": "window_gather", "window_border_kernel": "window_border", "window_paste_kernel": "window_paste",
    "(anonymous namespace)::window_paste_feather_kernel": "window_paste_feather", "window_paste_feather_kernel": "window_paste_feather",
    "(anonymous namespace)::fill_masks_kernel": "fill_masks", "(anonymous namespace)::fill_keep_kernel": "fill_keep",
    "fill_masks_kernel": "fill_masks", "fill_keep_kernel": "fill_keep",
    "(anonymous namespace)::select_similar_kernel": "select_similar", "(anonymous namespace)::select_flood_kernel": "select_flood",
    "(anonymous namespace)::select_grow_kernel": "select_grow",
    "select_similar_kernel": "select_similar", "select_flood_kernel": "select_flood", "select_grow_kernel": "select_grow",
    "(anonymous namespace)::modify_disc_kernel": "modify_disc", "(anonymous namespace)::modify_vote_kernel": "modify_vote",
    "modify_disc_kernel": "modify_disc", "modify_vote_kernel": "modify_vote",
    "(anonymous namespace)::lasso_fill_kernel": "lasso_fill", "(anonymous namespace)::plane_combine_kernel": "plane_combine",
    "lasso_fill_kernel": "lasso_fill", "plane_combine_kernel": "plane_combine",
    "(anonymous namespace)::outline_tile_kernel<false>": "outline_count", "(anonymous namespace)::outline_tile_kernel<true>": "outline_emit",
    "(anonymous namespace)::outline_scan_kernel": "outline_scan",
    "outline_tile_kernel<false>": "outline_count", "outline_tile_kernel<true>": "outline_emit", "outline_scan_kernel": "outline_scan",
    "(anonymous namespace)::move_drop_kernel<false>": "move_drop", "(anonymous namespace)::move_drop_kernel<true>": "move_drop",
    "(anonymous namespace)::plane_shift_kernel": "plane_shift",
    "move_drop_kernel<false>": "move_drop", "move_drop_kernel<true>": "move_drop", "plane_shift_kernel": "plane_shift",
    "(anonymous namespace)::blend_init_kernel": "blend_init", "(anonymous namespace)::blend_pull_kernel": "blend_pull",
    "(anonymous namespace)::blend_relax_kernel": "blend_relax", "(anonymous namespace)::blend_apply_kernel": "blend_apply",
    "blend_init_kernel": "blend_init", "blend_pull_kernel": "blend_pull", "blend_relax_kernel": "blend_relax",
    "blend_apply_kernel": "blend_apply",
    "(anonymous namespace)::canvas_map_kernel": "canvas_map", "(anonymous namespace)::canvas_turn_kernel": "canvas_turn",
    "canvas_map_kernel": "canvas_map", "canvas_turn_kernel": "canvas_turn",
    "(anonymous namespace)::warp_drop_kernel": "warp_drop", "(anonymous namespace)::plane_warp_kernel": "plane_warp",
    "warp_drop_kernel": "warp_drop", "plane_warp_kernel": "plane_warp",
    "(anonymous namespace)::filter_blur_kernel<8>": "filter_blur", "(anonymous namespace)::filter_blur_kernel<16>": "filter_blur",
    "(anonymous namespace)::filter_blur_kernel<32>": "filter_blur", "(anonymous namespace)::filter_mosaic_kernel": "filter_mosaic",
    "filter_blur_kernel<8>": "filter_blur", "filter_blur_kernel<16>": "filter_blur", "filter_blur_kernel<32>": "filter_blur",
    "filter_mosaic_kernel": "filter_mosaic",
    "(anonymous namespace)::adjust_kernel": "adjust", "(anonymous namespace)::hist_tiles_kernel": "hist_tiles",
    "(anonymous namespace)::hist_sum_kernel": "hist_sum", "(anonymous namespace)::adjust_lut_kernel": "adjust_lut",
    "adjust_kernel": "adjust", "hist_tiles_kernel": "hist_tiles", "hist_sum_kernel": "hist_sum", "adjust_lut_kernel": "adjust_lut",
    "(anonymous namespace)::window_save_kernel": "window_save", "(anonymous namespace)::window_swap_kernel": "window_swap",
    "window_save_kernel": "window_save", "window_swap_kernel": "window_swap",
    "(anonymous namespace)::sketch_tiles_kernel": "sketch_tiles", "sketch_tiles_kernel": "sketch_tiles",
    "(anonymous namespace)::sketch_strokes_kernel": "sketch_strokes", "sketch_strokes_kernel": "sketch_strokes",
    "(anonymous namespace)::png_rows_kernel": "png_rows", "(anonymous namespace)::png_stripe_kernel": "png_stripes",
    "(anonymous namespace)::png_finish_kernel": "png_finish",
    "png_rows_kernel": "png_rows", "png_stripe_kernel": "png_stripes", "png_finish_kernel": "png_finish",
    "(anonymous namespace)::jpg_blocks_kernel": "jpg_blocks", "(anonymous namespace)::jpg_rows_kernel": "jpg_rows",
    "(anonymous namespace)::jpg_finish_kernel": "jpg_finish",
    "jpg_blocks_kernel": "jpg_blocks", "jpg_rows_kernel": "jpg_rows", "jpg_finish_kernel": "jpg_finish",
    "(anonymous namespace)::jpg2_blocks420_kernel": "jpg2_blocks420", "(anonymous namespace)::jpg2_hist_kernel": "jpg2_hist",
    "(anonymous namespace)::jpg2_tables_kernel": "jpg2_tables", "(anonymous namespace)::jpg2_rows_kernel": "jpg2_rows",
    "jpg2_blocks420_kernel": "jpg2_blocks420", "jpg2_hist_kernel": "jpg2_hist", "jpg2_tables_kernel": "jpg2_tables",
    "jpg2_rows_kernel": "jpg2_rows",
}


def kernel_key(name):
    return name.split("(")[0].replace("void se::", "").replace("se::", "")


def label_of(name):
    k = kernel_key(name)
    return next((v for pre, v in KERNEL_LABELS.items() if k.startswith(pre)), None)
```

Measured before the change: 3058 images/sec.

## Add merged polyphase MFMA kernel for stride-2 24-to-96 gated convolutions

Adds an s2poly24 form for 3x3 stride-2 gated convolutions with 24 input and 96 output channels. The weights are repacked into merged polyphase groups, so each 4x4 input tile produces a 2x2 output block with shared accumulators that fold into several outputs. The kernel uses MFMA, a three-stage LDS pipeline and the gating fused into the epilogue. It replaces the generic rtile path for these layers, and it needs an extra packed weight image and a large amount of complex unrolled code.

```diff
diff --git a/sketchedit_amd/_lib.py b/sketchedit_amd/_lib.py
--- a/sketchedit_amd/_lib.py
+++ b/sketchedit_amd/_lib.py
@@ -9,7 +9,7 @@
 _HERE = os.path.dirname(os.path.abspath(__file__))
 LIB_PATH = os.environ.get("SKETCHEDIT_HIP_LIB") or os.path.join(_HERE, "lib", "libsketchedit_hip.so")
 CSRC = os.path.join(_HERE, "csrc")
-SOURCES = ["se_gconv.hip", "se_rconv16.hip", "se_rconv96.hip", "se_rtile.hip", "se_rtilew.hip", "se_wino.hip", "se_wino24.hip", "se_wino48.hip", "se_wino_up.hip", "se_wino_up48.hip", "se_s2poly.hip", "se_attention.hip", "se_att_stream.hip", "se_misc.hip", "se_resize.hip",
+SOURCES = ["se_gconv.hip", "se_rconv16.hip", "se_rconv96.hip", "se_rtile.hip", "se_rtilew.hip", "se_wino.hip", "se_wino24.hip", "se_wino48.hip", "se_wino_up.hip", "se_wino_up48.hip", "se_s2poly.hip", "se_s2poly24.hip", "se_attention.hip", "se_att_stream.hip", "se_misc.hip", "se_resize.hip",
            "se_window.hip", "se_feather.hip", "se_fill.hip", "se_select.hip", "se_lasso.hip", "se_modify.hip", "se_outline.hip", "se_move.hip", "se_blend.hip", "se_canvas.hip", "se_warp.hip", "se_filter.hip", "se_adjust.hip", "se_png.hip", "se_jpg.hip", "se_pack.hip",
            "se_plan.hip", "se_api_window.hip", "se_api_select.hip", "se_api_move.hip", "se_api_codec.hip", "se_api_debug.hip", "se_api.hip"]
 
@@ -391,6 +391,32 @@
     return f[:n].reshape(cout // 96, 38, 96, 32).copy(), f[n:].copy()
 
 
+def s2poly24_groups():
+    return np.array([[get_option("SE_S2POLY24_GROUP:%d,%d" % (g, j)) for j in range(10)] for g in range(9)], np.int32)
+
+
+def s2poly24_khalves():
+    return np.array([[get_option("SE_S2POLY24_KHALF:%d,%d" % (kh, j)) for j in range(5)] for kh in range(38)], np.int32)
+
+
+def s2poly24_probe_layer(cout=96):
+    p = lambda n: (((7919 * n) % 2053 - 1026) / 1024.0).astype(np.float32)
+    return p(np.arange(cout * 24 * 9, dtype=np.int64)).reshape(cout, 24, 3, 3), p(10007 + np.arange(cout, dtype=np.int64))
+
+
+def s2poly24_probe_pack(cout=96):
+    fn = load_library().se_debug_get_option
+    n = 19 * cout * 32
+    out = np.zeros(n + cout, np.int32)
+    v = ctypes.c_int(0)
+    for i in range(n + cout):
+        if fn(("SE_S2POLY24_PACK:%d,%d" % (cout, i)).encode(), ctypes.byref(v)):
+            raise SketchEditHipError("SE_S2POLY24_PACK: cout must be 96")
+        out[i] = v.value
+    f = out.view(np.float32)
+    return f[:n].reshape(19, cout, 32).copy(), f[n:].copy()
+
+
 def pair_rule(B, H, W, low_latency=False):
     v = ctypes.c_int(-1)
     name = "SE_PAIR_RULE:%d,%d,%d,%d" % (B, H, W, FLAG_LOW_LATENCY if low_latency else 0)
diff --git a/sketchedit_amd/csrc/se_api_debug.hip b/sketchedit_amd/csrc/se_api_debug.hip
--- a/sketchedit_amd/csrc/se_api_debug.hip
+++ b/sketchedit_amd/csrc/se_api_debug.hip
@@ -1,5 +1,6 @@
 #include "se_host.h"
 #include "se_s2poly.h"
+#include "se_s2poly24.h"
 
 using namespace se;
 
@@ -106,6 +107,40 @@
       for (size_t n = 0; n < w.size(); ++n) w[n] = probe((long long)n);
       for (int n = 0; n < cout; ++n) b[n] = probe(10007 + n);
       if (!s2poly_pack_host(w.data(), b.data(), cout, all, bias)) return 1;
+      all.insert(all.end(), bias.begin(), bias.end());
+    }
+    if ((size_t)i >= all.size()) return 1;
+    memcpy(value, &all[(size_t)i], sizeof(int));
+    return 0;
+  }
+  static const char qg[] = "SE_S2POLY24_GROUP:", qk[] = "SE_S2POLY24_KHALF:", qq[] = "SE_S2POLY24_PACK:";
+  if (name && value && !strncmp(name, qg, sizeof qg - 1)) {
+    int g = -1, j = -1, end = 0;
+    if (sscanf(name + sizeof qg - 1, "%d,%d%n", &g, &j, &end) != 2 || name[sizeof qg - 1 + end] || g < 0 || g >= S2POLY24_NGRP || j < 0 || j > 9) return 1;
+    if (j == 0) *value = s2poly24_mult(g);
+    else if (j == 1) *value = (s2poly24_feeds(g, 0, 0) ? 1 : 0) | (s2poly24_feeds(g, 0, 1) ? 2 : 0) | (s2poly24_feeds(g, 1, 0) ? 4 : 0) | (s2poly24_feeds(g, 1, 1) ? 8 : 0);
+    else *value = (j & 1) ? s2poly24_sign(g, (j - 2) / 2) : s2poly24_pos(g, (j - 2) / 2);
+    return 0;
+  }
+  if (name && value && !strncmp(name, qk, sizeof qk - 1)) {
+    int kh = -1, j = -1, end = 0;
+    if (sscanf(name + sizeof qk - 1, "%d,%d%n", &kh, &j, &end) != 2 || name[sizeof qk - 1 + end] || kh < 0 || kh >= S2POLY24_NKH || j < 0 || j > 4) return 1;
+    *value = j == 0 ? s2poly24_kh_group(kh) : j == 1 ? s2poly24_kh_lo(kh) : j < 4 ? s2poly24_kh_hi(kh, j - 2) : s2poly24_kh_steps(kh);
+    return 0;
+  }
+  if (name && value && !strncmp(name, qq, sizeof qq - 1)) {
+    int cout = 0, end = 0;
+    long long i = -1;
+    if (sscanf(name + sizeof qq - 1, "%d,%lld%n", &cout, &i, &end) != 2 || name[sizeof qq - 1 + end] || cout != 96 || i < 0) return 1;
+    static std::mutex mu;
+    static std::vector<float> all;
+    std::lock_guard<std::mutex> lk(mu);
+    if (all.empty()) {
+      auto probe = [](long long n) { return (float)((7919 * n) % 2053 - 1026) / 1024.f; };
+      std::vector<float> w((size_t)cout * 24 * 9), b(cout), bias;
+      for (size_t n = 0; n < w.size(); ++n) w[n] = probe((long long)n);
+      for (int n = 0; n < cout; ++n) b[n] = probe(10007 + n);
+      if (!s2poly24_pack_host(w.data(), b.data(), cout, all, bias)) return 1;
       all.insert(all.end(), bias.begin(), bias.end());
     }
     if ((size_t)i >= all.size()) return 1;
diff --git a/sketchedit_amd/csrc/se_dispatch.h b/sketchedit_amd/csrc/se_dispatch.h
--- a/sketchedit_amd/csrc/se_dispatch.h
+++ b/sketchedit_amd/csrc/se_dispatch.h
@@ -42,6 +42,7 @@
   int dense, nchd;
   bool u, ub, u1, wv, wv16, u24, ub24, u24b, wx, wx2, wd, wdw, w16d, w16s, w96;
   bool s2p;
+  bool s2p24;
 };
 
 inline LayerFacts layer_facts(const LayerDef& d, int nchans) {
@@ -68,6 +69,7 @@
   f.w16s = d.k == 3 && d.stride == 1 && !d.up && (d.cin == 96 || d.cin == 192) && d.cout == 192;
   f.w96 = rconv96_eligible(d);
   f.s2p = d.k == 3 && d.stride == 2 && d.rate == 1 && !d.up && nchans == 48 && d.cin == 48 && (d.cout == 96 || d.cout == 192);
+  f.s2p24 = d.k == 3 && d.stride == 2 && d.rate == 1 && !d.up && nchans == 24 && d.cin == 24 && d.cout == 96;
   if (d.k != 3 || d.stride != 1 || (nchans + 3) / 4 * 4 != d.cin) return f;
   if (d.up) {
     f.u = f.ub = (d.cin == 96 && d.cout == 96) || (d.cin == 48 && d.cout == 48);
@@ -96,7 +98,7 @@
 
 enum Form {
   F_SMALL_CONV, F_WINO, F_WINO24, F_WINO24_C48, F_WINO48, F_WINO48_C24, F_WINOUP, F_WINOUP48, F_RTILEW, F_RTILEW2,
-  F_RTILE_DENSE5, F_RTILE_DENSE5W, F_RTILE_D4, F_RTILE, F_RCONV16, F_RCONV16_DUAL, F_RCONV96, F_S2POLY48, F_GATHER
+  F_RTILE_DENSE5, F_RTILE_DENSE5W, F_RTILE_D4, F_RTILE, F_RCONV16, F_RCONV16_DUAL, F_RCONV96, F_S2POLY48, F_S2POLY24, F_GATHER
 };
 struct Choice {
   Form form;
@@ -207,6 +209,11 @@
   if ((s2_mode == 1 || (s2_mode == 2 && q.net == 0)) && !ll && f.s2p && !two && d.k == 3 && d.stride == 2 && d.rate == 1 && !d.up && C0 == 48 &&
       d.cin == 48 && (d.cout == 96 || d.cout == 192) && (Hin % 4) == 0 && (Win % 4) == 0 && fits48)
     return is(F_S2POLY48);
+  const int s24_mode = opt(OPT_S2_POLY24);
+  const long wg24 = ((long)(Hin / 4) * (Win / 4) + 63) / 64;
+  if (wg24 >= opt(OPT_S2_POLY24_MIN_WG) && (s24_mode == 1 || (s24_mode == 2 && q.net == 0)) && !ll && f.s2p24 && !two && d.k == 3 && d.stride == 2 && d.rate == 1 && !d.up && C0 == 24 &&
+      d.cin == 24 && d.cout == 96 && (Hin % 4) == 0 && (Win % 4) == 0 && fits48)
+    return is(F_S2POLY24);
   return is(choose_rtile(q));
 }
 
@@ -241,6 +248,7 @@
     case F_RCONV16: return "rconv16";
     case F_RCONV16_DUAL: return "rconv16_dual";
     case F_S2POLY48: return "s2poly48";
+    case F_S2POLY24: return "s2poly24";
     case F_RCONV96: return d.up ? "rconv96_up" : d.stride == 2 ? "rconv96_s2" : q.C0 == 24 ? "rconv96_c24" : "rconv96";
     case F_GATHER: return gconv_form_name(q.facts.cfg, q.low_latency, d.up != 0, q.C0 / (q.bf16 ? 8 : 4) != q.facts.CG[q.bf16], q.bf16);
   }
diff --git a/sketchedit_amd/csrc/se_kernels.h b/sketchedit_amd/csrc/se_kernels.h
--- a/sketchedit_amd/csrc/se_kernels.h
+++ b/sketchedit_amd/csrc/se_kernels.h
@@ -45,6 +45,8 @@
   X(WINOGRAD, 1) X(WINOGRAD48, 1) X(WINOGRAD_UP, 1) X(WINOGRAD_UP48, 1)                                         \
   X(WINOGRAD_F43, 1)      \
   X(S2_POLY, 1)           \
+  X(S2_POLY24, 1)         \
+  X(S2_POLY24_MIN_WG, 16)  \
   X(GCONV_FAST, 1) X(FORK_DEFAULT, 1) X(LL_WINO_MIN_WG, 64) X(LL_WINO48_MIN_WG, 128)                            \
   X(ATT_FUSED, -1) X(ATT_FUSED_BF16, -1) X(ATT_PTILDE_LDS, 1) X(ATT_STATS_LDS, 1) X(ATT_E16, 1) X(ATT_SYM, 1)   \
   X(ATT_STREAM, 0)        \
@@ -132,6 +134,7 @@
 hipError_t launch_winoup(const WinoParams& p, hipStream_t st);
 hipError_t launch_winoup48(const WinoParams& p, hipStream_t st);
 hipError_t launch_s2poly48(const WinoParams& p, int halves, hipStream_t st);
+hipError_t launch_s2poly24(const WinoParams& p, hipStream_t st);
 
 struct RConvParams {
   const void* src;
diff --git a/sketchedit_amd/csrc/se_pack.h b/sketchedit_amd/csrc/se_pack.h
--- a/sketchedit_amd/csrc/se_pack.h
+++ b/sketchedit_amd/csrc/se_pack.h
@@ -55,6 +55,8 @@
   DevBuf d_wdw;
   DevBuf d_s2p;
   DevBuf d_s2pb;
+  DevBuf d_s2q;
+  DevBuf d_s2qb;
 };
 
 int pack_layer_images(Layer& L, const std::vector<int>& chans, std::string& err);
diff --git a/sketchedit_amd/csrc/se_pack.hip b/sketchedit_amd/csrc/se_pack.hip
--- a/sketchedit_amd/csrc/se_pack.hip
+++ b/sketchedit_amd/csrc/se_pack.hip
@@ -1,6 +1,7 @@
 #include "se_pack.h"
 #include "se_kernels.h"
 #include "se_s2poly.h"
+#include "se_s2poly24.h"
 
 #include <cstring>
 
@@ -425,6 +426,17 @@
   return upload(L.d_s2pb, bias, err);
 }
 
+int pack_s2poly24(Layer& L, std::string& err) {
+  const LayerDef& d = L.def;
+  std::vector<float> img, bias;
+  if (d.cin != 24 || d.cout != 96 || (int)L.w.size() != 96 * 24 * 9 || !s2poly24_pack_host(L.w.data(), L.b.data(), d.cout, img, bias)) {
+    err = std::string("layer ") + d.name + ": no merged polyphase image for this shape";
+    return 1;
+  }
+  if (upload(L.d_s2q, img, err)) return 1;
+  return upload(L.d_s2qb, bias, err);
+}
+
 int pack_small(Layer& L, std::string& err) {
   const LayerDef& d = L.def;
   std::vector<float> img((size_t)d.cout * 9 * 12);
@@ -456,6 +468,11 @@
       if (chans[i] != i) { err = std::string("layer ") + L.def.name + ": the polyphase image needs its input channels in checkpoint order"; return 1; }
     if (pack_s2poly48(L, err)) return 1;
   }
+  if (f.s2p24) {
+    for (int i = 0; i < nc; ++i)
+      if (chans[i] != i) { err = std::string("layer ") + L.def.name + ": the merged polyphase image needs its input channels in checkpoint order"; return 1; }
+    if (pack_s2poly24(L, err)) return 1;
+  }
   return pack_layer(L, padded(4), err);
 }
 
@@ -468,7 +485,7 @@
       {"u", L.d_u, f.u}, {"ub", L.d_ub, f.ub}, {"u1", L.d_u1, f.u1}, {"wv", L.d_wv, f.wv}, {"wv16", L.d_wv16, f.wv16},
       {"u24", L.d_u24, f.u24}, {"ub24", L.d_ub24, f.ub24}, {"u24b", L.d_u24b, f.u24b}, {"wx", L.d_wx, f.wx}, {"wx2", L.d_wx2, f.wx2},
       {"wd", L.d_wd, f.wd}, {"wdw", L.d_wdw, f.wdw}, {"w16d", L.d_w16d, f.w16d}, {"w16s", L.d_w16s, f.w16s}, {"w96", L.d_w96, f.w96},
-      {"s2p", L.d_s2p, f.s2p}, {"s2pb", L.d_s2pb, f.s2p}};
+      {"s2p", L.d_s2p, f.s2p}, {"s2pb", L.d_s2pb, f.s2p}, {"s2q", L.d_s2q, f.s2p24}, {"s2qb", L.d_s2qb, f.s2p24}};
   for (const auto& h : have)
     if ((h.img != nullptr) != h.fact) {
       err = std::string("layer ") + L.def.name + ": weight image " + h.name + (h.fact ? " is missing" : " was built against the layer's facts");
diff --git a/sketchedit_amd/csrc/se_plan.hip b/sketchedit_amd/csrc/se_plan.hip
--- a/sketchedit_amd/csrc/se_plan.hip
+++ b/sketchedit_amd/csrc/se_plan.hip
@@ -102,6 +102,15 @@
     udiv_magic_host((unsigned)wp.tw, &wp.div_tw_m, &wp.div_tw_l);
     set_launch_cost(alg(9), 4.0 * ((double)halves * B * Hin * Win * 48 + (double)B * Ho * Wo * (d.cout / 2)), d.name, alg(9) * 25.0 / 36.0);
     HIPCHK(c, launch_s2poly48(wp, halves, c->st));
+    return 0;
+  }
+  int launch_form_s2poly24(const Choice&) const {
+    WinoParams wp = wino_params(L.d_s2q, L.d_s2qb, 1, 2);
+    wp.th = Hin / 4; wp.tw = Win / 4; wp.total_tiles = B * wp.th * wp.tw;
+    udiv_magic_host((unsigned)(wp.th * wp.tw), &wp.div_tpi_m, &wp.div_tpi_l);
+    udiv_magic_host((unsigned)wp.tw, &wp.div_tw_m, &wp.div_tw_l);
+    set_launch_cost(alg(9), 4.0 * ((double)B * Hin * Win * 24 + (double)B * Ho * Wo * 48), d.name, alg(9) * 25.0 / 36.0);
+    HIPCHK(c, launch_s2poly24(wp, c->st));
     return 0;
   }
   int launch_form_winoup(const Choice& ch) const {
@@ -271,6 +280,7 @@
     case F_RCONV16: case F_RCONV16_DUAL: return a.launch_form_rconv16(ch);
     case F_RCONV96: return a.launch_form_rconv96(ch);
     case F_S2POLY48: return a.launch_form_s2poly(ch);
+    case F_S2POLY24: return a.launch_form_s2poly24(ch);
     case F_GATHER: return a.launch_form_gather(ch);
     case F_SMALL_CONV: break;
   }
diff --git a/sketchedit_amd/csrc/se_s2poly24.h b/sketchedit_amd/csrc/se_s2poly24.h
--- /dev/null
+++ b/sketchedit_amd/csrc/se_s2poly24.h
@@ -0,0 +1,114 @@
+#pragma once
+#include "se_s2poly.h"
+
+namespace se {
+
+constexpr int S2POLY24_NGRP = 9;
+constexpr int S2POLY24_NIT = 19;
+constexpr int S2POLY24_NKH = 38;
+
+__host__ __device__ constexpr int s2poly24_grp1(int q) { return s2poly_fold(q, 0) != 0 ? (s2poly_fold(q, 1) != 0 ? 1 : 0) : 2; }
+__host__ __device__ constexpr int s2poly24_sign1(int q) { return s2poly_fold(q, 0) != 0 ? s2poly_fold(q, 0) : s2poly_fold(q, 1); }
+__host__ __device__ constexpr bool s2poly24_signs_ok() {
+  for (int q = 0; q < 5; ++q)
+    if (s2poly_fold(q, 0) != 0 && s2poly_fold(q, 1) != 0 && s2poly_fold(q, 0) != s2poly_fold(q, 1)) return false;
+  return true;
+}
+static_assert(s2poly24_signs_ok(), "a 1-D position folds into both outputs with different signs");
+__host__ __device__ constexpr int s2poly24_mult1(int g) {
+  int n = 0;
+  for (int q = 0; q < 5; ++q) n += s2poly24_grp1(q) == g;
+  return n;
+}
+__host__ __device__ constexpr int s2poly24_member1(int g, int j) {
+  for (int q = 0; q < 5; ++q)
+    if (s2poly24_grp1(q) == g && j-- == 0) return q;
+  return -1;
+}
+__host__ __device__ constexpr bool s2poly24_feeds1(int g, int o) { return g == 1 || g == 2 * o; }
+
+__host__ __device__ constexpr int s2poly24_mult(int g) { return s2poly24_mult1(g / 3) * s2poly24_mult1(g % 3); }
+__host__ __device__ constexpr int s2poly24_pos(int g, int j) {
+  if (j < 0 || j >= s2poly24_mult(g)) return -1;
+  const int mx = s2poly24_mult1(g % 3);
+  return 5 * s2poly24_member1(g / 3, j / mx) + s2poly24_member1(g % 3, j % mx);
+}
+__host__ __device__ constexpr int s2poly24_sign(int g, int j) {
+  const int pos = s2poly24_pos(g, j);
+  return pos < 0 ? 0 : s2poly24_sign1(pos / 5) * s2poly24_sign1(pos % 5);
+}
+__host__ __device__ constexpr bool s2poly24_feeds(int g, int a, int b) { return s2poly24_feeds1(g / 3, a) && s2poly24_feeds1(g % 3, b); }
+__host__ __device__ constexpr int s2poly24_nfeeds(int g) {
+  return (int)s2poly24_feeds(g, 0, 0) + (int)s2poly24_feeds(g, 0, 1) + (int)s2poly24_feeds(g, 1, 0) + (int)s2poly24_feeds(g, 1, 1);
+}
+
+__host__ __device__ constexpr int s2poly24_order(int i) {
+  constexpr int order[S2POLY24_NGRP] = {0, 1, 3, 2, 6, 5, 7, 8, 4};
+  return order[i];
+}
+__host__ __device__ constexpr int s2poly24_group_khs(int g) { return s2poly24_mult(g) + (s2poly24_mult(g) + 1) / 2; }
+__host__ __device__ constexpr int s2poly24_kh_group(int kh) {
+  for (int i = 0, at = 0; i < S2POLY24_NGRP; ++i) {
+    const int n = s2poly24_group_khs(s2poly24_order(i));
+    if (kh >= at && kh < at + n) return s2poly24_order(i);
+    at += n;
+  }
+  return -1;
+}
+__host__ __device__ constexpr int s2poly24_kh_local(int kh) {
+  for (int i = 0, at = 0; i < S2POLY24_NGRP; ++i) {
+    const int n = s2poly24_group_khs(s2poly24_order(i));
+    if (kh >= at && kh < at + n) return kh - at;
+    at += n;
+  }
+  return -1;
+}
+__host__ __device__ constexpr int s2poly24_total_khs() {
+  int n = 0;
+  for (int g = 0; g < S2POLY24_NGRP; ++g) n += s2poly24_group_khs(g);
+  return n;
+}
+static_assert(s2poly24_total_khs() == S2POLY24_NKH && S2POLY24_NKH == 2 * S2POLY24_NIT, "the K order fills 19 iterations");
+__host__ __device__ constexpr int s2poly24_kh_lo(int kh) {
+  const int g = s2poly24_kh_group(kh), l = s2poly24_kh_local(kh);
+  return g >= 0 && l < s2poly24_mult(g) ? l : -1;
+}
+__host__ __device__ constexpr int s2poly24_kh_hi(int kh, int which) {
+  const int g = s2poly24_kh_group(kh), l = s2poly24_kh_local(kh);
+  if (g < 0 || l < s2poly24_mult(g)) return -1;
+  const int j = 2 * (l - s2poly24_mult(g)) + which;
+  return j < s2poly24_mult(g) ? j : -1;
+}
+__host__ __device__ constexpr int s2poly24_kh_steps(int kh) { return s2poly24_kh_lo(kh) < 0 && s2poly24_kh_hi(kh, 1) < 0 ? 2 : 4; }
+__host__ __device__ constexpr int s2poly24_k_member(int kh, int k) {
+  return s2poly24_kh_lo(kh) >= 0 ? s2poly24_kh_lo(kh) : s2poly24_kh_hi(kh, (k % 4) / 2);
+}
+__host__ __device__ constexpr int s2poly24_k_channel(int kh, int k) { return s2poly24_kh_lo(kh) >= 0 ? k : 16 + 2 * (k / 4) + k % 2; }
+
+inline bool s2poly24_pack_host(const float* w, const float* b, int cout, std::vector<float>& img, std::vector<float>& bias) {
+  if (cout != 96) return false;
+  const int NP = cout, G = cout / 2;
+  img.assign((size_t)S2POLY24_NIT * NP * 32, 0.f);
+  bias.assign((size_t)NP, 0.f);
+  for (int n = 0; n < NP; ++n) {
+    const int f = n / 16 * 8 + n % 8, oc = n % 16 < 8 ? f : G + f;
+    bias[n] = b[oc];
+    for (int kh = 0; kh < S2POLY24_NKH; ++kh) {
+      const int g = s2poly24_kh_group(kh);
+      for (int k = 0; k < 16; ++k) {
+        const int j = s2poly24_k_member(kh, k), ic = s2poly24_k_channel(kh, k);
+        if (j < 0) continue;
+        const int pos = s2poly24_pos(g, j), py = pos / 5, px = pos % 5;
+        const float* t = w + ((size_t)oc * 24 + ic) * 9;
+        double u = 0.;
+        for (int ky = 0; ky < 3; ++ky)
+          for (int kx = 0; kx < 3; ++kx) u += (double)(s2poly_wcoef(py, ky) * s2poly_wcoef(px, kx)) * (double)t[ky * 3 + kx];
+        const int kin = (kh & 1) * 16 + k, slot = (kin / 4) ^ ((n >> 1) & 7);
+        img[((size_t)(kh >> 1) * NP + n) * 32 + slot * 4 + kin % 4] = (float)((double)s2poly24_sign(g, j) * u);
+      }
+    }
+  }
+  return true;
+}
+
+}
diff --git a/sketchedit_amd/csrc/se_s2poly24.hip b/sketchedit_amd/csrc/se_s2poly24.hip
--- /dev/null
+++ b/sketchedit_amd/csrc/se_s2poly24.hip
@@ -0,0 +1,319 @@
+#include "se_device.h"
+#include "se_s2poly24.h"
+
+#include <cstdlib>
+#include <type_traits>
+
+namespace se {
+
+template <int N>
+using ic24 = std::integral_constant<int, N>;
+
+template <int I, int N, typename F>
+DEVFN void static_for_s24(F&& f) {
+  if constexpr (I < N) {
+    f(ic24<I>{});
+    static_for_s24<I + 1, N>(f);
+  }
+}
+
+constexpr bool s24_need(int pos, int i) {
+  return pos >= 0 && !((i >= 2 && s2poly_src_b(pos / 5) < 0) || ((i & 1) && s2poly_src_b(pos % 5) < 0));
+}
+constexpr int s24_slot_pos(int kh, int t) {
+  if (kh < 0 || kh >= S2POLY24_NKH) return -1;
+  const int j = t / 4 == 0 ? s2poly24_kh_lo(kh) : s2poly24_kh_hi(kh, t / 4 - 1);
+  return j < 0 ? -1 : s2poly24_pos(s2poly24_kh_group(kh), j);
+}
+constexpr bool s24_it_need(int it, int u) { return s24_need(s24_slot_pos(2 * it + u / 12, u % 12), u % 4); }
+constexpr int s24_it_count(int it, int upto) {
+  int n = 0;
+  for (int u = 0; u < upto; ++u) n += s24_it_need(it, u);
+  return n;
+}
+constexpr int s24_max_gathers() {
+  int m = 0;
+  for (int it = 0; it < S2POLY24_NIT; ++it) m = s24_it_count(it, 24) > m ? s24_it_count(it, 24) : m;
+  return m;
+}
+static_assert(s24_max_gathers() <= 12, "gathers of one iteration");
+
+template <int POS, typename V>
+DEVFN V s24_signed_sum(const V (&q)[4], float negone) {
+  V ps = q[0];
+  if constexpr (s24_need(POS, 3)) ps = ps + q[3];
+  if constexpr (s24_need(POS, 1) && s24_need(POS, 2)) return (q[1] + q[2]) * negone + ps;
+  else if constexpr (s24_need(POS, 1)) return q[1] * negone + ps;
+  else if constexpr (s24_need(POS, 2)) return q[2] * negone + ps;
+  else return ps;
+}
+
+__global__ __launch_bounds__(256, 2) void s2poly24_kernel(const WinoParams p) {
+  constexpr int TILES = 64, NWV = 4, COUT = 96;
+  constexpr int NQ = 2;
+  constexpr int XB = TILES * 128, WB = COUT * 128;
+  constexpr int NIT = S2POLY24_NIT, NKH = S2POLY24_NKH;
+  constexpr unsigned PSB = 96;
+  extern __shared__ __attribute__((aligned(16))) char smem[];
+  char* Xb = smem;
+  char* Wb = smem + 3 * XB;
+
+  const int tid = threadIdx.x, lane = tid & 63;
+  const float eluw = p.act == 0 ? 1.f : 0.f;
+  const int w = __builtin_amdgcn_readfirstlane(tid >> 6);
+  const int chh = w & 1, trow0 = (w >> 1) * 32;
+  const int tile_base = (p.xcd ? xcd_tile(blockIdx.x, gridDim.x) : (int)blockIdx.x) * TILES;
+  const int tpi = p.th * p.tw;
+
+  auto tile_origin = [&](int t, int& b, int& iy, int& ix) {
+    b = (int)udiv_magic((unsigned)t, p.div_tpi_m, p.div_tpi_l);
+    const int rem = t - b * tpi;
+    iy = (int)udiv_magic((unsigned)rem, p.div_tw_m, p.div_tw_l);
+    ix = rem - iy * p.tw;
+  };
+
+  const int sg = tid & 3, srow = (tid >> 6) * 16 + ((tid >> 2) & 1) * 8 + ((tid >> 3) & 7);
+  const int swz = (srow >> 1) & 7;
+  char* xw[2] = {Xb + srow * 128 + ((sg ^ swz) << 4),
+                 Xb + srow * 128 + (((4 + sg) ^ swz) << 4)};
+  unsigned yo[5], xo[5];
+  {
+    const int t = tile_base + srow;
+    int b, iy, ix;
+    tile_origin(t < p.total_tiles ? t : 0, b, iy, ix);
+#pragma unroll
+    for (int i = 0; i < 5; ++i) {
+      const int y = 4 * iy - 1 + i, x = 4 * ix - 1 + i;
+      yo[i] = (t < p.total_tiles && (unsigned)y < (unsigned)p.h) ? (unsigned)((b * p.h + y) * p.w) * PSB + (unsigned)sg * 16u : 0x80000000u + (unsigned)sg * 16u;
+      xo[i] = ((unsigned)x < (unsigned)p.w) ? (unsigned)x * PSB : 0x80000000u;
+    }
+  }
+  const unsigned lds_w = lds_addr_of(Wb);
+  int off0, off1;
+  frag_offsets(lane, off0, off1);
+
+  const __amdgpu_buffer_rsrc_t rs0 = __builtin_amdgcn_make_buffer_rsrc((void*)p.src, 0, (int)((unsigned)p.B * (unsigned)p.h * (unsigned)p.w * PSB), 0x00020000);
+  const unsigned adj8 = (unsigned)sg * 8u;
+  auto gather = [&](auto it_c, auto u_c, auto& lo, auto& hi) {
+    typedef unsigned u32x4 __attribute__((ext_vector_type(4)));
+    typedef unsigned u32x2 __attribute__((ext_vector_type(2)));
+    constexpr int it = decltype(it_c)::value, u = decltype(u_c)::value, h = u / 12, t = u % 12, i = t % 4;
+    if constexpr (s24_it_need(it, u)) {
+      constexpr int pos = s24_slot_pos(2 * it + h, t);
+      constexpr int ry = i >= 2 ? s2poly_src_b(pos / 5) : s2poly_src_a(pos / 5), rx = (i & 1) ? s2poly_src_b(pos % 5) : s2poly_src_a(pos % 5);
+      const unsigned o = __builtin_elementwise_add_sat(yo[ry], xo[rx]);
+      if constexpr (t < 4) lo[h][i] = __builtin_bit_cast(f32x4, (u32x4)__builtin_amdgcn_raw_buffer_load_b128(rs0, (int)o, 0, 0));
+      else hi[h][t / 4 - 1][i] = __builtin_bit_cast(f32x2, (u32x2)__builtin_amdgcn_raw_buffer_load_b64(rs0, (int)(o - adj8), 64, 0));
+    }
+  };
+  auto gather_part = [&](auto it_c, auto part_c, auto& lo, auto& hi) {
+    constexpr int it = decltype(it_c)::value, part = decltype(part_c)::value, total = s24_it_count(it, 24);
+    static_for_s24<0, 24>([&](auto u_c) __attribute__((always_inline)) {
+      constexpr int u = decltype(u_c)::value;
+      if constexpr (s24_it_need(it, u) && s24_it_count(it, u) * 4 / total == part) gather(it_c, u_c, lo, hi);
+    });
+  };
+  float negone = -1.f;
+  asm volatile("" : "+v"(negone));
+  auto write_x = [&](auto it_c, int buf, const auto& lo, const auto& hi) {
+    constexpr int it = decltype(it_c)::value;
+    static_for_s24<0, 2>([&](auto h_c) __attribute__((always_inline)) {
+      constexpr int h = decltype(h_c)::value, kh = 2 * it + h, g = s2poly24_kh_group(kh);
+      if constexpr (s2poly24_kh_lo(kh) >= 0) {
+        *(f32x4*)(xw[h] + buf * XB) = s24_signed_sum<s2poly24_pos(g, s2poly24_kh_lo(kh))>(lo[h], negone);
+      } else {
+        const f32x2 a = s24_signed_sum<s2poly24_pos(g, s2poly24_kh_hi(kh, 0))>(hi[h][0], negone);
+        if constexpr (s2poly24_kh_hi(kh, 1) >= 0) {
+          const f32x2 b = s24_signed_sum<s2poly24_pos(g, s2poly24_kh_hi(kh, 1))>(hi[h][1], negone);
+          *(f32x4*)(xw[h] + buf * XB) = (f32x4){a[0], a[1], b[0], b[1]};
+        } else {
+          *(f32x2*)(xw[h] + buf * XB) = a;
+        }
+      }
+    });
+  };
+  auto dma_w = [&](int it, int buf, int j) {
+    const int rbk = j * NWV + w;
+    glds16_s(p.upk + (size_t)it * COUT * 32 + rbk * 256, (unsigned)lane * 16u, lds_w + buf * WB + rbk * 1024);
+  };
+
+  f32x4 am[3][NQ];
+  f32x4 oy[2][2][3][NQ];
+#pragma unroll
+  for (int j = 0; j < 3; ++j)
+#pragma unroll
+    for (int q = 0; q < NQ; ++q) {
+      am[j][q] = (f32x4){0.f, 0.f, 0.f, 0.f};
+      const f32x4 b4 = *(const f32x4*)(p.bias + (3 * chh + j) * 16 + (lane >> 4) * 4);
+#pragma unroll
+      for (int a = 0; a < 2; ++a)
+#pragma unroll
+        for (int b = 0; b < 2; ++b) oy[a][b][j][q] = b4;
+    }
+  auto fold = [&](auto g_c) {
+    constexpr int g = decltype(g_c)::value;
+#pragma unroll
+    for (int j = 0; j < 3; ++j)
+#pragma unroll
+      for (int q = 0; q < NQ; ++q) {
+        if constexpr (s2poly24_feeds(g, 0, 0)) oy[0][0][j][q] += am[j][q];
+        if constexpr (s2poly24_feeds(g, 0, 1)) oy[0][1][j][q] += am[j][q];
+        if constexpr (s2poly24_feeds(g, 1, 0)) oy[1][0][j][q] += am[j][q];
+        if constexpr (s2poly24_feeds(g, 1, 1)) oy[1][1][j][q] += am[j][q];
+        asm volatile("" : "+v"(oy[0][0][j][q]), "+v"(oy[0][1][j][q]), "+v"(oy[1][0][j][q]), "+v"(oy[1][1][j][q]));
+      }
+  };
+  auto fold_before = [&](auto kh_c) {
+    constexpr int kh = decltype(kh_c)::value;
+    if constexpr (kh > 0 && kh <= NKH) {
+      constexpr int gp = s2poly24_kh_group(kh - 1);
+      if constexpr ((kh == NKH || s2poly24_kh_group(kh) != gp) && s2poly24_nfeeds(gp) > 1) {
+        fold(ic24<gp>{});
+        __builtin_amdgcn_sched_barrier(0);
+      }
+    }
+  };
+  auto mfma_group = [&](auto kh_c, auto e_c, const f32x4 (&wf)[3], const f32x4 (&xf)[NQ]) {
+    constexpr int kh = decltype(kh_c)::value, e = decltype(e_c)::value, g = s2poly24_kh_group(kh);
+    if constexpr (e < s2poly24_kh_steps(kh)) {
+      constexpr bool corner = s2poly24_nfeeds(g) == 1, first = s2poly24_kh_local(kh) == 0 && e == 0;
+      constexpr int a = s2poly24_feeds(g, 0, 0) || s2poly24_feeds(g, 0, 1) ? 0 : 1, b = s2poly24_feeds(g, 0, 0) || s2poly24_feeds(g, 1, 0) ? 0 : 1;
+#pragma unroll
+      for (int j = 0; j < 3; ++j)
+#pragma unroll
+        for (int q = 0; q < NQ; ++q) {
+          if constexpr (corner) {
+            oy[a][b][j][q] = __builtin_amdgcn_mfma_f32_16x16x4f32(wf[j][e], xf[q][e], oy[a][b][j][q], 0, 0, 0);
+          } else {
+            const f32x4 cin = first ? (f32x4){0.f, 0.f, 0.f, 0.f} : am[j][q];
+            am[j][q] = __builtin_amdgcn_mfma_f32_16x16x4f32(wf[j][e], xf[q][e], cin, 0, 0, 0);
+          }
+        }
+    }
+    __builtin_amdgcn_sched_barrier(0);
+  };
+
+  auto end_barrier = [&]() {
+    __builtin_amdgcn_sched_barrier(0);
+    asm volatile("s_waitcnt lgkmcnt(0)\n\ts_barrier" ::: "memory");
+    __builtin_amdgcn_sched_barrier(0);
+  };
+
+  f32x4 lo[2][4];
+  f32x2 hi[2][2][4];
+#pragma unroll
+  for (int i0 = 0; i0 < 3; ++i0) { dma_w(i0, i0, 0); dma_w(i0, i0, 1); dma_w(i0, i0, 2); }
+  {
+    f32x4 lo1[2][4];
+    f32x2 hi1[2][2][4];
+    static_for_s24<0, 4>([&](auto part) __attribute__((always_inline)) { gather_part(ic24<0>{}, part, lo, hi); });
+    static_for_s24<0, 4>([&](auto part) __attribute__((always_inline)) { gather_part(ic24<1>{}, part, lo1, hi1); });
+    write_x(ic24<0>{}, 0, lo, hi);
+    write_x(ic24<1>{}, 1, lo1, hi1);
+  }
+  dma_wait_all();
+  __syncthreads();
+  static_for_s24<0, 4>([&](auto part) __attribute__((always_inline)) { gather_part(ic24<2>{}, part, lo, hi); });
+
+  const char* Xw = Xb + trow0 * 128;
+  const char* Ww = Wb + (3 * chh) * 2048;
+  f32x4 wa[3], xa[NQ];
+#pragma unroll
+  for (int q = 0; q < NQ; ++q) xa[q] = *(const f32x4*)(Xw + q * 2048 + off0);
+#pragma unroll
+  for (int j = 0; j < 3; ++j) wa[j] = *(const f32x4*)(Ww + j * 2048 + off0);
+
+  static_for_s24<0, NIT>([&](auto it_c) __attribute__((always_inline)) {
+    constexpr int it = decltype(it_c)::value;
+    constexpr int b0 = it % 3, b1 = (it + 1) % 3, b2 = (it + 2) % 3;
+    constexpr int w0 = it % 4, w1 = (it + 1) % 4, w3 = (it + 3) % 4;
+    constexpr bool more1 = it + 1 < NIT, more2 = it + 2 < NIT, more3 = it + 3 < NIT;
+    constexpr ic24<2 * it> kh0{};
+    constexpr ic24<2 * it + 1> kh1{};
+    constexpr ic24<(more3 ? it + 3 : 0)> it3{};
+    f32x4 wb[3], xb[NQ];
+#pragma unroll
+    for (int q = 0; q < NQ; ++q) xb[q] = *(const f32x4*)(Xw + b0 * XB + q * 2048 + off1);
+#pragma unroll
+    for (int j = 0; j < 3; ++j) wb[j] = *(const f32x4*)(Ww + w0 * WB + j * 2048 + off1);
+    __builtin_amdgcn_sched_barrier(0);
+    fold_before(kh0);
+    mfma_group(kh0, ic24<0>{}, wa, xa);
+    mfma_group(kh0, ic24<1>{}, wa, xa);
+    mfma_group(kh0, ic24<2>{}, wa, xa);
+    mfma_group(kh0, ic24<3>{}, wa, xa);
+    fold_before(kh1);
+    if constexpr (more2) {
+      dma_wait_all();
+      write_x(ic24<(more2 ? it + 2 : 0)>{}, b2, lo, hi);
+    }
+    __builtin_amdgcn_sched_barrier(0);
+    mfma_group(kh1, ic24<0>{}, wb, xb);
+    if constexpr (more3) { dma_w(it + 3, w3, 0); gather_part(it3, ic24<0>{}, lo, hi); }
+    if constexpr (more1) {
+#pragma unroll
+      for (int q = 0; q < NQ; ++q) xa[q] = *(const f32x4*)(Xw + b1 * XB + q * 2048 + off0);
+#pragma unroll
+      for (int j = 0; j < 3; ++j) wa[j] = *(const f32x4*)(Ww + w1 * WB + j * 2048 + off0);
+    }
+    __builtin_amdgcn_sched_barrier(0);
+    mfma_group(kh1, ic24<1>{}, wb, xb);
+    if constexpr (more3) { dma_w(it + 3, w3, 1); gather_part(it3, ic24<1>{}, lo, hi); }
+    __builtin_amdgcn_sched_barrier(0);
+    mfma_group(kh1, ic24<2>{}, wb, xb);
+    if constexpr (more3) { dma_w(it + 3, w3, 2); gather_part(it3, ic24<2>{}, lo, hi); }
+    __builtin_amdgcn_sched_barrier(0);
+    mfma_group(kh1, ic24<3>{}, wb, xb);
+    if constexpr (more3) gather_part(it3, ic24<3>{}, lo, hi);
+    if constexpr (more1) end_barrier();
+  });
+  fold_before(ic24<NKH>{});
+
+  const int q = lane >> 4;
+  const int OH = p.h >> 1, OW = p.w >> 1;
+  constexpr unsigned pix_bytes = COUT / 2 * 4;
+#pragma unroll
+  for (int tq = 0; tq < NQ; ++tq) {
+    const int t = tile_base + trow0 + tq * 16 + (lane & 15);
+    int b = 0, iy = 0, ix = 0;
+    tile_origin(t < p.total_tiles ? t : 0, b, iy, ix);
+#pragma unroll
+    for (int j = 0; j < 3; ++j) {
+      const int c0 = (3 * chh + j) * 8 + (q & 1) * 4 + (q >> 1) * 2;
+#pragma unroll
+      for (int a = 0; a < 2; ++a)
+#pragma unroll
+        for (int bb = 0; bb < 2; ++bb) {
+          const f32x4 v = oy[a][bb][j][tq];
+          const auto s02 = __builtin_amdgcn_permlane32_swap(__float_as_uint(v[0]), __float_as_uint(v[2]), false, false);
+          const auto s13 = __builtin_amdgcn_permlane32_swap(__float_as_uint(v[1]), __float_as_uint(v[3]), false, false);
+          const float f0 = __uint_as_float(s02[0]), g0 = __uint_as_float(s02[1]);
+          const float f1 = __uint_as_float(s13[0]), g1 = __uint_as_float(s13[1]);
+          float2 ov;
+          ov.x = act_fast(f0, eluw) * sigmoid_fast(g0);
+          ov.y = act_fast(f1, eluw) * sigmoid_fast(g1);
+          if (t < p.total_tiles)
+            *(float2*)((char*)p.dst + ((unsigned)((b * OH + 2 * iy + a) * OW + 2 * ix + bb) * pix_bytes + (unsigned)c0 * 4u)) = ov;
+        }
+    }
+  }
+}
+
+hipError_t launch_s2poly24(const WinoParams& p, hipStream_t st) {
+  constexpr int TILES = 64;
+  constexpr int LDS = 3 * TILES * 128 + 4 * 96 * 128;
+  static_assert(2 * LDS <= 160 * 1024, "two workgroups per CU");
+  if ((p.h % 4) || (p.w % 4) || p.th != p.h / 4 || p.tw != p.w / 4 || p.total_tiles != p.B * p.th * p.tw) return hipErrorInvalidValue;
+  if ((double)p.B * p.h * p.w * 96.0 >= 2147483648.0) return hipErrorInvalidValue;
+  {
+    hipError_t e = ensure_max_lds((const void*)s2poly24_kernel, LDS);
+    if (e != hipSuccess) return e;
+  }
+  const int grid = (p.total_tiles + TILES - 1) / TILES;
+  set_launch_grid(grid);
+  ProfScope ps_(st, PL_WINO_N96, "s2poly24");
+  hipLaunchKernelGGL(s2poly24_kernel, dim3(grid), dim3(TILES * 4), LDS, st, p);
+  return hipGetLastError();
+}
+
+}
diff --git a/sketchedit_amd/kernel_labels.py b/sketchedit_amd/kernel_labels.py
--- a/sketchedit_amd/kernel_labels.py
+++ b/sketchedit_amd/kernel_labels.py
@@ -3,6 +3,7 @@
     "wino_kernel": "wino_n192", "wino24_kernel": "wino_n192", "rconv16": "gconv_n192", "gconv_kernel<12": "gconv_n192",
     "wino48_kernel": "wino_n96", "rconv96": "gconv_n96", "gconv_kernel<6": "gconv_n96",
     "s2poly48_kernel": "wino_n96",
+    "s2poly24_kernel": "wino_n96",
     "winoup_kernel": "wino_up96",
     "winoup48_kernel": "gconv_n48", "rtile_dense5w_kernel": "gconv_n48", "rtile_dense5_kernel": "gconv_n48",
     "rtile_kernel<3": "gconv_n48", "gconv_kernel<3": "gconv_n48",
```

Result: no change. 3081 images/sec, median of 6 (+0.7%).
